# bezirganyan/m2-mixer

Hardware: AMD Instinct MI355X
Metric: training samples/sec AV-MNIST M2-Mixer-B bf16 (higher is better)
Workload: dtype bf16

## Files before the change

### include/m2mixer.h

```cpp
#ifndef M2MIXER_H
#define M2MIXER_H

#include <stdint.h>

#ifdef __cplusplus
extern "C" {
#endif

#define M2M_ABI_VERSION 18
#define M2M_MAX_BLOCKS 8
#define M2M_ROWS_PER_WG 16

#define M2M_SPLIT_GPART 1472

#define M2M_PREC_BF16 0
#define M2M_PREC_F32 1

typedef struct m2m_block {
    const float* ln1_w;
    const float* ln1_b;
    const float* tok_w1;
    const float* tok_b1;
    const float* tok_w2;
    const float* tok_b2;
    const float* ln2_w;
    const float* ln2_b;
    const float* ch_w1;
    const float* ch_b1;
    const float* ch_w2;
    const float* ch_b2;
    void* w1n;
    void* w2c;
    void* w2tn;
    void* w1tc;
    float* ch_b1p;
    float* g_ln1_w; float* g_ln1_b; float* g_tok_w1; float* g_tok_b1; float* g_tok_w2; float* g_tok_b2;
    float* g_ln2_w; float* g_ln2_b; float* g_ch_w1; float* g_ch_b1; float* g_ch_w2; float* g_ch_b2;
    float* x_in;
    float* x_mid;
    void* at_chn;
    void* dyt_chn;
    void* h_chn;
    void* dh_chn;
} m2m_block;

typedef struct m2m_tower {
    int32_t prec;
    int32_t D, N, T, C;
    int32_t Cp;
    int32_t nblocks;
    int32_t has_final_ln;
    float p_drop;
    uint32_t site_base;
    const float* lnf_w;
    const float* lnf_b;
    float* g_lnf_w;
    float* g_lnf_b;
    float* x_final;
    float* ws_a;
    float* ws_b;
    m2m_block blk[M2M_MAX_BLOCKS];
    float* slabs;
    int32_t nsplit;
    int32_t wgrad_flags;
    float* xres;
    float* gpart;
    void* a_nat[M2M_MAX_BLOCKS];
    void* dy_nat[M2M_MAX_BLOCKS];
    float* wslot[M2M_MAX_BLOCKS];
    void* dx0_chn;
} m2m_tower;
#define M2M_WGRAD_OVERWRITE 1
#define M2M_WGRAD_GROUP_SLOTS 4
#define M2M_WGRAD_REDUCES_SMALL 2

typedef struct m2m_embed {
    int32_t prec;
    int32_t Cin, H, W, ph, pw;
    int32_t D;
    int32_t K;
    int32_t Kp;
    const float* w;
    const float* b;
    void* wn;
    float* g_w;
    float* g_b;
    int32_t wgrad_flags;
    int32_t reserved;
} m2m_embed;

int m2m_abi_version(void);
const char* m2m_last_error(void);
int64_t m2m_packed_bytes(int prec, int64_t I, int64_t K);

int m2m_pack(int prec, int mode, int order_k_major, const float* src, int64_t stride_i, int64_t stride_k,
             int64_t I, int64_t K, void* dst, void* stream);
int m2m_pack_tower(const m2m_tower* t, void* stream);
int m2m_pack_embed(const m2m_embed* e, void* stream);
int m2m_pack_all(const m2m_tower* const* towers, int ntowers, const m2m_embed* const* embeds, int nembeds, void* stream);
int m2m_pack_skips_w1tc(const m2m_tower* t);

int m2m_embed_forward(const m2m_embed* e, const float* input, int B, float* x0, void* stream);
typedef struct m2m_step_head {
    float* adam_state; uint32_t* drop_counter; float* losses; int32_t nlosses;
} m2m_step_head;
int m2m_embeds_forward(const m2m_embed* const* embeds, const float* const* inputs, float* const* x0s, const int* nsplits,
                       const int64_t* part_strides, int nembeds, int B, const m2m_step_head* head, void* stream);
int m2m_embed_fwd_splits(const m2m_embed* e);
int m2m_embed_forward_head(const m2m_embed* e, const float* input, int B, float* x0, const m2m_step_head* head, void* stream);

int m2m_tower_forward(const m2m_tower* t, const float* x0, int64_t x0_sample_stride, int B,
                      float* out, int64_t out_sample_stride, float* pooled,
                      int training, uint32_t seed, uint32_t step, const uint32_t* step_dev, void* stream);

int m2m_towers_can_group(const m2m_tower* a, const m2m_tower* b, int B);
typedef struct m2m_tower_io {
    const float* x0; int64_t x0_sample_stride;
    float* out; int64_t out_sample_stride;
    float* pooled;
    int32_t x0_parts;
    int64_t x0_part_stride;
} m2m_tower_io;
int m2m_towers_forward(const m2m_tower* const* towers, const m2m_tower_io* io, int ntowers, int B, int training,
                       uint32_t seed, uint32_t step, const uint32_t* step_dev, void* stream);
int m2m_towers_forward_embeds_ok(const m2m_tower* const* towers, int ntowers, const m2m_embed* const* embeds, int B);
int m2m_towers_forward_embeds(const m2m_tower* const* towers, const m2m_tower_io* io, int ntowers,
                              const m2m_embed* const* embeds, const float* const* inputs, const m2m_step_head* head,
                              int B, int training, uint32_t seed, uint32_t step, const uint32_t* step_dev, void* stream);

int m2m_tower_backward(const m2m_tower* t, int B, const float* d_out, int64_t d_out_sample_stride,
                       const float* d_pooled, float* d_x0, int64_t d_x0_sample_stride,
                       uint32_t seed, uint32_t step, const uint32_t* step_dev, void* stream);
typedef struct m2m_tower_gio {
    const float* d_out; int64_t d_out_sample_stride;
    const float* d_pooled;
    float* d_x0; int64_t d_x0_sample_stride;
} m2m_tower_gio;
int m2m_towers_backward(const m2m_tower* const* towers, const m2m_tower_gio* io, int ntowers, int B,
                        uint32_t seed, uint32_t step, const uint32_t* step_dev, void* stream);
int m2m_tower_wgrad(const m2m_tower* t, int B, uint32_t seed, uint32_t step, const uint32_t* step_dev, void* stream);
int m2m_wgrad_form(const m2m_tower* t, int B);
int m2m_towers_wgrad(const m2m_tower* const* towers, const m2m_tower* const* dev_towers, int ntowers,
                     const m2m_embed* const* embeds, const float* const* inputs, const float* const* d_x0s,
                     const m2m_tower* const* embed_towers, int nembeds,
                     int B, uint32_t seed, uint32_t step, const uint32_t* step_dev, void* stream);
int m2m_wgrad_groups(const m2m_tower* t, int B);
int m2m_embeds_wgrad_form(const m2m_embed* const* embeds, const m2m_tower* const* embed_towers, int nembeds, int B);
int m2m_wgrad_slot_groups(const m2m_tower* const* towers, int ntowers, int B);
int m2m_wgrad_fold(const m2m_tower* t, void* stream);
int m2m_embed_wgrad(const m2m_embed* e, const float* input, const float* d_x0, int B, void* stream);
int m2m_embeds_wgrad(const m2m_embed* const* embeds, const float* const* inputs, const float* const* d_x0s, int nembeds, int B,
                     void* stream);

typedef struct m2m_head {
    const float* pooled;
    const float* w;
    const float* b;
    float* g_w;
    float* g_b;
    float* d_pooled;
    float weight;
    float* g_part;
    const float* tokens;
    int64_t tok_sample_stride;
    int32_t ntok;
} m2m_head;
int m2m_heads_part_tiles(int B);
int m2m_heads_ce(const m2m_head* heads, int nheads, const int64_t* labels, int B, int D, int K,
                 float* logits, float* losses, int32_t* preds, int zero_losses, void* stream);

int m2m_heads_bce(const m2m_head* heads, int nheads, const float* targets, const float* pos_weight, int B, int D, int K,
                  float* logits, float* losses, int32_t* preds, int zero_losses, void* stream);

int m2m_heads_ce_w(const m2m_head* heads, int nheads, const int64_t* labels, int B, int D, int K,
                   float* logits, float* losses, int32_t* preds, int zero_losses, const float* weights, void* stream);
int m2m_heads_bce_w(const m2m_head* heads, int nheads, const float* targets, const float* pos_weight, int B, int D, int K,
                    float* logits, float* losses, int32_t* preds, int zero_losses, const float* weights, void* stream);

int m2m_towers_wgrad_heads(const m2m_tower* const* towers, const m2m_tower* const* dev_towers, int ntowers,
                           const m2m_embed* const* embeds, const float* const* inputs, const float* const* d_x0s,
                           const m2m_tower* const* embed_towers, int nembeds,
                           int B, uint32_t seed, uint32_t step, const uint32_t* step_dev,
                           const m2m_head* heads, int nheads, int K, void* stream);

int m2m_towers_wgrad_tail(const m2m_tower* const* towers, const m2m_tower* const* dev_towers, int ntowers,
                          const m2m_embed* const* embeds, const float* const* inputs, const float* const* d_x0s,
                          const m2m_tower* const* embed_towers, int nembeds,
                          int B, uint32_t seed, uint32_t step, const uint32_t* step_dev,
                          const m2m_head* heads, int nheads, int K, uint32_t* bump_counter, void* stream);

int m2m_tower_backward_heads_ok(const m2m_tower* t, int B, int nheads, int K);
int m2m_tower_backward_heads(const m2m_tower* t, int B, const m2m_head* heads, int nheads, int own, const int64_t* labels,
                             int K, float* logits, float* losses, int32_t* preds, float* d_x0, int64_t d_x0_sample_stride,
                             uint32_t seed, uint32_t step, const uint32_t* step_dev, void* stream);

#define M2M_MLP_MAX_LAYERS 4
typedef struct m2m_mlp {
    int32_t nlayers;
    int32_t has_out;
    int32_t dims[M2M_MLP_MAX_LAYERS + 1];
    float p_drop;
    uint32_t site_base;
    const float* w[M2M_MLP_MAX_LAYERS];
    const float* b[M2M_MLP_MAX_LAYERS];
    float* g_w[M2M_MLP_MAX_LAYERS];
    float* g_b[M2M_MLP_MAX_LAYERS];
    float* act[M2M_MLP_MAX_LAYERS];
} m2m_mlp;
int m2m_mlp_forward(const m2m_mlp* m, const float* x, int B, float* out, int64_t out_sample_stride, float* out_dense,
                    int training, uint32_t seed, uint32_t step, const uint32_t* step_dev, void* stream);
int m2m_mlp_backward(const m2m_mlp* m, const float* x, int B, const float* d_out, int64_t d_out_sample_stride,
                     const float* d_out_dense, void* stream);
int m2m_mlp_forward_ride(const m2m_mlp* m, const float* x, int B, float* out, int64_t out_sample_stride, float* out_dense,
                         int training, uint32_t seed, uint32_t step, const uint32_t* step_dev);
int m2m_mlp_backward_ride(const m2m_mlp* m, const float* x, int B, const float* d_out, int64_t d_out_sample_stride,
                          const float* d_out_dense);
int m2m_mlp_ride_flush(void* stream);

int m2m_adam_step(float* param, float* grad, float* exp_avg, float* exp_avg_sq, int64_t n,
                  float* state, float beta1, float beta2, float eps, float weight_decay,
                  float grad_scale, int bump_step, void* stream);
int m2m_adam_step_bf16(float* param, float* grad, const void* grad_bf16, float* exp_avg, float* exp_avg_sq, int64_t n,
                       float* state, float beta1, float beta2, float eps, float weight_decay,
                       float grad_scale, int bump_step, void* stream);

#define M2M_MAX_GRAD_RANGES 16
typedef struct m2m_grad_range { int64_t lo, n; const float* add; int32_t keep; int32_t reserved; } m2m_grad_range;
int m2m_adam_step_ranges(float* param, float* grad, const void* grad_bf16, float* exp_avg, float* exp_avg_sq, int64_t n,
                         float* state, float beta1, float beta2, float eps, float weight_decay, float grad_scale, int bump_step,
                         const m2m_grad_range* ranges, int nranges, void* stream);

int64_t m2m_adam_pack_plan_bytes(void);
int m2m_adam_pack_plan(const m2m_tower* const* towers, int ntowers, const m2m_embed* const* embeds, int nembeds,
                       float* param, float* grad, const void* grad_bf16, float* exp_avg, float* exp_avg_sq, int64_t n,
                       const float* state, float beta1, float beta2, float eps, float weight_decay, float grad_scale,
                       void* plan_host);
int m2m_adam_pack_plan_ranges(const m2m_tower* const* towers, int ntowers, const m2m_embed* const* embeds, int nembeds,
                              float* param, float* grad, const void* grad_bf16, float* exp_avg, float* exp_avg_sq, int64_t n,
                              const float* state, float beta1, float beta2, float eps, float weight_decay, float grad_scale,
                              const m2m_grad_range* ranges, int nranges, void* plan_host);
int m2m_adam_pack_all(const m2m_tower* const* towers, int ntowers, const m2m_embed* const* embeds, int nembeds,
                      const void* plan_dev, const void* plan_host, void* stream);

int m2m_step_prologue(float* adam_state, uint32_t* drop_counter, float* losses, int nlosses, void* stream);

int m2m_counter_add(uint32_t* counter, uint32_t delta, void* stream);

#define M2M_FUSION_SUM 1
#define M2M_FUSION_MEAN 2
#define M2M_FUSION_MAX 3
int m2m_fusion_forward(int mode, const float* a, const float* b, float* y, int64_t n, void* stream);
int m2m_fusion_backward(int mode, const float* a, const float* b, const float* dy, float* da, float* db, int64_t n, void* stream);

typedef struct m2m_gate {
    int32_t D;
    int32_t reserved;
    const float *w1, *b1, *w2, *b2, *wz, *bz;
    float *g_w1, *g_b1, *g_w2, *g_b2, *g_wz, *g_bz;
    float *t1, *t2, *z, *dh, *part;
} m2m_gate;
int64_t m2m_gate_part_floats(int64_t rows, int D);
int m2m_gate_forward(const m2m_gate* g, const float* a, const float* b, float* y, int64_t rows, int save, void* stream);
int m2m_gate_backward(const m2m_gate* g, const float* dy, float* da, float* db, int64_t rows, void* stream);
int m2m_gate_wgrad(const m2m_gate* g, const float* a, const float* b, int64_t rows, void* stream);

#define M2M_SCORES_MAX_CLASSES 64
#define M2M_SCORES_MAX_LABELS 128
int m2m_scores_multiclass(const int32_t* preds, const int64_t* labels, int nheads, int B, int K, uint64_t* table, void* stream);
int m2m_scores_multilabel(const int32_t* preds, const float* targets, int nheads, int B, int K, uint64_t* table, void* stream);

int m2m_dropout_mask(const m2m_tower* t, int blk, int site, int B, uint32_t seed, uint32_t step,
                     uint8_t* mask, void* stream);
int m2m_gelu_probe(const float* x, float* y, float* dy, int64_t n, void* stream);
int m2m_gelu_table_probe(int form, const float* x, float* y, float* dy, int64_t n, float scale, void* stream);
int m2m_gemm_probe(int prec, const float* A, const float* Bm, int I, int J, int K,
                   const float* Bc, int J2, float* C, float* C2, void* workspace, void* stream);

int m2m_clock_probe(uint64_t* out, int nwg, int spin_ticks, void* stream);

#ifdef __cplusplus
}
#endif
#endif
```

### m2_mixer_amd/_lib.py

```python
from __future__ import annotations

import ctypes as C
import os
import subprocess

_HERE = os.path.dirname(os.path.abspath(__file__))
LIB_PATH = os.environ.get("M2M_LIB_PATH", os.path.join(_HERE, "libm2mixer.so"))
CSRC = os.path.join(_HERE, "csrc")

ABI_VERSION = 18
MAX_BLOCKS = 8
ROWS_PER_WG = 16
HCHN_PAD = 4096
SPLIT_ROWS = 128
SPLIT_MAX = 8
SPLIT_GPART = 1472
PREC_BF16, PREC_F32 = 0, 1
PREC_BY_NAME = {"bf16": PREC_BF16, "fp32": PREC_F32, "f32": PREC_F32}

_fp = C.c_void_p


class Block(C.Structure):
    PARAMS = ["ln1_w", "ln1_b", "tok_w1", "tok_b1", "tok_w2", "tok_b2", "ln2_w", "ln2_b",
              "ch_w1", "ch_b1", "ch_w2", "ch_b2"]
    PACKED = ["w1n", "w2c", "w2tn", "w1tc", "ch_b1p"]
    GRADS = ["g_" + p for p in PARAMS]
    SAVED = ["x_in", "x_mid", "at_chn", "dyt_chn", "h_chn", "dh_chn"]
    _fields_ = [(n, _fp) for n in PARAMS + PACKED + GRADS + SAVED]


class Tower(C.Structure):
    _fields_ = [("prec", C.c_int32), ("D", C.c_int32), ("N", C.c_int32), ("T", C.c_int32), ("C", C.c_int32),
                ("Cp", C.c_int32), ("nblocks", C.c_int32), ("has_final_ln", C.c_int32),
                ("p_drop", C.c_float), ("site_base", C.c_uint32),
                ("lnf_w", _fp), ("lnf_b", _fp), ("g_lnf_w", _fp), ("g_lnf_b", _fp), ("x_final", _fp),
                ("ws_a", _fp), ("ws_b", _fp), ("blk", Block * MAX_BLOCKS),
                ("slabs", _fp), ("nsplit", C.c_int32), ("wgrad_flags", C.c_int32), ("xres", _fp), ("gpart", _fp),
                ("a_nat", _fp * MAX_BLOCKS), ("dy_nat", _fp * MAX_BLOCKS),
                ("wslot", _fp * MAX_BLOCKS),
                ("dx0_chn", _fp)]


WGRAD_OVERWRITE = 1
WGRAD_REDUCES_SMALL = 2
WGRAD_GROUP_SLOTS = 4
MAX_GRAD_RANGES = 16


class GradRange(C.Structure):
    _fields_ = [("lo", C.c_int64), ("n", C.c_int64), ("add", _fp), ("keep", C.c_int32), ("reserved", C.c_int32)]


class TowerIO(C.Structure):
    _fields_ = [("x0", _fp), ("x0_ss", C.c_int64), ("out", _fp), ("out_ss", C.c_int64), ("pooled", _fp),
                ("x0_parts", C.c_int32), ("x0_part_stride", C.c_int64)]


class StepHead(C.Structure):
    _fields_ = [("adam_state", _fp), ("drop_counter", _fp), ("losses", _fp), ("nlosses", C.c_int32)]


class TowerGIO(C.Structure):
    _fields_ = [("d_out", _fp), ("d_out_ss", C.c_int64), ("d_pooled", _fp), ("d_x0", _fp), ("d_x0_ss", C.c_int64)]


class Embed(C.Structure):
    _fields_ = [("prec", C.c_int32), ("Cin", C.c_int32), ("H", C.c_int32), ("W", C.c_int32), ("ph", C.c_int32),
                ("pw", C.c_int32), ("D", C.c_int32), ("K", C.c_int32), ("Kp", C.c_int32),
                ("w", _fp), ("b", _fp), ("wn", _fp), ("g_w", _fp), ("g_b", _fp), ("wgrad_flags", C.c_int32), ("reserved", C.c_int32)]


class Head(C.Structure):
    _fields_ = [("pooled", _fp), ("w", _fp), ("b", _fp), ("g_w", _fp), ("g_b", _fp), ("d_pooled", _fp),
                ("weight", C.c_float), ("g_part", _fp), ("tokens", _fp), ("tok_sample_stride", C.c_int64), ("ntok", C.c_int32)]


SCORES_MAX_CLASSES, SCORES_MAX_LABELS = 64, 128
FUSION_SUM, FUSION_MEAN, FUSION_MAX = 1, 2, 3


class Gate(C.Structure):
    _fields_ = [("D", C.c_int32), ("reserved", C.c_int32)] + [(n, _fp) for n in (
        "w1", "b1", "w2", "b2", "wz", "bz", "g_w1", "g_b1", "g_w2", "g_b2", "g_wz", "g_bz", "t1", "t2", "z", "dh", "part")]


MLP_MAX_LAYERS = 4


class Mlp(C.Structure):
    _fields_ = [("nlayers", C.c_int32), ("has_out", C.c_int32), ("dims", C.c_int32 * (MLP_MAX_LAYERS + 1)),
                ("p_drop", C.c_float), ("site_base", C.c_uint32),
                ("w", _fp * MLP_MAX_LAYERS), ("b", _fp * MLP_MAX_LAYERS), ("g_w", _fp * MLP_MAX_LAYERS),
                ("g_b", _fp * MLP_MAX_LAYERS), ("act", _fp * MLP_MAX_LAYERS)]


SIGNATURES = {
    "m2m_abi_version": (C.c_int, []),
    "m2m_last_error": (C.c_char_p, []),
    "m2m_packed_bytes": (C.c_int64, [C.c_int, C.c_int64, C.c_int64]),
    "m2m_pack": (C.c_int, [C.c_int, C.c_int, C.c_int, _fp, C.c_int64, C.c_int64, C.c_int64, C.c_int64, _fp, _fp]),
    "m2m_pack_tower": (C.c_int, [C.POINTER(Tower), _fp]),
    "m2m_pack_embed": (C.c_int, [C.POINTER(Embed), _fp]),
    "m2m_pack_skips_w1tc": (C.c_int, [C.POINTER(Tower)]),
    "m2m_pack_all": (C.c_int, [C.POINTER(C.POINTER(Tower)), C.c_int, C.POINTER(C.POINTER(Embed)), C.c_int, _fp]),
    "m2m_embed_forward": (C.c_int, [C.POINTER(Embed), _fp, C.c_int, _fp, _fp]),
    "m2m_embed_forward_head": (C.c_int, [C.POINTER(Embed), _fp, C.c_int, _fp, C.POINTER(StepHead), _fp]),
    "m2m_tower_forward": (C.c_int, [C.POINTER(Tower), _fp, C.c_int64, C.c_int, _fp, C.c_int64, _fp, C.c_int,
                                    C.c_uint32, C.c_uint32, _fp, _fp]),
    "m2m_tower_backward": (C.c_int, [C.POINTER(Tower), C.c_int, _fp, C.c_int64, _fp, _fp, C.c_int64,
                                     C.c_uint32, C.c_uint32, _fp, _fp]),
    "m2m_tower_backward_heads_ok": (C.c_int, [C.POINTER(Tower), C.c_int, C.c_int, C.c_int]),
    "m2m_tower_backward_heads": (C.c_int, [C.POINTER(Tower), C.c_int, C.POINTER(Head), C.c_int, C.c_int, _fp, C.c_int, _fp, _fp, _fp, _fp,
                                           C.c_int64, C.c_uint32, C.c_uint32, _fp, _fp]),
    "m2m_tower_wgrad": (C.c_int, [C.POINTER(Tower), C.c_int, C.c_uint32, C.c_uint32, _fp, _fp]),
    "m2m_towers_can_group": (C.c_int, [C.POINTER(Tower), C.POINTER(Tower), C.c_int]),
    "m2m_towers_forward": (C.c_int, [C.POINTER(C.POINTER(Tower)), C.POINTER(TowerIO), C.c_int, C.c_int, C.c_int, C.c_uint32,
                                     C.c_uint32, _fp, _fp]),
    "m2m_towers_forward_embeds_ok": (C.c_int, [C.POINTER(C.POINTER(Tower)), C.c_int, C.POINTER(C.POINTER(Embed)), C.c_int]),
    "m2m_towers_forward_embeds": (C.c_int, [C.POINTER(C.POINTER(Tower)), C.POINTER(TowerIO), C.c_int, C.POINTER(C.POINTER(Embed)),
                                            C.POINTER(_fp), C.POINTER(StepHead), C.c_int, C.c_int, C.c_uint32, C.c_uint32, _fp, _fp]),
    "m2m_towers_backward": (C.c_int, [C.POINTER(C.POINTER(Tower)), C.POINTER(TowerGIO), C.c_int, C.c_int, C.c_uint32, C.c_uint32,
                                      _fp, _fp]),
    "m2m_towers_wgrad": (C.c_int, [C.POINTER(C.POINTER(Tower)), C.POINTER(_fp), C.c_int, C.POINTER(C.POINTER(Embed)), C.POINTER(_fp),
                                   C.POINTER(_fp), C.POINTER(C.POINTER(Tower)), C.c_int, C.c_int, C.c_uint32, C.c_uint32, _fp, _fp]),
    "m2m_towers_wgrad_heads": (C.c_int, [C.POINTER(C.POINTER(Tower)), C.POINTER(_fp), C.c_int, C.POINTER(C.POINTER(Embed)), C.POINTER(_fp),
                                         C.POINTER(_fp), C.POINTER(C.POINTER(Tower)), C.c_int, C.c_int, C.c_uint32, C.c_uint32, _fp,
                                         C.POINTER(Head), C.c_int, C.c_int, _fp]),
    "m2m_towers_wgrad_tail": (C.c_int, [C.POINTER(C.POINTER(Tower)), C.POINTER(_fp), C.c_int, C.POINTER(C.POINTER(Embed)), C.POINTER(_fp),
                                        C.POINTER(_fp), C.POINTER(C.POINTER(Tower)), C.c_int, C.c_int, C.c_uint32, C.c_uint32, _fp,
                                        C.POINTER(Head), C.c_int, C.c_int, _fp, _fp]),
    "m2m_heads_part_tiles": (C.c_int, [C.c_int]),
    "m2m_wgrad_form": (C.c_int, [C.POINTER(Tower), C.c_int]),
    "m2m_embeds_wgrad_form": (C.c_int, [C.POINTER(C.POINTER(Embed)), C.POINTER(C.POINTER(Tower)), C.c_int, C.c_int]),
    "m2m_wgrad_groups": (C.c_int, [C.POINTER(Tower), C.c_int]),
    "m2m_wgrad_slot_groups": (C.c_int, [C.POINTER(C.POINTER(Tower)), C.c_int, C.c_int]),
    "m2m_wgrad_fold": (C.c_int, [C.POINTER(Tower), _fp]),
    "m2m_adam_step_ranges": (C.c_int, [_fp, _fp, _fp, _fp, _fp, C.c_int64, _fp, C.c_float, C.c_float, C.c_float, C.c_float,
                                       C.c_float, C.c_int, C.POINTER(GradRange), C.c_int, _fp]),
    "m2m_counter_add": (C.c_int, [_fp, C.c_uint32, _fp]),
    "m2m_embed_wgrad": (C.c_int, [C.POINTER(Embed), _fp, _fp, C.c_int, _fp]),
    "m2m_embeds_wgrad": (C.c_int, [C.POINTER(C.POINTER(Embed)), C.POINTER(_fp), C.POINTER(_fp), C.c_int, C.c_int, _fp]),
    "m2m_embeds_forward": (C.c_int, [C.POINTER(C.POINTER(Embed)), C.POINTER(_fp), C.POINTER(_fp), C.POINTER(C.c_int), C.POINTER(C.c_int64),
                                     C.c_int, C.c_int, C.POINTER(StepHead), _fp]),
    "m2m_embed_fwd_splits": (C.c_int, [C.POINTER(Embed)]),
    "m2m_heads_ce": (C.c_int, [C.POINTER(Head), C.c_int, _fp, C.c_int, C.c_int, C.c_int, _fp, _fp, _fp, C.c_int, _fp]),
    "m2m_step_prologue": (C.c_int, [_fp, _fp, _fp, C.c_int, _fp]),
    "m2m_heads_bce": (C.c_int, [C.POINTER(Head), C.c_int, _fp, _fp, C.c_int, C.c_int, C.c_int, _fp, _fp, _fp, C.c_int, _fp]),
    "m2m_heads_ce_w": (C.c_int, [C.POINTER(Head), C.c_int, _fp, C.c_int, C.c_int, C.c_int, _fp, _fp, _fp, C.c_int, _fp, _fp]),
    "m2m_heads_bce_w": (C.c_int, [C.POINTER(Head), C.c_int, _fp, _fp, C.c_int, C.c_int, C.c_int, _fp, _fp, _fp, C.c_int, _fp, _fp]),
    "m2m_fusion_forward": (C.c_int, [C.c_int, _fp, _fp, _fp, C.c_int64, _fp]),
    "m2m_fusion_backward": (C.c_int, [C.c_int, _fp, _fp, _fp, _fp, _fp, C.c_int64, _fp]),
    "m2m_gate_part_floats": (C.c_int64, [C.c_int64, C.c_int]),
    "m2m_gate_forward": (C.c_int, [C.POINTER(Gate), _fp, _fp, _fp, C.c_int64, C.c_int, _fp]),
    "m2m_gate_backward": (C.c_int, [C.POINTER(Gate), _fp, _fp, _fp, C.c_int64, _fp]),
    "m2m_gate_wgrad": (C.c_int, [C.POINTER(Gate), _fp, _fp, C.c_int64, _fp]),
    "m2m_scores_multiclass": (C.c_int, [_fp, _fp, C.c_int, C.c_int, C.c_int, _fp, _fp]),
    "m2m_scores_multilabel": (C.c_int, [_fp, _fp, C.c_int, C.c_int, C.c_int, _fp, _fp]),
    "m2m_mlp_forward": (C.c_int, [C.POINTER(Mlp), _fp, C.c_int, _fp, C.c_int64, _fp, C.c_int, C.c_uint32, C.c_uint32,
                                  _fp, _fp]),
    "m2m_mlp_backward": (C.c_int, [C.POINTER(Mlp), _fp, C.c_int, _fp, C.c_int64, _fp, _fp]),
    "m2m_mlp_forward_ride": (C.c_int, [C.POINTER(Mlp), _fp, C.c_int, _fp, C.c_int64, _fp, C.c_int, C.c_uint32, C.c_uint32, _fp]),
    "m2m_mlp_backward_ride": (C.c_int, [C.POINTER(Mlp), _fp, C.c_int, _fp, C.c_int64, _fp]),
    "m2m_mlp_ride_flush": (C.c_int, [_fp]),
    "m2m_adam_step": (C.c_int, [_fp, _fp, _fp, _fp, C.c_int64, _fp, C.c_float, C.c_float, C.c_float, C.c_float,
                                C.c_float, C.c_int, _fp]),
    "m2m_adam_step_bf16": (C.c_int, [_fp, _fp, _fp, _fp, _fp, C.c_int64, _fp, C.c_float, C.c_float, C.c_float, C.c_float,
                                     C.c_float, C.c_int, _fp]),
    "m2m_adam_pack_plan_bytes": (C.c_int64, []),
    "m2m_adam_pack_plan": (C.c_int, [C.POINTER(C.POINTER(Tower)), C.c_int, C.POINTER(C.POINTER(Embed)), C.c_int, _fp, _fp, _fp, _fp, _fp,
                                    C.c_int64, _fp, C.c_float, C.c_float, C.c_float, C.c_float, C.c_float, _fp]),
    "m2m_adam_pack_plan_ranges": (C.c_int, [C.POINTER(C.POINTER(Tower)), C.c_int, C.POINTER(C.POINTER(Embed)), C.c_int, _fp, _fp, _fp, _fp, _fp,
                                           C.c_int64, _fp, C.c_float, C.c_float, C.c_float, C.c_float, C.c_float,
                                           C.POINTER(GradRange), C.c_int, _fp]),
    "m2m_adam_pack_all": (C.c_int, [C.POINTER(C.POINTER(Tower)), C.c_int, C.POINTER(C.POINTER(Embed)), C.c_int, _fp, _fp, _fp]),
    "m2m_dropout_mask": (C.c_int, [C.POINTER(Tower), C.c_int, C.c_int, C.c_int, C.c_uint32, C.c_uint32, _fp, _fp]),
    "m2m_gelu_probe": (C.c_int, [_fp, _fp, _fp, C.c_int64, _fp]),
    "m2m_gelu_table_probe": (C.c_int, [C.c_int, _fp, _fp, _fp, C.c_int64, C.c_float, _fp]),
    "m2m_gemm_probe": (C.c_int, [C.c_int, _fp, _fp, C.c_int, C.c_int, C.c_int, _fp, C.c_int, _fp, _fp, _fp, _fp]),
    "m2m_clock_probe": (C.c_int, [_fp, C.c_int, C.c_int, _fp]),
}

_lib = None


def csrc_hash() -> str:
    import glob
    import hashlib
    h = hashlib.sha256()
    for f in sorted(glob.glob(os.path.join(CSRC, "*.hip")) + glob.glob(os.path.join(CSRC, "*.h")) +
                    [os.path.join(os.path.dirname(_HERE), "include", "m2mixer.h")]):
        h.update(os.path.basename(f).encode())
        h.update(open(f, "rb").read())
    return h.hexdigest()


def build(force: bool = False, verbose: bool = False) -> str:
    if force:
        subprocess.run(["make", "-C", CSRC, "clean"], check=True, capture_output=not verbose)
    r = subprocess.run(["make", "-C", CSRC, "-j", str(min(6, os.cpu_count() or 2))], capture_output=True, text=True)
    if r.returncode != 0:
        raise RuntimeError("building libm2mixer.so failed:\n" + r.stdout[-4000:] + r.stderr[-4000:])
    if verbose:
        print(r.stdout)
    return LIB_PATH


def lib() -> C.CDLL:
    global _lib
    if _lib is None:
        if not os.path.exists(LIB_PATH):
            raise RuntimeError(
                f"{LIB_PATH} is missing: the M2-Mixer hot path exists only as the HIP library "
                "(python -c 'import __graft_entry__ as g; g.build()' builds it); there is no CPU fallback")
        L = C.CDLL(LIB_PATH)
        for name, (res, args) in SIGNATURES.items():
            fn = getattr(L, name)
            fn.restype = res
            fn.argtypes = args
        got = L.m2m_abi_version()
        if got != ABI_VERSION:
            raise RuntimeError(f"libm2mixer ABI {got} != binding ABI {ABI_VERSION}; rebuild")
        _lib = L
    return _lib


def check(rc: int, what: str = "") -> None:
    if rc != 0:
        msg = lib().m2m_last_error().decode("utf-8", "replace")
        kind = "unsupported shape/argument" if rc == -1 else "HIP runtime error"
        raise RuntimeError(f"libm2mixer {what}: {kind}: {msg}")


def ptr(t) -> int:
    return 0 if t is None else t.data_ptr()


def stream_ptr() -> int:
    import torch
    return torch.cuda.current_stream().cuda_stream


def packed_bytes(prec: int, I: int, K: int) -> int:
    kb = 32 if prec == PREC_BF16 else 16
    return ((I + 15) // 16) * ((K + kb - 1) // kb) * 1024
```

### m2_mixer_amd/config.py

```python
from __future__ import annotations

import os

from . import _lib as L

_state = {
    "precision": os.environ.get("M2M_PRECISION", "bf16"),
    "seed": None,
    "device_step": False,
}


SWITCHES = {
    "M2M_PRECISION": ("bf16", "import of config", "bf16 / fp32: the precision of engines and modules built without an explicit one"),
    "M2M_LIB_PATH": (None, "import of _lib", "load another build of libm2mixer.so (default: the one beside the package)"),
    "M2M_DIST_BACKEND": (None, "parallel.init_from_env", "torch.distributed backend (default nccl on GPUs; gloo: several ranks on one GPU)"),
    "M2M_FUSED_UPDATE": (None, "engine construction", "1 / 0 force Adam + operand re-pack as one launch / as two; unset: one launch"),
    "M2M_CONCURRENT": ("1", "engine construction", "0: every launch on the main stream, no grouped two-tower launches"),
    "M2M_WGRAD_OVERWRITE": ("1", "engine construction", "weight gradients with a single owner are written, Adam leaves them uncleared"),
    "M2M_WGRAD_SLOT": ("1", "engine construction", "second row group of a grouped weight-gradient launch into a slot that Adam adds"),
    "M2M_EARLY_FUSION_WGRAD": ("0", "engine construction", "wide towers: the fusion tower's weight gradients on a side stream"),
    "M2M_HEADS_POOL": ("1", "engine construction", "wide towers: the heads launch pools the tower outputs itself"),
    "M2M_DEFER_SMALL": ("1", "engine construction", "the fusion backward's small-gradient slots are reduced by the weight-gradient launch"),
    "M2M_HEAD_SLOTS": ("1", "engine construction", "the heads' weight gradients through slots (bit-reproducible) instead of float atomics"),
    "M2M_GROUP_SLOTS": ("1", "engine construction", "the two-tower backward's small gradients through per-workgroup slots"),
    "M2M_EMBED_FAST": ("1", "engine construction", "patch-embedding weight gradients in the single-owner form (d_x0^T image)"),
    "M2M_EMBED_FOLD": ("0", "engine construction", "patch embeddings inside the two-tower forward launch"),
    "M2M_MIMIC_STREAMS": (None, "engine construction", "none / fwd / bwd / both: side streams of the MIMIC step; unset: none up to batch 1024, else both"),
    "M2M_MIMIC_MERGED_TAIL": ("1", "engine construction", "MIMIC on one stream: one weight-gradient launch, one Adam, one re-pack"),
    "M2M_MIMIC_EMBED_WGRAD_MERGED": ("1", "engine construction", "MIMIC merged tail: the input projection's weight gradient inside the towers' launch"),
    "M2M_MLP_RIDE": ("1", "engine construction", "MIMIC: the static MLP's workgroups ride in the time tower's token-mixing launches"),
    "M2M_CAPTURE_SHARE_SLOTS": ("0", "engine.capture()", "multi-step capture: every step reads the same input slot (diagnostic)"),
}


def switch(name: str, default=None):
    return os.environ.get(name, SWITCHES[name][0] if default is None else default)


def switch_on(name: str) -> bool:
    return switch(name) != "0" if SWITCHES[name][0] == "1" else switch(name) == "1"


def set_precision(name: str) -> None:
    if name not in L.PREC_BY_NAME:
        raise ValueError(f"precision must be one of {sorted(L.PREC_BY_NAME)}")
    _state["precision"] = name


def get_precision() -> str:
    return _state["precision"]


def prec_id(name: str | None = None) -> int:
    return L.PREC_BY_NAME[name or _state["precision"]]


def set_dropout_seed(seed: int) -> None:
    _state["seed"] = int(seed) & 0xFFFFFFFF


def dropout_seed() -> int:
    if _state["seed"] is None:
        import torch
        _state["seed"] = int(torch.initial_seed()) & 0xFFFFFFFF
    return _state["seed"]


def set_device_dropout_step(on: bool) -> None:
    _state["device_step"] = bool(on)


def device_dropout_step() -> bool:
    return _state["device_step"]
```

### m2_mixer_amd/csrc/embed.hip

```cpp
#include "tile.h"
#include "embed_wgrad.h"

#include "embed_fwd.h"
#include "dispatch.h"

template <int P, int D, int RB>
__global__ __launch_bounds__(NTHREADS) void embed_fwd_kernel(const m2m_embed em, const float* __restrict__ in, long M, int N,
                                                             float* __restrict__ x0, int fast, const m2m_step_head head) {
    extern __shared__ __attribute__((aligned(16))) char smem[];
    if (blockIdx.x == 0) {
        const int t = threadIdx.x;
        if (t == 0 && head.adam_state) head.adam_state[0] += 1.0f;
        if (t == 1 && head.drop_counter) *head.drop_counter += 1u;
        if (head.losses && t < head.nlosses) head.losses[t] = 0.f;
    }
    if (P == PREC_BF16 && fast) embed_fwd_fast_body<D>(em, in, M, N, x0, blockIdx.x, 0, 1, smem);
    else embed_fwd_body<P, D, RB>(em, in, M, N, x0, blockIdx.x, smem);
}

struct EmbedFwdGroupArgs {
    m2m_embed em[2];
    const float* in[2];
    float* x0[2];
    long M[2];
    int N[2], nwg0, fast[2], nsplit[2];
    long part_stride[2];
    float* adam_state;
    unsigned int* drop_counter;
    float* losses;
    int nlosses, prologue;
};
template <int P, int D, int RB>
__global__ __launch_bounds__(NTHREADS, (P == PREC_BF16 && D <= 128) ? 4 : 1) void embed_fwd_group_kernel(const EmbedFwdGroupArgs a) {
    extern __shared__ __attribute__((aligned(16))) char smem[];
    if (a.prologue && blockIdx.x == 0) {
        const int t = threadIdx.x;
        if (t == 0 && a.adam_state) a.adam_state[0] += 1.0f;
        if (t == 1 && a.drop_counter) *a.drop_counter += 1u;
        if (a.losses && t < a.nlosses) a.losses[t] = 0.f;
    }
    const int e = (int)blockIdx.x < a.nwg0 ? 0 : 1;
    const int wg = e ? blockIdx.x - a.nwg0 : blockIdx.x;
    if (P == PREC_BF16 && a.fast[e]) {
        const int ns = a.nsplit[e], split = wg % ns;
        embed_fwd_fast_body<D>(a.em[e], a.in[e], a.M[e], a.N[e], a.x0[e] + split * a.part_stride[e], wg / ns, split, ns, smem);
    }
    else {
        const int ns = a.nsplit[e], split = wg % ns, tile = wg / ns;
        if (split == 0) embed_fwd_body<P, D, RB>(a.em[e], a.in[e], a.M[e], a.N[e], a.x0[e], tile, smem);
        else {
            float* part = a.x0[e] + split * a.part_stride[e];
            const long m0 = (long)tile * RB;
            for (int idx = threadIdx.x; idx < RB * D; idx += NTHREADS) {
                const long m = m0 + idx / D;
                if (m < a.M[e]) part[m * D + idx % D] = 0.f;
            }
        }
    }
}

template <int P, int D>
__global__ __launch_bounds__(NTHREADS) void embed_wgrad_kernel(const m2m_embed em, const float* __restrict__ in,
                                                               const float* __restrict__ dx0, long M, int N, int tiles_per_group) {
    extern __shared__ __attribute__((aligned(16))) char smem[];
    embed_wgrad_body<P, D, NTHREADS>(em, in, dx0, M, N, tiles_per_group, blockIdx.x, blockIdx.y, gridDim.y == 1, smem);
}

template <int P, int D>
__global__ __launch_bounds__(NTHREADS) void embed_wgrad_group_kernel(const EmbedWgradGroupArgs a) {
    extern __shared__ __attribute__((aligned(16))) char smem[];
    embed_wgrad_group_body<P, D, NTHREADS>(a, blockIdx.x, smem);
}

int m2m_check_embed(const m2m_embed* e, int B) {
    if (!e || B < 1) { m2m_set_error("embed: bad argument", __FILE__, __LINE__); return -1; }
    if (e->H % e->ph || e->W % e->pw) { m2m_set_error("embed: image not divisible by patch", __FILE__, __LINE__); return -1; }
    if (e->K != e->Cin * e->ph * e->pw) { m2m_set_error("embed: K != Cin*ph*pw", __FILE__, __LINE__); return -1; }
    const int KB = e->prec == PREC_BF16 ? 32 : 16;
    if (e->Kp % KB || e->Kp < e->K) { m2m_set_error("embed: Kp must be K rounded up to the k-block", __FILE__, __LINE__); return -1; }
    if (e->Kp > EMB_KMAX - EMB_KS) { m2m_set_error("embed: patch too large (Cin*ph*pw must be <= 3968)", __FILE__, __LINE__); return -1; }
    return 0;
}

template <int P, int D>
static int launch_embed_fwd(const m2m_embed* e, const float* in, int B, float* x0, hipStream_t st, const m2m_step_head* head = nullptr) {
    m2m_step_head hd;
    memset(&hd, 0, sizeof(hd));
    if (head) {
        if (head->nlosses < 0 || head->nlosses > 64) { m2m_set_error("embed_forward: step head nlosses must be in [0, 64]", __FILE__, __LINE__); return -1; }
        hd = *head;
    }
    const int N = (e->H / e->ph) * (e->W / e->pw);
    const long M = (long)B * N;
    constexpr int RB = 16;
    const size_t lds = (size_t)RB * EMB_LD * 4 + (size_t)RB * EMB_KS * Prec<P>::ESZ + EMB_KMAX * 4 + RB * 8;
    return m2m_launch<embed_fwd_kernel<P, D, RB>>(dim3((unsigned)((M + RB - 1) / RB)), dim3(NTHREADS), lds, lds, st, *e, in, M, N, x0,
                                                  (int)embed_fwd_fast_ok(e, in), hd);
}
template <int P, int D>
static int launch_embed_fwd_group(const m2m_embed* const* es, const float* const* ins, float* const* x0s, const int* nsplits,
                                  const int64_t* part_strides, const m2m_step_head* head, int B, hipStream_t st) {
    constexpr int RB = 16;
    EmbedFwdGroupArgs a;
    memset(&a, 0, sizeof(a));
    if (head) {
        if (head->nlosses < 0 || head->nlosses > 64) { m2m_set_error("embeds_forward: step head nlosses must be in [0, 64]", __FILE__, __LINE__); return -1; }
        a.prologue = 1; a.adam_state = head->adam_state; a.drop_counter = head->drop_counter; a.losses = head->losses; a.nlosses = head->nlosses;
    }
    const int first = es[1]->Kp > es[0]->Kp ? 1 : 0;
    int total = 0;
    for (int k = 0; k < 2; ++k) {
        const int i = k == 0 ? first : 1 - first;
        const int N = (es[i]->H / es[i]->ph) * (es[i]->W / es[i]->pw);
        a.em[k] = *es[i]; a.in[k] = ins[i]; a.x0[k] = x0s[i]; a.N[k] = N; a.M[k] = (long)B * N;
        a.fast[k] = embed_fwd_fast_ok(es[i], ins[i]);
        a.nsplit[k] = nsplits ? nsplits[i] : 1;
        a.part_stride[k] = part_strides ? (long)part_strides[i] : 0;
        if (a.nsplit[k] < 1 || a.nsplit[k] > 4 || (a.nsplit[k] > 1 && a.part_stride[k] < a.M[k] * (long)D)) {
            m2m_set_error("embeds_forward: 1..4 k-splits, part stride >= B*N*D", __FILE__, __LINE__);
            return -1;
        }
        const int nwg = (int)((a.M[k] + RB - 1) / RB) * a.nsplit[k];
        if (k == 0) a.nwg0 = nwg;
        total += nwg;
    }
    const size_t lds = (size_t)RB * EMB_LD * 4 + (size_t)RB * EMB_KS * Prec<P>::ESZ + EMB_KMAX * 4 + RB * 8;
    return m2m_launch<embed_fwd_group_kernel<P, D, RB>>(dim3((unsigned)total), dim3(NTHREADS), lds, lds, st, a);
}

template <int P, int D>
static int launch_embed_wgrad(const m2m_embed* e, const float* in, const float* dx0, int B, hipStream_t st) {
    const EmbedWgradPlan pl = embed_wgrad_plan(e, B, 256);
    const size_t lds = embed_wgrad_lds<D, P>();
    return m2m_launch<embed_wgrad_kernel<P, D>>(dim3((unsigned)pl.nchunks, (unsigned)pl.groups), dim3(NTHREADS), lds, lds, st, *e, in, dx0, pl.M, pl.N, pl.tpg);
}
template <int P, int D>
static int launch_embed_wgrad_group(const m2m_embed* const* es, const float* const* ins, const float* const* dx0s, int B, hipStream_t st) {
    EmbedWgradGroupArgs a;
    const int total = embed_wgrad_group_args(a, es, ins, dx0s, B, 256);
    const size_t lds = embed_wgrad_lds<D, P>();
    return m2m_launch<embed_wgrad_group_kernel<P, D>>(dim3((unsigned)total), dim3(NTHREADS), lds, lds, st, a);
}

extern "C" int m2m_embed_forward(const m2m_embed* e, const float* input, int B, float* x0, void* stream) {
    return m2m_embed_forward_head(e, input, B, x0, nullptr, stream);
}
extern "C" int m2m_embed_forward_head(const m2m_embed* e, const float* input, int B, float* x0, const m2m_step_head* head, void* stream) {
    if (int rc = m2m_check_embed(e, B)) return rc;
    hipStream_t st = reinterpret_cast<hipStream_t>(stream);
    const int rc = m2m_dispatch_pd(m2m_wide_dims{}, e->prec, e->D, [&](auto P, auto D) { return launch_embed_fwd<P(), D()>(e, input, B, x0, st, head); });
    if (rc != M2M_NO_BUILD) return rc;
    m2m_set_error("embed_forward: unsupported (prec, D)", __FILE__, __LINE__);
    return -1;
}

extern "C" int m2m_embed_wgrad(const m2m_embed* e, const float* input, const float* d_x0, int B, void* stream) {
    if (int rc = m2m_check_embed(e, B)) return rc;
    hipStream_t st = reinterpret_cast<hipStream_t>(stream);
    const int rc = m2m_dispatch_pd(m2m_wide_dims{}, e->prec, e->D, [&](auto P, auto D) { return launch_embed_wgrad<P(), D()>(e, input, d_x0, B, st); });
    if (rc != M2M_NO_BUILD) return rc;
    m2m_set_error("embed_wgrad: unsupported (prec, D)", __FILE__, __LINE__);
    return -1;
}

extern "C" int m2m_embeds_wgrad(const m2m_embed* const* embeds, const float* const* inputs, const float* const* d_x0s, int nembeds,
                                int B, void* stream) {
    if (!embeds || !inputs || !d_x0s || nembeds != EMB_GROUP) { m2m_set_error("embeds_wgrad: exactly two embeddings", __FILE__, __LINE__); return -1; }
    for (int i = 0; i < nembeds; ++i) {
        if (int rc = m2m_check_embed(embeds[i], B)) return rc;
        if (embeds[i]->prec != embeds[0]->prec || embeds[i]->D != embeds[0]->D) {
            m2m_set_error("embeds_wgrad: the embeddings of one launch must share precision and hidden_dim", __FILE__, __LINE__);
            return -1;
        }
    }
    hipStream_t st = reinterpret_cast<hipStream_t>(stream);
    const m2m_embed* e = embeds[0];
    const int rc = m2m_dispatch_pd(m2m_wide_dims{}, e->prec, e->D, [&](auto P, auto D) { return launch_embed_wgrad_group<P(), D()>(embeds, inputs, d_x0s, B, st); });
    if (rc != M2M_NO_BUILD) return rc;
    m2m_set_error("embeds_wgrad: unsupported (prec, D)", __FILE__, __LINE__);
    return -1;
}

extern "C" int m2m_embed_fwd_splits(const m2m_embed* e) {
    if (!e) return 1;
    static const int forced = m2m_env_int("M2M_EMBED_SPLITS", 0);
    const bool pays = embed_fwd_fast_ok(e, nullptr) && e->Kp >= 4 * EMB_FKS;
    if (pays && forced >= 1 && forced <= 4) return forced;
    return pays ? 2 : 1;
}

extern "C" int m2m_embeds_forward(const m2m_embed* const* embeds, const float* const* inputs, float* const* x0s, const int* nsplits,
                                  const int64_t* part_strides, int nembeds, int B, const m2m_step_head* head, void* stream) {
    if (!embeds || !inputs || !x0s || nembeds != 2) { m2m_set_error("embeds_forward: exactly two embeddings", __FILE__, __LINE__); return -1; }
    for (int i = 0; i < nembeds; ++i) {
        if (int rc = m2m_check_embed(embeds[i], B)) return rc;
        if (embeds[i]->prec != embeds[0]->prec || embeds[i]->D != embeds[0]->D) {
            m2m_set_error("embeds_forward: the embeddings of one launch must share precision and hidden_dim", __FILE__, __LINE__);
            return -1;
        }
    }
    hipStream_t st = reinterpret_cast<hipStream_t>(stream);
    const m2m_embed* e = embeds[0];
    const int rc = m2m_dispatch_pd(m2m_wide_dims{}, e->prec, e->D, [&](auto P, auto D) { return launch_embed_fwd_group<P(), D()>(embeds, inputs, x0s, nsplits, part_strides, head, B, st); });
    if (rc != M2M_NO_BUILD) return rc;
    m2m_set_error("embeds_forward: unsupported (prec, D)", __FILE__, __LINE__);
    return -1;
}
```

### m2_mixer_amd/csrc/embed_fwd.h

```cpp
#pragma once
#include "tile.h"
#include "embed_wgrad.h"

#define EMB_KS 128
#define EMB_LD (EMB_KS + 4)
#define EMB_KMAX 4096

template <int P, int D, int RB>
static __device__ __forceinline__ void embed_fwd_body(const m2m_embed& em, const float* __restrict__ in, long M, int N,
                                                      float* __restrict__ x0, int wg, char* smem) {
    typedef Prec<P> Pr;
    constexpr int DT = D / 16, KSB = EMB_KS / Pr::KB;
    constexpr int DPW = (DT + NWAVES - 1) / NWAVES;
    float* tile = reinterpret_cast<float*>(smem);
    char* img = smem + RB * EMB_LD * 4;
    int* koff = reinterpret_cast<int*>(img + RB * EMB_KS * Pr::ESZ);
    long* rbase = reinterpret_cast<long*>(koff + EMB_KMAX);

    const int tid = threadIdx.x, lane = tid & 63, wave = tid >> 6, g = lane >> 4, il = lane & 15;
    PatchGeom pg{em.Cin, em.H, em.W, em.ph, em.pw, em.W / em.pw, N, em.K};
    const long m0 = (long)wg * RB;
    const int nKB = em.Kp / Pr::KB;
    const int kext = (em.Kp + EMB_KS - 1) / EMB_KS * EMB_KS;
    for (int k = tid; k < kext; k += NTHREADS) koff[k] = patch_koff(pg, k);
    if (tid < RB) rbase[tid] = patch_rowbase(pg, m0 + tid, M);

    f32x4_t acc[(RB / 16)][DPW];
#pragma unroll
    for (int mt = 0; mt < (RB / 16); ++mt)
#pragma unroll
        for (int j = 0; j < DPW; ++j) acc[mt][j] = f32x4_t{0.f, 0.f, 0.f, 0.f};

    constexpr int EPT = RB * EMB_KS / NTHREADS;
    float pre[EPT];
    Frag wpre[DPW][KSB];
    auto load_stage = [&](int k0) {
#pragma unroll
        for (int i = 0; i < EPT; ++i) {
            const int idx = i * NTHREADS + tid;
            const int r = idx / EMB_KS, kk = idx % EMB_KS;
            const long rb = rbase[r];
            const int ko = koff[k0 + kk];
            pre[i] = (rb >= 0 && ko >= 0) ? in[rb + ko] : 0.f;
        }
        const int kb0 = k0 / Pr::KB;
#pragma unroll
        for (int j = 0; j < DPW; ++j) {
            const int dt = wave + NWAVES * j;
#pragma unroll
            for (int kb = 0; kb < KSB; ++kb) {
                wpre[j][kb].u = u32x4_t{0u, 0u, 0u, 0u};
                if (dt < DT && kb0 + kb < nKB) wpre[j][kb] = ld_frag_global(em.wn, (long)dt * nKB + kb0 + kb, lane);
            }
        }
    };
    __syncthreads();
    load_stage(0);
    for (int k0 = 0; k0 < em.Kp; k0 += EMB_KS) {
#pragma unroll
        for (int i = 0; i < EPT; ++i) {
            const int idx = i * NTHREADS + tid;
            tile[(idx / EMB_KS) * EMB_LD + idx % EMB_KS] = pre[i];
        }
        Frag wcur[DPW][KSB];
#pragma unroll
        for (int j = 0; j < DPW; ++j)
#pragma unroll
            for (int kb = 0; kb < KSB; ++kb) wcur[j][kb] = wpre[j][kb];
        __syncthreads();
        if (k0 + EMB_KS < em.Kp) load_stage(k0 + EMB_KS);
        for (int slot = tid; slot < (RB / 16) * KSB * 64; slot += NTHREADS) {
            const int blk = slot >> 6;
            *reinterpret_cast<u32x4_t*>(img + slot * 16) =
                gather_slot<P>(tile, EMB_LD, PACK_NAT, false, blk / KSB, blk % KSB, slot & 63);
        }
        __syncthreads();
#pragma unroll
        for (int j = 0; j < DPW; ++j) {
            const int dt = wave + NWAVES * j;
            if (dt < DT) {
#pragma unroll
                for (int kb = 0; kb < KSB; ++kb) {
#pragma unroll
                    for (int mt = 0; mt < (RB / 16); ++mt) {
                        const Frag a = ld_frag_lds(img, mt * KSB + kb, lane);
                        Pr::mma(acc[mt][j], a, wcur[j][kb]);
                    }
                }
            }
        }
    }
#pragma unroll
    for (int j = 0; j < DPW; ++j) {
        const int dt = wave + NWAVES * j;
        if (dt < DT) {
            const int d = 16 * dt + il;
            const float bv = em.b[d];
#pragma unroll
            for (int mt = 0; mt < (RB / 16); ++mt)
#pragma unroll
                for (int r = 0; r < 4; ++r) {
                    const long m = m0 + 16 * mt + 4 * g + r;
                    if (m < M) x0[m * D + d] = acc[mt][j][r] + bv;
                }
        }
    }
}

#define EMB_FKS 256
#define EMB_FDEPTH 2
template <int D>
static __device__ __forceinline__ void embed_fwd_fast_body(const m2m_embed& em, const float* __restrict__ in, long M, int N,
                                                           float* __restrict__ x0, int wg, int split, int nsplit, char* smem) {
    typedef Prec<PREC_BF16> Pr;
    constexpr int KSB = EMB_FKS / 32, DT = D / 16, DPW = (DT + NWAVES - 1) / NWAVES, IMG_B = 16 * EMB_FKS * 2;
    static_assert(KSB == NWAVES, "one k-block of the stage per wave");
    char* img = smem;
    const int tid = threadIdx.x, lane = tid & 63, wave = tid >> 6, g = lane >> 4, il = lane & 15;
    PatchGeom pg{em.Cin, em.H, em.W, em.ph, em.pw, em.W / em.pw, N, em.K};
    const long m0 = (long)wg * 16;
    const long rb = patch_rowbase(pg, m0 + il, M);
    const int nKB = em.Kp / 32;
    const int nst_all = (em.Kp + EMB_FKS - 1) / EMB_FKS;
    const int per = (nst_all + nsplit - 1) / nsplit;
    const int st_begin = split * per, nst = min(nst_all, st_begin + per);

    f32x4_t acc[DPW];
#pragma unroll
    for (int j = 0; j < DPW; ++j) acc[j] = f32x4_t{0.f, 0.f, 0.f, 0.f};
    struct Pre {
        f32x4_t p0, p1;
        Frag w[DPW][KSB];
    };
    auto load = [&](Pre& p, int st) {
        const int k = min(st * EMB_FKS + wave * 32 + 8 * g, em.K - 8);
        const float* src = in + (rb >= 0 ? rb : 0) + patch_koff(pg, k);
        p.p0 = *reinterpret_cast<const f32x4_t*>(src);
        p.p1 = *reinterpret_cast<const f32x4_t*>(src + 4);
#pragma unroll
        for (int j = 0; j < DPW; ++j) {
            const int dt = min(wave + NWAVES * j, DT - 1);
#pragma unroll
            for (int kb = 0; kb < KSB; ++kb) p.w[j][kb] = ld_frag_global(em.wn, (long)dt * nKB + min(st * KSB + kb, nKB - 1), lane);
        }
    };
    auto step = [&](Pre& p, int st) {
        const bool valid = rb >= 0 && st < nst && st * EMB_FKS + wave * 32 + 8 * g < em.K;
        Frag f;
        f.u[0] = pack_bf2(p.p0[0], p.p0[1]); f.u[1] = pack_bf2(p.p0[2], p.p0[3]);
        f.u[2] = pack_bf2(p.p1[0], p.p1[1]); f.u[3] = pack_bf2(p.p1[2], p.p1[3]);
        if (!valid) f.u = u32x4_t{0u, 0u, 0u, 0u};
        char* cur = img + ((st - st_begin) & 1) * IMG_B;
        *reinterpret_cast<u32x4_t*>(cur + tid * 16) = f.u;
        __syncthreads();
#pragma unroll
        for (int kb = 0; kb < KSB; ++kb) {
            const Frag a = ld_frag_lds(cur, kb, lane);
#pragma unroll
            for (int j = 0; j < DPW; ++j)
                if (wave + NWAVES * j < DT) Pr::mma(acc[j], a, p.w[j][kb]);
        }
        load(p, st + EMB_FDEPTH);
    };
    Pre ring[EMB_FDEPTH];
#pragma unroll
    for (int d = 0; d < EMB_FDEPTH; ++d) load(ring[d], st_begin + d);
    for (int st = st_begin; st < nst; st += EMB_FDEPTH) {
#pragma unroll
        for (int d = 0; d < EMB_FDEPTH; ++d) step(ring[d], st + d);
    }
#pragma unroll
    for (int j = 0; j < DPW; ++j) {
        const int dt = wave + NWAVES * j;
        if (dt < DT) {
            const int d = 16 * dt + il;
            const float bv = split == 0 ? em.b[d] : 0.f;
#pragma unroll
            for (int r = 0; r < 4; ++r) {
                const long m = m0 + 4 * g + r;
                if (m < M) x0[m * D + d] = acc[j][r] + bv;
            }
        }
    }
}
static inline bool embed_fwd_fast_ok(const m2m_embed* e, const float* in) {
    return e->prec == PREC_BF16 && e->pw % 8 == 0 && e->W % 4 == 0 && e->K >= 8 && (reinterpret_cast<uintptr_t>(in) & 15) == 0;
}
```

### m2_mixer_amd/csrc/embed_wgrad.h

```cpp
#pragma once
#include "host.h"

#define EBM 32

struct PatchGeom {
    int Cin, H, W, ph, pw, GW, N, K;
};
static __device__ __forceinline__ int patch_koff(const PatchGeom& pg, int k) {
    if (k >= pg.K) return -1;
    const int c = k / (pg.ph * pg.pw), rem = k % (pg.ph * pg.pw);
    const int py = rem / pg.pw, px = rem % pg.pw;
    return (c * pg.H + py) * pg.W + px;
}
static __device__ __forceinline__ long patch_rowbase(const PatchGeom& pg, long m, long M) {
    if (m >= M) return -1;
    const long b = m / pg.N;
    const int n = (int)(m % pg.N);
    const int gy = n / pg.GW, gx = n % pg.GW;
    return (b * pg.Cin * pg.H + gy * pg.ph) * (long)pg.W + gx * pg.pw;
}

template <int P, int D, int NT>
static __device__ __forceinline__ void embed_wgrad_body(const m2m_embed& em, const float* __restrict__ in,
                                                        const float* __restrict__ dx0, long M, int N, int tiles_per_group,
                                                        int chunk, int group, bool single, char* smem) {
    typedef Prec<P> Pr;
    constexpr int DT = D / 16, NKM = EBM / Pr::KB, XLD = TileGeom<D>::XLD;
    constexpr int KC = 64, KCT = KC / 16, PLD = KC + 4;
    constexpr int DPW = (DT + (NT / 64) - 1) / (NT / 64);
    constexpr int NDX = (EBM * (D / 4) + NT - 1) / NT;
    constexpr int NPT = EBM * KC / NT;
    static_assert(NT % KC == 0 && EBM % (NT / KC) == 0, "patch tile mapping");
    float* dxt = reinterpret_cast<float*>(smem);
    float* pt = dxt + EBM * XLD;
    char* aimg = reinterpret_cast<char*>(pt + EBM * PLD);
    char* bimg = aimg + EBM * D * Pr::ESZ;

    const int tid = threadIdx.x, lane = tid & 63, wave = tid >> 6, g = lane >> 4, il = lane & 15;
    PatchGeom pg{em.Cin, em.H, em.W, em.ph, em.pw, em.W / em.pw, N, em.K};
    const int k0 = chunk * KC;
    const int ko = patch_koff(pg, k0 + (tid % KC));

    f32x4_t acc[DPW][KCT];
#pragma unroll
    for (int j = 0; j < DPW; ++j)
#pragma unroll
        for (int kt = 0; kt < KCT; ++kt) acc[j][kt] = f32x4_t{0.f, 0.f, 0.f, 0.f};
    float bsum = 0.f;

    const long ntiles = (M + EBM - 1) / EBM;
    const long t_begin = (long)group * tiles_per_group;
    const long t_end = min(ntiles, t_begin + tiles_per_group);
    float4 dxr[NDX];
    float ptr_[NPT];
    auto load_tile = [&](long tl) {
        const long m0 = tl * EBM;
#pragma unroll
        for (int i = 0; i < NDX; ++i) {
            const int idx = i * NT + tid;
            const int r = idx / (D / 4), c = (idx % (D / 4)) * 4;
            dxr[i] = make_float4(0.f, 0.f, 0.f, 0.f);
            if (idx < EBM * (D / 4) && m0 + r < M) dxr[i] = *reinterpret_cast<const float4*>(dx0 + (m0 + r) * D + c);
        }
#pragma unroll
        for (int i = 0; i < NPT; ++i) {
            const long rb = patch_rowbase(pg, m0 + tid / KC + (NT / KC) * i, M);
            ptr_[i] = (rb >= 0 && ko >= 0) ? in[rb + ko] : 0.f;
        }
    };
    if (t_begin < t_end) load_tile(t_begin);
    for (long tl = t_begin; tl < t_end; ++tl) {
        __syncthreads();
#pragma unroll
        for (int i = 0; i < NDX; ++i) {
            const int idx = i * NT + tid;
            if (idx < EBM * (D / 4)) *reinterpret_cast<float4*>(dxt + (idx / (D / 4)) * XLD + (idx % (D / 4)) * 4) = dxr[i];
        }
#pragma unroll
        for (int i = 0; i < NPT; ++i) pt[(tid / KC + (NT / KC) * i) * PLD + tid % KC] = ptr_[i];
        if (tl + 1 < t_end) load_tile(tl + 1);
        __syncthreads();
        if (chunk == 0 && tid < D) {
            float s = 0.f;
            for (int r = 0; r < EBM; ++r) s += dxt[r * XLD + tid];
            bsum += s;
        }
        for (int slot = tid; slot < DT * NKM * 64; slot += NT) {
            const int blk = slot >> 6;
            *reinterpret_cast<u32x4_t*>(aimg + slot * 16) =
                gather_slot<P>(dxt, XLD, PACK_NAT, true, blk / NKM, blk % NKM, slot & 63);
        }
        for (int slot = tid; slot < KCT * NKM * 64; slot += NT) {
            const int blk = slot >> 6;
            *reinterpret_cast<u32x4_t*>(bimg + slot * 16) =
                gather_slot<P>(pt, PLD, PACK_NAT, true, blk / NKM, blk % NKM, slot & 63);
        }
        __syncthreads();
#pragma unroll
        for (int j = 0; j < DPW; ++j) {
            const int dt = wave + (NT / 64) * j;
            if (dt < DT) {
#pragma unroll
                for (int kbm = 0; kbm < NKM; ++kbm) {
                    const Frag a = ld_frag_lds(aimg, dt * NKM + kbm, lane);
#pragma unroll
                    for (int kt = 0; kt < KCT; ++kt) {
                        const Frag b = ld_frag_lds(bimg, kt * NKM + kbm, lane);
                        Pr::mma(acc[j][kt], a, b);
                    }
                }
            }
        }
    }
#pragma unroll
    for (int j = 0; j < DPW; ++j) {
        const int dt = wave + (NT / 64) * j;
        if (dt < DT) {
#pragma unroll
            for (int kt = 0; kt < KCT; ++kt)
#pragma unroll
                for (int r = 0; r < 4; ++r) {
                    const int d = 16 * dt + 4 * g + r, k = k0 + 16 * kt + il;
                    if (k < em.K) {
                        float* p = em.g_w + (long)d * em.K + k;
                        if (single) *p += acc[j][kt][r]; else atomicAdd(p, acc[j][kt][r]);
                    }
                }
        }
    }
    if (chunk == 0 && tid < D) { if (single) em.g_b[tid] += bsum; else atomicAdd(em.g_b + tid, bsum); }
}

#define EFK 32
template <int D, int NT> static constexpr size_t embed_wgrad_fast_red_bytes() { return (size_t)(NT / 64) * (EFK / 16) * (D / 16) * 64 * 16; }
template <int D, int NT>
static __device__ __forceinline__ void embed_wgrad_fast_body(const m2m_embed& em, const float* __restrict__ in,
                                                             const char* __restrict__ dx0_chn, long M, int N, int npairs, int rpt,
                                                             int chunk, bool vec2, char* smem) {
    typedef Prec<PREC_BF16> Pr;
    constexpr int DT = D / 16, NW = NT / 64, NB = EFK / 16;
    static_assert(NB == 2, "two 16-column fragments per workgroup (the 8-byte gather pairs them)");
    const int tid = threadIdx.x, lane = tid & 63, g = lane >> 4, il = lane & 15;
    const int wave = __builtin_amdgcn_readfirstlane(tid >> 6);
    PatchGeom pg{em.Cin, em.H, em.W, em.ph, em.pw, em.W / em.pw, N, em.K};
    const int k0 = chunk * EFK;
    int ko[NB];
#pragma unroll
    for (int jb = 0; jb < NB; ++jb) ko[jb] = patch_koff(pg, vec2 ? k0 + 2 * il + jb : k0 + 16 * jb + il);
    int* tokoff = reinterpret_cast<int*>(smem + embed_wgrad_fast_red_bytes<D, NT>());
    for (int n = tid; n < N; n += NT) tokoff[n] = (n / pg.GW) * pg.ph * pg.W + (n % pg.GW) * pg.pw;
    __syncthreads();
    const unsigned int sstride = (unsigned int)(em.Cin * em.H * em.W), uN = (unsigned int)N, uM = (unsigned int)M;
    const unsigned int magic = 0xFFFFFFFFu / uN;

    f32x4_t acc[NB][DT];
#pragma unroll
    for (int jb = 0; jb < NB; ++jb)
#pragma unroll
        for (int dt = 0; dt < DT; ++dt) acc[jb][dt] = f32x4_t{0.f, 0.f, 0.f, 0.f};

    struct Tile { Frag a[DT]; float v[NB][8]; unsigned int okbits; };
    auto load = [&](Tile& t, int p) {
#pragma unroll
        for (int dt = 0; dt < DT; ++dt) t.a[dt] = ld_frag_global(dx0_chn, (long)p * DT + dt, lane);
        unsigned int rb[8];
        bool okr[8];
#pragma unroll
        for (int e = 0; e < 8; ++e) {
            const int r = 4 * g + (e & 3);
            const unsigned int row = (unsigned int)((2 * p + (e >> 2)) * rpt + r);
            okr[e] = r < rpt && row < uM;
            const unsigned int rowc = okr[e] ? row : 0u;
            unsigned int q = __umulhi(rowc, magic);
            unsigned int n = rowc - q * uN;
            if (n >= uN) { n -= uN; q += 1u; }
            rb[e] = q * sstride + (unsigned int)tokoff[n];
        }
        if (vec2) {
            const unsigned int k2 = (unsigned int)max(ko[0], 0);
#pragma unroll
            for (int e = 0; e < 8; ++e) {
                const float2 x = *reinterpret_cast<const float2*>(in + rb[e] + k2);
                t.v[0][e] = x.x; t.v[1][e] = x.y;
            }
        } else {
#pragma unroll
            for (int e = 0; e < 8; ++e)
#pragma unroll
                for (int jb = 0; jb < NB; ++jb) t.v[jb][e] = in[rb[e] + (unsigned int)max(ko[jb], 0)];
        }
        t.okbits = 0u;
#pragma unroll
        for (int e = 0; e < 8; ++e) t.okbits |= (okr[e] ? 1u : 0u) << e;
    };
    auto mac = [&](const Tile& t) {
#pragma unroll
        for (int jb = 0; jb < NB; ++jb) {
            Frag b;
            float z[8];
#pragma unroll
            for (int e = 0; e < 8; ++e) z[e] = ((t.okbits >> e) & 1u) && ko[jb] >= 0 ? t.v[jb][e] : 0.f;
#pragma unroll
            for (int e = 0; e < 4; ++e) b.u[e] = pack_bf2(z[2 * e], z[2 * e + 1]);
#pragma unroll
            for (int dt = 0; dt < DT; ++dt) Pr::mma(acc[jb][dt], t.a[dt], b);
        }
    };
    Tile t0, t1;
    const int p0 = wave;
    if (p0 < npairs) load(t0, p0);
    for (int p = p0; p < npairs; p += 2 * NW) {
        if (p + NW < npairs) load(t1, p + NW);
        mac(t0);
        if (p + NW < npairs) {
            if (p + 2 * NW < npairs) load(t0, p + 2 * NW);
            mac(t1);
        }
    }
    f32x4_t* red = reinterpret_cast<f32x4_t*>(smem);
#pragma unroll
    for (int jb = 0; jb < NB; ++jb)
#pragma unroll
        for (int dt = 0; dt < DT; ++dt) red[((wave * NB + jb) * DT + dt) * 64 + lane] = acc[jb][dt];
    __syncthreads();
    for (int q = wave; q < NB * DT; q += NW) {
        const int jb = q / DT, dt = q % DT;
        f32x4_t s = red[q * 64 + lane];
#pragma unroll
        for (int w = 1; w < NW; ++w) s = s + red[(w * NB * DT + q) * 64 + lane];
        const int k = vec2 ? k0 + 2 * il + jb : k0 + 16 * jb + il;
        if (k < em.K) {
            const bool store = (em.wgrad_flags & M2M_WGRAD_OVERWRITE) != 0;
#pragma unroll
            for (int r = 0; r < 4; ++r) {
                float* qd = em.g_w + (long)(16 * dt + 4 * g + r) * em.K + k;
                *qd = store ? s[r] : *qd + s[r];
            }
        }
    }
    if (chunk == 0) {
        Frag ones;
        ones.u = u32x4_t{0x3F803F80u, 0x3F803F80u, 0x3F803F80u, 0x3F803F80u};
        f32x4_t accb[DT];
#pragma unroll
        for (int dt = 0; dt < DT; ++dt) accb[dt] = f32x4_t{0.f, 0.f, 0.f, 0.f};
        for (int p = wave; p < npairs; p += NW) {
            Frag a[DT];
#pragma unroll
            for (int dt = 0; dt < DT; ++dt) a[dt] = ld_frag_global(dx0_chn, (long)p * DT + dt, lane);
#pragma unroll
            for (int dt = 0; dt < DT; ++dt) Pr::mma(accb[dt], a[dt], ones);
        }
        __syncthreads();
#pragma unroll
        for (int dt = 0; dt < DT; ++dt) red[(wave * DT + dt) * 64 + lane] = accb[dt];
        __syncthreads();
        for (int dt = wave; dt < DT; dt += NW) {
            f32x4_t sb = red[dt * 64 + lane];
#pragma unroll
            for (int w = 1; w < NW; ++w) sb = sb + red[(w * DT + dt) * 64 + lane];
            if (il == 0) {
#pragma unroll
                for (int r = 0; r < 4; ++r) em.g_b[16 * dt + 4 * g + r] += sb[r];
            }
        }
    }
}
template <int D, int NT> static constexpr size_t embed_wgrad_fast_lds() { return embed_wgrad_fast_red_bytes<D, NT>() + 128 * sizeof(int); }

#define EMB_GROUP 2
struct EmbedWgradGroupArgs {
    m2m_embed em[EMB_GROUP];
    const float* in[EMB_GROUP];
    const float* dx0[EMB_GROUP];
    long M[EMB_GROUP];
    int N[EMB_GROUP], tpg[EMB_GROUP], nchunks[EMB_GROUP], groups[EMB_GROUP];
    const char* dx0_chn[EMB_GROUP];
    int npairs[EMB_GROUP], rpt[EMB_GROUP], vec2[EMB_GROUP], fast;
};
template <int P, int D, int NT>
static __device__ __forceinline__ void embed_wgrad_group_body(const EmbedWgradGroupArgs& a, int id, char* smem) {
    const int n0 = a.nchunks[0] * a.groups[0];
    const int e = id < n0 ? 0 : 1;
    if (e) id -= n0;
    if constexpr (P == PREC_BF16) {
        if (a.fast) {
            embed_wgrad_fast_body<D, NT>(a.em[e], a.in[e], a.dx0_chn[e], a.M[e], a.N[e], a.npairs[e], a.rpt[e], id, a.vec2[e] != 0, smem);
            return;
        }
    }
    if constexpr (NT % 64 == 0 && EBM % (NT / 64) == 0)
        embed_wgrad_body<P, D, NT>(a.em[e], a.in[e], a.dx0[e], a.M[e], a.N[e], a.tpg[e], id % a.nchunks[e], id / a.nchunks[e],
                                   a.groups[e] == 1, smem);
}

struct EmbedWgradPlan { long M; int N, nchunks, groups, tpg; };
static EmbedWgradPlan embed_wgrad_plan(const m2m_embed* e, int B, int target_wgs) {
    EmbedWgradPlan pl;
    pl.N = (e->H / e->ph) * (e->W / e->pw);
    pl.M = (long)B * pl.N;
    pl.nchunks = (e->K + 63) / 64;
    const long ntiles = (pl.M + EBM - 1) / EBM;
    long groups = (target_wgs + pl.nchunks - 1) / pl.nchunks;
    if (groups > ntiles / 4) groups = ntiles / 4;
    if (groups < 1) groups = 1;
    pl.tpg = (int)((ntiles + groups - 1) / groups);
    pl.groups = (int)((ntiles + pl.tpg - 1) / pl.tpg);
    return pl;
}
template <int D, int P> static constexpr size_t embed_wgrad_lds() {
    return (size_t)EBM * TileGeom<D>::XLD * 4 + (size_t)EBM * 68 * 4 + (size_t)EBM * D * Prec<P>::ESZ + (size_t)EBM * 64 * Prec<P>::ESZ;
}


static inline int embed_wgrad_group_args_fast(EmbedWgradGroupArgs& a, const m2m_embed* const* es, const float* const* ins,
                                              const m2m_tower* const* tw, int B) {
    memset(&a, 0, sizeof(a));
    int total = 0;
    for (int i = 0; i < EMB_GROUP; ++i) {
        const m2m_embed* e = es[i];
        const m2m_tower* t = tw ? tw[i] : nullptr;
        const int N = (e->H / e->ph) * (e->W / e->pw);
        if (!t || !t->dx0_chn || e->prec != PREC_BF16 || t->prec != PREC_BF16 || m2m_is_wide(t) || t->N != N || t->D != e->D) return 0;
        if (m2m_split_eligible(t, B, 1)) return 0;
        if (N > 128 || e->D > 128 || (long)B * e->Cin * e->H * e->W >= (1L << 31)) return 0;
        const int SPW = BM / t->N, nchain = (B + SPW - 1) / SPW;
        a.em[i] = *e; a.in[i] = ins[i]; a.dx0_chn[i] = (const char*)t->dx0_chn;
        a.M[i] = (long)B * N; a.N[i] = N; a.npairs[i] = (nchain * BM + WPAIR - 1) / WPAIR; a.rpt[i] = SPW * t->N;
        a.nchunks[i] = (e->K + EFK - 1) / EFK; a.groups[i] = 1; a.tpg[i] = 0;
        static const int vec2_on = m2m_env_int("M2M_EMBED_VEC2", 1);
        a.vec2[i] = (vec2_on && e->pw % 2 == 0 && e->W % 2 == 0 && ((long)e->H * e->W) % 2 == 0 && e->K % 2 == 0 && ((uintptr_t)ins[i] & 7) == 0) ? 1 : 0;
        total += a.nchunks[i];
    }
    a.fast = 1;
    return total;
}

static inline int embed_wgrad_group_args(EmbedWgradGroupArgs& a, const m2m_embed* const* es, const float* const* ins,
                                         const float* const* dx0s, int B, int target_wgs, int n = EMB_GROUP) {
    memset(&a, 0, sizeof(a));
    if (n == 1) {
        const EmbedWgradPlan p0 = embed_wgrad_plan(es[0], B, target_wgs);
        a.em[0] = *es[0]; a.in[0] = ins[0]; a.dx0[0] = dx0s[0];
        a.M[0] = p0.M; a.N[0] = p0.N; a.tpg[0] = p0.tpg; a.nchunks[0] = p0.nchunks; a.groups[0] = p0.groups;
        a.em[1] = *es[0];
        return p0.nchunks * p0.groups;
    }
    EmbedWgradPlan pl[EMB_GROUP];
    for (int i = 0; i < EMB_GROUP; ++i) pl[i] = embed_wgrad_plan(es[i], B, target_wgs);
    const int first = pl[1].tpg > pl[0].tpg ? 1 : 0;
    int total = 0;
    for (int k = 0; k < EMB_GROUP; ++k) {
        const int i = k == 0 ? first : 1 - first;
        a.em[k] = *es[i]; a.in[k] = ins[i]; a.dx0[k] = dx0s[i];
        a.M[k] = pl[i].M; a.N[k] = pl[i].N; a.tpg[k] = pl[i].tpg; a.nchunks[k] = pl[i].nchunks; a.groups[k] = pl[i].groups;
        total += pl[i].nchunks * pl[i].groups;
    }
    return total;
}
```

### m2_mixer_amd/csrc/tower_wgrad.hip

```cpp
#include "tile.h"
#include "embed_wgrad.h"
#include "dispatch.h"
#include <string.h>

#if defined(__HIP_DEVICE_COMPILE__)
#define M2M_GLOBAL_AS __attribute__((address_space(1)))
#else
#define M2M_GLOBAL_AS
#endif

#define WBM 32
#define WG_RING_MAX 24
#define WG_WAVES 4
#define WG_WAVES_WIDE 5
#define WG_LA 4
#define WG_MINWAVES 2
#define WG_OUT_ATOMIC 0
#define WG_OUT_ADD 1
#define WG_OUT_STORE 2

TIMER_DECL(g_tm_wg);
TIMER_READER(m2m_debug_timers_wgrad, g_tm_wg)

#include "tower_wgrad_rc.h"
// ... 174 lines not shown
#pragma unroll
            for (int j = 0; j < CPW; ++j) {
                hf[j].u = u32x4_t{x.h0[2 * j], x.h0[2 * j + 1], x.h1[2 * j], x.h1[2 * j + 1]};
                df[j].u = u32x4_t{x.d0[2 * j], x.d0[2 * j + 1], x.d1[2 * j], x.d1[2 * j + 1]};
            }
            load_st(min(tile + 1, t_end - 1));
            load_hd(x, min(tile + 2, t_end - 1));
            __syncthreads();
            constexpr int NQ = DT;
            constexpr int LA = WG_LA < NQ ? WG_LA : NQ;
            Frag aq[LA], dq[LA];
#pragma unroll
            for (int q = 0; q < LA; ++q) { aq[q] = ld_frag_lds(cur, q, lane); dq[q] = ld_frag_lds(cur + IMG_B, q, lane); }
#pragma unroll
            for (int q = 0; q < NQ; ++q) {
                const Frag at = aq[q % LA], dyt = dq[q % LA];
                if (q + LA < NQ) { aq[q % LA] = ld_frag_lds(cur, q + LA, lane); dq[q % LA] = ld_frag_lds(cur + IMG_B, q + LA, lane); }
#pragma unroll
                for (int j = 0; j < CPW; ++j) {
                    Pr::mma(dw1[j][q], df[j], at);
                    Pr::mma(dw2[j][q], hf[j], dyt);
                }
                if (q == NQ - 1) {
#pragma unroll
                    for (int j = 0; j < CPW; ++j) Pr::mma(db1[j], df[j], ones);
                }
            }
        };
        HD ring[2];
        load_hd(ring[0], t_begin);
        load_st(t_begin);
        load_hd(ring[1], min(t_begin + 1, t_end - 1));
        int tile = t_begin, it = 0;
        for (; tile + 2 <= t_end; tile += 2) {
            step2(ring[0], tile, it++);
            step2(ring[1], tile + 1, it++);
        }
        if (tile < t_end) step2(ring[0], tile, it++);
    } else {
    Pre p[DEPTH];
#pragma unroll
    for (int k = 0; k < DEPTH; ++k) tile_load(p[k], min(t_begin + k, t_end - 1), t_end);
    int tile = t_begin, it = 0;
    if (DEPTH == 1) {
        for (; tile < t_end; ++tile) step(p[0], tile, t_end, it++);
    } else {
        for (; tile + DEPTH <= t_end; tile += DEPTH) {
#pragma unroll
            for (int k = 0; k < DEPTH; ++k) step(p[k], tile + k, t_end, it++);
        }
#pragma unroll
        for (int k = 0; k + 1 < DEPTH; ++k)
            if (tile + k < t_end) step(p[k], tile + k, t_end, it++);
    }
    }

    __syncthreads();
    wgrad_write_w<D, CPW>(dw1, dw2, out, ct0, nct, C, smem, wave, lane);
#pragma unroll
    for (int j = 0; j < CPW; ++j) {
        if (ct0 + j >= nct || il != 0) continue;
#pragma unroll
        for (int r = 0; r < 4; ++r) {
            const int c = 16 * (ct0 + j) + 4 * g + r;
            if (c >= C) continue;
            if (out.mode == WG_OUT_ATOMIC) atomicAdd(out.b1 + c, db1[j][r]);
            else if (out.mode == WG_OUT_ADD) out.b1[c] += db1[j][r];
            else out.b1[c] = db1[j][r];
        }
    }
    TIMER_MARK(g_tm_wg, 4);
}

template <class TW>
static __device__ __forceinline__ WgOut wgrad_out(const TW& tw, int b, int group, int ngroups, int slot_mode) {
    const m2m_block& bk = tw.blk[b];
    WgOut o;
    o.w1 = bk.g_ch_w1; o.w2 = bk.g_ch_w2; o.b1 = bk.g_ch_b1;
    const bool overwrite = (tw.wgrad_flags & M2M_WGRAD_OVERWRITE) != 0;
    if (ngroups == 1) o.mode = overwrite ? WG_OUT_STORE : WG_OUT_ADD;
    else if (slot_mode) {
        if (group == 0) o.mode = overwrite ? WG_OUT_STORE : WG_OUT_ADD;
        else {
            const long cd = (long)tw.C * tw.D;
            float* s = tw.wslot[b];
            o.w1 = s; o.b1 = s + cd; o.w2 = s + cd + tw.C;
            o.mode = WG_OUT_STORE;
        }
    } else o.mode = WG_OUT_ATOMIC;
    return o;
}

template <int P, int D, int RCDM> struct WgradKernelGeom {
    static constexpr bool RC = RCDM >= 0;
    static constexpr int LDS_B = RC ? RcGeom<D>::LDS_B : WgradGeom<P, D>::LDS_B;
    static constexpr int COLS = RC ? RcGeom<D>::COLS : WgradGeom<P, D>::COLS;
    static constexpr int MINWAVES = RC ? 2 : WgradGeom<P, D>::MINWAVES;
    static constexpr int THREADS = RC ? RC_THREADS : WgradGeom<P, D>::THREADS;
};

template <int P, int D, int RCDM, class TW>
static __device__ __forceinline__ void wgrad_dispatch(const TW& tw, int b, int slice, int group, int ngroups, int slot_mode, int ntiles,
                                                      int tpg, int rows_per_t16, unsigned int seed, unsigned int step, char* smem) {
    const WgOut out = wgrad_out(tw, b, group, ngroups, slot_mode);
    if constexpr (RCDM >= 0) {
        const Drop dr = make_drop(true, tw.p_drop, seed, step, tw.site_base + 4u * (unsigned int)b + 2u);
        wgrad_rc_body<D, RCDM>(tw.blk[b], out, tw.Cp, tw.C, slice, group, ntiles, tpg, rows_per_t16, dr.key, dr.scale, smem);
    } else {
        wgrad_body<P, D>(tw.blk[b], out, tw.Cp, tw.C, slice, group, ntiles, tpg, smem);
    }
}

template <int P, int D, int RCDM>
__global__ __launch_bounds__((WgradKernelGeom<P, D, RCDM>::THREADS), (WgradKernelGeom<P, D, RCDM>::MINWAVES)) void tower_wgrad_kernel(
    const m2m_tower tw, int ntiles, int tiles_per_group, int slot_mode, int rows_per_t16, unsigned int seed, unsigned int step_host,
    const unsigned int* __restrict__ step_dev, int dma) {
    extern __shared__ __attribute__((aligned(16))) char smem[];
    const unsigned int step = step_host + (step_dev ? *step_dev : 0u);
    wgrad_dispatch<P, D, RCDM>(tw, (int)blockIdx.y, (int)blockIdx.x, (int)blockIdx.z, (int)gridDim.z, slot_mode, ntiles, tiles_per_group,
                               rows_per_t16, seed, step, smem);
}

#define WG_MAX_TOWERS 4
#define WG_MAX_JOBS 32
struct WgradGroupArgs {
    const m2m_tower* tw[WG_MAX_TOWERS];
    int ntiles[WG_MAX_TOWERS], tpg[WG_MAX_TOWERS], groups[WG_MAX_TOWERS], nsl[WG_MAX_TOWERS], slot[WG_MAX_TOWERS], rpt[WG_MAX_TOWERS];
    unsigned char job_tower[WG_MAX_JOBS], job_block[WG_MAX_JOBS];
    short job_start[WG_MAX_JOBS + 1];
    short xcd_start[8], xcd_len[8];
    int njobs, n_tower_wgs;
    int dma;
    int n_embed_first, n_embed_pad;
    int n_reduce, reduce_sets;
    unsigned int seed, step_host;
    const unsigned int* step_dev;
    unsigned int* bump_counter;
};
template <int P, int D, int RCDM>
__global__ __launch_bounds__((WgradKernelGeom<P, D, RCDM>::THREADS), (WgradKernelGeom<P, D, RCDM>::MINWAVES)) void tower_wgrad_group_kernel(const WgradGroupArgs a,
                                                                                                          const EmbedWgradGroupArgs ea,
                                                                                                          const SplitReduceArgs ra) {
    extern __shared__ __attribute__((aligned(16))) char smem[];
    int id = blockIdx.x;
    if (a.bump_counter && blockIdx.x == 0 && threadIdx.x == 0) *a.bump_counter += 1u;
#ifndef M2M_WG_PROBE_TOWERS_ONLY
    if (a.n_reduce && id >= (int)gridDim.x - a.n_reduce) {
        const int rid = id - ((int)gridDim.x - a.n_reduce);
        const int bx = rid % SPR_NBX, L = (rid / SPR_NBX) % a.reduce_sets, z = rid / (SPR_NBX * a.reduce_sets);
        split_small_grads_body<WgradKernelGeom<P, D, RCDM>::THREADS>(ra.t[z], bx, L, reinterpret_cast<float*>(smem));
        return;
    }
    if (id < a.n_embed_pad) {
        if (id < a.n_embed_first) embed_wgrad_group_body<P, D, WgradKernelGeom<P, D, RCDM>::THREADS>(ea, id, smem);
        return;
    }
    id -= a.n_embed_pad;
    if (id >= a.n_tower_wgs) {
        embed_wgrad_group_body<P, D, WgradKernelGeom<P, D, RCDM>::THREADS>(ea, id - a.n_tower_wgs, smem);
        return;
    }
#endif
    const int xcd = id & 7, idx = id >> 3;
    if (idx >= a.xcd_len[xcd]) return;
    const int lin = a.xcd_start[xcd] + idx;
    int job = 0;
    while (job + 1 < a.njobs && lin >= a.job_start[job + 1]) ++job;
    const int t = a.job_tower[job], rel = lin - a.job_start[job];
    const int slice = rel % a.nsl[t], group = rel / a.nsl[t];
    const m2m_tower& tw = *a.tw[t];
    const unsigned int step = a.step_host + (a.step_dev ? *a.step_dev : 0u);
    wgrad_dispatch<P, D, RCDM>(tw, (int)a.job_block[job], slice, group, a.groups[t], a.slot[t], a.ntiles[t], a.tpg[t], a.rpt[t], a.seed,
                               step, smem);
}

static_assert(sizeof(WgradGroupArgs) + sizeof(EmbedWgradGroupArgs) + sizeof(SplitReduceArgs) <= 3840, "kernel arguments are limited to 4 KiB");

#ifdef M2M_ISA_PROBE
template __global__ void tower_wgrad_group_kernel<PREC_BF16, 128, -1>(const WgradGroupArgs, const EmbedWgradGroupArgs, const SplitReduceArgs);
template __global__ void tower_wgrad_group_kernel<PREC_BF16, 128, DM_HALF>(const WgradGroupArgs, const EmbedWgradGroupArgs, const SplitReduceArgs);
#else
template <int D>
__global__ __launch_bounds__(256, 2) void embed_wgrad_fast_group_kernel(const EmbedWgradGroupArgs ea) {
    extern __shared__ __attribute__((aligned(16))) char smem[];
    embed_wgrad_group_body<PREC_BF16, D, 256>(ea, blockIdx.x, smem);
}

bool m2m_wgrad_recompute(const m2m_tower* t, int B) {
    static const int on = m2m_env_int("M2M_WGRAD_RECOMP", 0);
    if (!on || t->prec != PREC_BF16 || t->D != 128 || t->nblocks < 1 || t->Cp < 64) return false;
    if (m2m_drop_mode(1, t->p_drop) == DM_GEN) return false;
    if (m2m_split_eligible(t, B, 1)) return false;
    return true;
}
extern "C" int m2m_wgrad_form(const m2m_tower* t, int B) { return t && m2m_wgrad_recompute(t, B) ? 1 : 0; }

static bool wgrad_slot_usable(const m2m_tower* t) {
    static const int on = m2m_env_int("M2M_WGRAD_SLOT", 1);
    if (!on || t->nblocks < 1) return false;
    for (int b = 0; b < t->nblocks; ++b) {
        const m2m_block& k = t->blk[b];
        if (!t->wslot[b]) return false;
        if (k.g_ch_b1 != k.g_ch_w1 + (long)t->C * t->D || k.g_ch_w2 != k.g_ch_b1 + t->C) return false;
    }
    return true;
}

struct WgradPlan { int ntiles, nsl, groups, tpg, rpt, slot; };
static WgradPlan wgrad_plan(const m2m_tower* t, int B, int cols, bool honour_overwrite = true) {
    const bool wide = m2m_is_wide(t);
    const int SPW = wide ? 1 : BM / t->N;
    const int nchain = wide ? (int)(((long)B * t->N + BM - 1) / BM) : (B + SPW - 1) / SPW;
    const int ntiles = (nchain * BM + WBM - 1) / WBM;
    const int nsl = (t->Cp + cols - 1) / cols;
    int groups = 1;
    const int wgs = nsl * t->nblocks;
    while (wgs * groups < 128 && (ntiles + groups - 1) / groups > 64) ++groups;
    if (groups < (32 + wgs - 1) / wgs) groups = (32 + wgs - 1) / wgs;
    groups = m2m_env_int("M2M_WGRAD_GROUPS", groups);
    if (ntiles > 64) groups = m2m_env_int("M2M_WGRAD_LONG_GROUPS", groups);
    if (honour_overwrite && (t->wgrad_flags & M2M_WGRAD_OVERWRITE)) groups = 1;
    if (groups < 1) groups = 1;
    int tpg = (ntiles + groups - 1) / groups;
    if (tpg < 4) tpg = 4;
    if (tpg > ntiles) tpg = ntiles;
    groups = (ntiles + tpg - 1) / tpg;
    WgradPlan pl;
    pl.ntiles = ntiles; pl.nsl = nsl; pl.groups = groups; pl.tpg = tpg; pl.slot = 0;
    pl.rpt = wide ? BM : SPW * t->N;
    return pl;
}
static int wgrad_cols(const m2m_tower* t, int B) {
    if (m2m_wgrad_recompute(t, B)) return RcGeom<128>::COLS;
    if (t->prec == PREC_BF16 && t->D == 128) return WgradGeom<PREC_BF16, 128>::COLS;
    return t->prec == PREC_BF16 && t->D < 128 ? WG_WAVES * 32 : WG_WAVES * 16;
}
extern "C" int m2m_wgrad_groups(const m2m_tower* t, int B) {
    if (!t || t->nblocks < 1) return 1;
    return wgrad_plan(t, B, wgrad_cols(t, B), false).groups;
}

template <int P, int D, int RCDM>
static int launch_wgrad(const m2m_tower* t, int B, unsigned int seed, unsigned int step, const unsigned int* step_dev, hipStream_t st) {
    typedef WgradKernelGeom<P, D, RCDM> KG;
    const WgradPlan pl = wgrad_plan(t, B, KG::COLS);
    const size_t lds = (size_t)KG::LDS_B;
    return m2m_launch<tower_wgrad_kernel<P, D, RCDM>>(dim3(pl.nsl, t->nblocks, pl.groups), dim3(KG::THREADS), lds, lds, st, *t, pl.ntiles, pl.tpg, 0,
                                                      pl.rpt, seed, step, step_dev, 0);
}

static void wgrad_group_plans(const m2m_tower* const* host, int n, int B, int cols, WgradPlan* pl) {
    int min_tpg = 1 << 30;
    WgradPlan nat[WG_MAX_TOWERS];
    for (int i = 0; i < n; ++i) {
        pl[i] = wgrad_plan(host[i], B, cols);
        nat[i] = wgrad_plan(host[i], B, cols, false);
        if (nat[i].tpg < min_tpg) min_tpg = nat[i].tpg;
    }
    for (int i = 0; i < n; ++i) {
        if (n < 2 || !wgrad_slot_usable(host[i])) continue;
        if (nat[i].groups == 2) { pl[i] = nat[i]; pl[i].slot = 1; }
        else if (nat[i].groups == 1 && nat[i].tpg >= 2 * min_tpg && nat[i].tpg >= 32) { pl[i] = nat[i]; pl[i].groups = 2; pl[i].tpg = (pl[i].ntiles + 1) / 2; pl[i].slot = 1; }
    }
}

template <int P, int D, int RCDM>
static int launch_wgrad_group(const m2m_tower* const* host, const m2m_tower* const* dev, int n, const m2m_embed* const* embeds,
                              const float* const* inputs, const float* const* d_x0s, const m2m_tower* const* embed_towers,
                              int nembeds, int B, unsigned int seed, unsigned int step, const unsigned int* step_dev, hipStream_t st,
                              const SplitReduceTower* heads_reduce = nullptr, unsigned int* bump_counter = nullptr) {
    typedef WgradKernelGeom<P, D, RCDM> KG;
    WgradGroupArgs a;
    memset(&a, 0, sizeof(a));
    int njobs = 0, total = 0;
    int order[WG_MAX_TOWERS];
    WgradPlan pl[WG_MAX_TOWERS];
    wgrad_group_plans(host, n, B, KG::COLS, pl);
    for (int i = 0; i < n; ++i) order[i] = i;
    for (int i = 0; i < n; ++i)
        for (int j = i + 1; j < n; ++j)
            if (pl[order[j]].tpg > pl[order[i]].tpg) { const int t = order[i]; order[i] = order[j]; order[j] = t; }
    for (int k = 0; k < n; ++k) {
        const int i = order[k];
        a.tw[i] = dev[i];
        a.ntiles[i] = pl[i].ntiles; a.tpg[i] = pl[i].tpg; a.groups[i] = pl[i].groups; a.nsl[i] = pl[i].nsl; a.slot[i] = pl[i].slot;
        a.rpt[i] = pl[i].rpt;
        for (int b = 0; b < host[i]->nblocks; ++b) {
            if (njobs >= WG_MAX_JOBS) { m2m_set_error("towers_wgrad: more than 32 (tower, block) jobs", __FILE__, __LINE__); return -1; }
            a.job_tower[njobs] = (unsigned char)i;
            a.job_block[njobs] = (unsigned char)b;
            a.job_start[njobs] = (short)total;
            total += pl[i].nsl * pl[i].groups;
            ++njobs;
        }
    }
    if (njobs == 0 && nembeds == 0) return 0;
    if (total > 32000) { m2m_set_error("towers_wgrad: too many workgroups for one launch", __FILE__, __LINE__); return -1; }
    a.job_start[njobs] = (short)total;
    int max_len = 0;
    for (int x = 0, at = 0; x < 8; ++x) {
        const int len = total / 8 + (x < total % 8 ? 1 : 0);
        a.xcd_start[x] = (short)at; a.xcd_len[x] = (short)len;
        at += len;
        if (len > max_len) max_len = len;
    }
    a.njobs = njobs; a.n_tower_wgs = 8 * max_len;
    a.seed = seed; a.step_host = step; a.step_dev = step_dev;
    a.bump_counter = bump_counter;
    a.dma = 0;
    EmbedWgradGroupArgs ea;
    memset(&ea, 0, sizeof(ea));
    int n_embed_wgs = 0;
    size_t lds_e = 0;
    bool embeds_separately = false;
    if (nembeds) {
        n_embed_wgs = (P == PREC_BF16 && nembeds == EMB_GROUP) ? embed_wgrad_group_args_fast(ea, embeds, inputs, embed_towers, B) : 0;
        if (n_embed_wgs) lds_e = embed_wgrad_fast_lds<D, KG::THREADS>();
        else if (KG::THREADS == 256) { static const int ewgs = m2m_env_int("M2M_EMBED_WGS", D >= 256 ? 128 : 512);    n_embed_wgs = embed_wgrad_group_args(ea, embeds, inputs, d_x0s, B, ewgs, nembeds); lds_e = embed_wgrad_lds<D, P>(); }
        else embeds_separately = true;
    }
    if (embeds_separately) {
        if (nembeds == 1) { if (int rc = m2m_embed_wgrad(embeds[0], inputs[0], d_x0s[0], B, (void*)st)) return rc; }
        else if (int rc = m2m_embeds_wgrad(embeds, inputs, d_x0s, nembeds, B, (void*)st)) return rc;
    }
    if constexpr (P == PREC_BF16) {
        static const int merged = m2m_env_int("M2M_EMBED_MERGED", 1);
        if (n_embed_wgs && ea.fast && !merged && KG::THREADS != 256) {
            const size_t le = embed_wgrad_fast_lds<D, 256>();
            if (int rc = m2m_launch<embed_wgrad_fast_group_kernel<D>>(dim3((unsigned)n_embed_wgs), dim3(256), le, le, st, ea)) return rc;
            n_embed_wgs = 0; lds_e = 0;
        }
    }
    const size_t lds_t = (size_t)KG::LDS_B;
    const size_t lds = lds_t > lds_e ? lds_t : lds_e;
    static const int embed_first = m2m_env_int("M2M_EMBED_FIRST", 1);
    if (ea.fast && n_embed_wgs && embed_first) { a.n_embed_first = n_embed_wgs; a.n_embed_pad = (n_embed_wgs + 7) & ~7; n_embed_wgs = 0; }
    SplitReduceArgs ra;
    memset(&ra, 0, sizeof(ra));
    for (int i = 0; i < n; ++i) {
        if (!(host[i]->wgrad_flags & M2M_WGRAD_REDUCES_SMALL)) continue;
        SplitReduceTower x;
        if (!m2m_small_part_deferred(x, host[i], B)) continue;
        if (ra.ntow < SPR_MAX_TOWERS && KG::THREADS % SPR_COLS == 0) { ra.t[ra.ntow++] = x; continue; }
        SplitReduceArgs one;
        memset(&one, 0, sizeof(one));
        one.t[0] = x; one.ntow = 1;
        if (int rc = m2m_split_small_grads(one, st)) return rc;
    }
    if (heads_reduce) {
        if (ra.ntow < SPR_MAX_TOWERS && KG::THREADS % SPR_COLS == 0) ra.t[ra.ntow++] = *heads_reduce;
        else {
            SplitReduceArgs one;
            memset(&one, 0, sizeof(one));
            one.t[0] = *heads_reduce; one.ntow = 1;
            if (int rc = m2m_split_small_grads(one, st)) return rc;
        }
    }
    for (int i = 0; i < ra.ntow; ++i) a.reduce_sets = ra.t[i].nlaunch > a.reduce_sets ? ra.t[i].nlaunch : a.reduce_sets;
    a.n_reduce = SPR_NBX * a.reduce_sets * ra.ntow;
    return m2m_launch<tower_wgrad_group_kernel<P, D, RCDM>>(dim3((unsigned)(a.n_embed_pad + a.n_tower_wgs + n_embed_wgs + a.n_reduce)), dim3(KG::THREADS),
                                                            lds, lds, st, a, ea, ra);
}

extern "C" int m2m_wgrad_slot_groups(const m2m_tower* const* towers, int ntowers, int B) {
    if (!towers || ntowers < 1 || ntowers > WG_MAX_TOWERS) return 0;
    WgradPlan pl[WG_MAX_TOWERS];
    wgrad_group_plans(towers, ntowers, B, wgrad_cols(towers[0], B), pl);
    int bits = 0;
    for (int i = 0; i < ntowers; ++i) bits |= pl[i].slot << i;
    return bits;
}

extern "C" int m2m_tower_wgrad(const m2m_tower* t, int B, uint32_t seed, uint32_t step, const uint32_t* step_dev, void* stream) {
    if (int rc = m2m_check_tower(t, B)) return rc;
    if (t->nblocks == 0) return 0;
    hipStream_t st = reinterpret_cast<hipStream_t>(stream);
    if (t->wgrad_flags & M2M_WGRAD_REDUCES_SMALL) {
        SplitReduceArgs one;
        memset(&one, 0, sizeof(one));
        if (m2m_small_part_deferred(one.t[0], t, B)) {
            one.ntow = 1;
            if (int rc = m2m_split_small_grads(one, st)) return rc;
        }
    }
    if (m2m_wgrad_recompute(t, B))
        return m2m_dispatch<DM_NONE, DM_HALF>(m2m_drop_mode(1, t->p_drop), -1, [&](auto DM) { return launch_wgrad<PREC_BF16, 128, DM()>(t, B, seed, step, step_dev, st); });
    const int rc = m2m_dispatch_pd(m2m_wide_dims{}, t->prec, t->D, [&](auto P, auto D) { return launch_wgrad<P(), D(), -1>(t, B, seed, step, step_dev, st); });
    if (rc != M2M_NO_BUILD) return rc;
    m2m_set_error("tower_wgrad: unsupported (prec, D)", __FILE__, __LINE__);
    return -1;
}

static int towers_wgrad_impl(const m2m_tower* const* towers, const m2m_tower* const* dev_towers, int ntowers,
                             const m2m_embed* const* embeds, const float* const* inputs, const float* const* d_x0s,
                             const m2m_tower* const* embed_towers, int nembeds,
                             int B, uint32_t seed, uint32_t step, const uint32_t* step_dev,
                             const m2m_head* heads, int nheads, int K, void* stream, uint32_t* bump_counter = nullptr) {
    SplitReduceTower hr;
    const SplitReduceTower* heads_reduce = nullptr;
    if (heads && nheads > 0) {
        if (nheads > 3 || K < 2 || !towers || ntowers < 1 || !towers[0]) { m2m_set_error("towers_wgrad_heads: 1..3 heads, K >= 2", __FILE__, __LINE__); return -1; }
        const int D = towers[0]->D, tiles = m2m_heads_part_tiles(B);
        if ((long)K * D + K + 2 > SPP_STRIDE) { m2m_set_error("towers_wgrad_heads: K*D + K + 2 exceeds the slot", __FILE__, __LINE__); return -1; }
        memset(&hr, 0, sizeof(hr));
        for (int h = 0; h < nheads; ++h) {
            if (!heads[h].g_part || !heads[h].g_w || !heads[h].g_b || heads[h].g_part != heads[0].g_part + (long)h * tiles * SPP_STRIDE) {
                m2m_set_error("towers_wgrad_heads: every head needs g_w, g_b and consecutive g_part buffers", __FILE__, __LINE__);
                return -1;
            }
            hr.g_hw[h] = heads[h].g_w; hr.g_hb[h] = heads[h].g_b;
        }
        hr.part = heads[0].g_part; hr.ntiles = tiles; hr.nlaunch = nheads; hr.D = D; hr.head_set0 = 0; hr.nheads = nheads; hr.K = K;
        hr.losses = nullptr;
        heads_reduce = &hr;
    }
    if (!towers || !dev_towers || ntowers < 1 || ntowers > WG_MAX_TOWERS) { m2m_set_error("towers_wgrad: 1..4 towers", __FILE__, __LINE__); return -1; }
    if (nembeds != 0 && (nembeds < 1 || nembeds > EMB_GROUP || !embeds || !inputs || !d_x0s)) {
        m2m_set_error("towers_wgrad: at most two patch embeddings", __FILE__, __LINE__);
        return -1;
    }
    for (int i = 0; i < ntowers; ++i) {
        if (int rc = m2m_check_tower(towers[i], B)) return rc;
        if (!dev_towers[i]) { m2m_set_error("towers_wgrad: missing device-resident descriptor", __FILE__, __LINE__); return -1; }
        if (towers[i]->prec != towers[0]->prec || towers[i]->D != towers[0]->D) {
            m2m_set_error("towers_wgrad: the towers of one launch must share precision and hidden_dim", __FILE__, __LINE__);
            return -1;
        }
        if (m2m_wgrad_recompute(towers[i], B) != m2m_wgrad_recompute(towers[0], B) ||
            (m2m_wgrad_recompute(towers[0], B) && m2m_drop_mode(1, towers[i]->p_drop) != m2m_drop_mode(1, towers[0]->p_drop))) {
            m2m_set_error("towers_wgrad: the towers of one launch must share the weight-gradient form and the dropout mode", __FILE__, __LINE__);
            return -1;
        }
    }
    for (int i = 0; i < nembeds; ++i) {
        if (int rc = m2m_check_embed(embeds[i], B)) return rc;
        if (!inputs[i] || !d_x0s[i]) { m2m_set_error("towers_wgrad: null embedding input", __FILE__, __LINE__); return -1; }
        if (embeds[i]->prec != towers[0]->prec || embeds[i]->D != towers[0]->D) {
            m2m_set_error("towers_wgrad: embeddings must share the towers' precision and hidden_dim", __FILE__, __LINE__);
            return -1;
        }
    }
    hipStream_t st = reinterpret_cast<hipStream_t>(stream);
    const m2m_tower* t = towers[0];
    if (bump_counter && m2m_wgrad_recompute(t, B)) {
        m2m_set_error("towers_wgrad_tail: the recompute form READS the dropout counter in this launch; advance it with m2m_counter_add", __FILE__, __LINE__);
        return -1;
    }
    if (m2m_wgrad_recompute(t, B))
        return m2m_dispatch<DM_NONE, DM_HALF>(m2m_drop_mode(1, t->p_drop), -1, [&](auto DM) {
            return launch_wgrad_group<PREC_BF16, 128, DM()>(towers, dev_towers, ntowers, embeds, inputs, d_x0s, embed_towers, nembeds, B, seed, step, step_dev, st, heads_reduce);
        });
    const int rc = m2m_dispatch_pd(m2m_wide_dims{}, t->prec, t->D, [&](auto P, auto D) {
        return launch_wgrad_group<P(), D(), -1>(towers, dev_towers, ntowers, embeds, inputs, d_x0s, embed_towers, nembeds, B, seed, step, step_dev, st, heads_reduce, bump_counter);
    });
    if (rc != M2M_NO_BUILD) return rc;
    m2m_set_error("towers_wgrad: unsupported (prec, D)", __FILE__, __LINE__);
    return -1;
}

extern "C" int m2m_towers_wgrad(const m2m_tower* const* towers, const m2m_tower* const* dev_towers, int ntowers,
                                const m2m_embed* const* embeds, const float* const* inputs, const float* const* d_x0s,
                                const m2m_tower* const* embed_towers, int nembeds,
                                int B, uint32_t seed, uint32_t step, const uint32_t* step_dev, void* stream) {
    return towers_wgrad_impl(towers, dev_towers, ntowers, embeds, inputs, d_x0s, embed_towers, nembeds, B, seed, step, step_dev, nullptr, 0, 0, stream);
}
extern "C" int m2m_towers_wgrad_heads(const m2m_tower* const* towers, const m2m_tower* const* dev_towers, int ntowers,
                                      const m2m_embed* const* embeds, const float* const* inputs, const float* const* d_x0s,
                                      const m2m_tower* const* embed_towers, int nembeds,
                                      int B, uint32_t seed, uint32_t step, const uint32_t* step_dev,
                                      const m2m_head* heads, int nheads, int K, void* stream) {
    return towers_wgrad_impl(towers, dev_towers, ntowers, embeds, inputs, d_x0s, embed_towers, nembeds, B, seed, step, step_dev, heads, nheads, K, stream);
}

extern "C" int m2m_towers_wgrad_tail(const m2m_tower* const* towers, const m2m_tower* const* dev_towers, int ntowers,
                                     const m2m_embed* const* embeds, const float* const* inputs, const float* const* d_x0s,
                                     const m2m_tower* const* embed_towers, int nembeds,
                                     int B, uint32_t seed, uint32_t step, const uint32_t* step_dev,
                                     const m2m_head* heads, int nheads, int K, uint32_t* bump_counter, void* stream) {
    return towers_wgrad_impl(towers, dev_towers, ntowers, embeds, inputs, d_x0s, embed_towers, nembeds, B, seed, step, step_dev, heads, nheads, K, stream, bump_counter);
}

extern "C" int m2m_embeds_wgrad_form(const m2m_embed* const* embeds, const m2m_tower* const* embed_towers, int nembeds, int B) {
    if (!embeds || !embed_towers || nembeds != EMB_GROUP) return 0;
    EmbedWgradGroupArgs ea;
    const float* ins[EMB_GROUP] = {nullptr, nullptr};
    return embed_wgrad_group_args_fast(ea, embeds, ins, embed_towers, B) > 0 ? 1 : 0;
}

__global__ void wgrad_fold_kernel(float* __restrict__ g, const float* __restrict__ s, long n) {
    const long stride = (long)gridDim.x * blockDim.x;
    for (long i = (long)blockIdx.x * blockDim.x + threadIdx.x; i < n; i += stride) g[i] += s[i];
}
extern "C" int m2m_wgrad_fold(const m2m_tower* t, void* stream) {
    if (!t) { m2m_set_error("wgrad_fold: null tower", __FILE__, __LINE__); return -1; }
    if (!wgrad_slot_usable(t)) { m2m_set_error("wgrad_fold: channel gradients are not contiguous", __FILE__, __LINE__); return -1; }
    hipStream_t st = reinterpret_cast<hipStream_t>(stream);
    const long n = 2L * t->C * t->D + t->C;
    for (int b = 0; b < t->nblocks; ++b) {
        if (int rc = m2m_launch<wgrad_fold_kernel>(dim3(512), dim3(256), 0, 0, st, t->blk[b].g_ch_w1, t->wslot[b], n)) return rc;
    }
    return 0;
}
#endif
```

### m2_mixer_amd/data.py

```python
from __future__ import annotations

import os
from typing import Dict, Iterator, Optional, Tuple

import numpy as np
import torch


class ResidentAVMnist:

    TRAIN_SPLIT = 55000

    def __init__(self, root_dir: str, device="cuda:0", rank: int = 0, world: int = 1):
        self.device = torch.device(device)
        self.rank, self.world = rank, world
        self.splits: Dict[str, Tuple[torch.Tensor, torch.Tensor, torch.Tensor]] = {}
        tr = self._load(root_dir, "train")
        n = tr[2].shape[0]
        cut = self.TRAIN_SPLIT if n > self.TRAIN_SPLIT else (n * 11) // 12
        self.splits["train"] = tuple(t[:cut] for t in tr)
        self.splits["val"] = tuple(t[cut:] for t in tr)
        if os.path.exists(os.path.join(root_dir, "test_labels.npy")):
            self.splits["test"] = self._load(root_dir, "test")

    def _load(self, root: str, stage: str):
        image = np.load(os.path.join(root, "image", f"{stage}_data.npy"))
        audio = np.load(os.path.join(root, "audio", f"{stage}_data.npy"))
        labels = np.load(os.path.join(root, f"{stage}_labels.npy"))
        if image.shape[0] != audio.shape[0] or image.shape[0] != labels.shape[0]:
            raise ValueError(f"{stage}: image / audio / label counts differ")
        image = torch.from_numpy(image.astype(np.float32)).reshape(image.shape[0], 1, 28, 28)
        audio = torch.from_numpy(audio.astype(np.float32))[:, None, :, :]
        labels = torch.from_numpy(labels.astype(np.int64))
        return image.to(self.device), audio.to(self.device), labels.to(self.device)

    def num_samples(self, split: str) -> int:
        n = self.splits[split][2].shape[0]
        return (n + self.world - 1) // self.world

    def num_batches(self, split: str, batch_size: int, drop_last: bool = False) -> int:
        n = self.num_samples(split)
        return n // batch_size if drop_last else (n + batch_size - 1) // batch_size

    def batches(self, split: str, batch_size: int, shuffle: bool = False, generator: Optional[torch.Generator] = None,
                drop_last: bool = False) -> Iterator[Tuple[torch.Tensor, torch.Tensor, torch.Tensor]]:
        image, audio, labels = self.splits[split]
        n = labels.shape[0]
        if shuffle:
            order = torch.randperm(n, device=self.device, generator=generator)
        elif self.world > 1:
            order = torch.arange(n, device=self.device)
        else:
            order = None
        if order is not None and self.world > 1:
            pad = self.num_samples(split) * self.world - n
            if pad:
                order = torch.cat([order, order[:pad]])
            order = order[self.rank::self.world]
        mine = self.num_samples(split)
        for b in range(self.num_batches(split, batch_size, drop_last)):
            lo, hi = b * batch_size, min((b + 1) * batch_size, mine)
            if order is None:
                yield image[lo:hi], audio[lo:hi], labels[lo:hi]
            else:
                idx = order[lo:hi]
                yield image.index_select(0, idx), audio.index_select(0, idx), labels.index_select(0, idx)


class PlateauLR:

    def __init__(self, engine, lr: float, patience: int = 5, factor: float = 0.1, threshold: float = 1e-4, min_lr: float = 0.0):
        self.engine, self.lr, self.patience, self.factor, self.threshold, self.min_lr = engine, lr, patience, factor, threshold, min_lr
        self.best, self.bad = float("inf"), 0

    def step(self, metric: float) -> float:
        if metric < self.best * (1 - self.threshold):
            self.best, self.bad = metric, 0
        else:
            self.bad += 1
        if self.bad > self.patience:
            self.lr = max(self.lr * self.factor, self.min_lr)
            self.engine.set_lr(self.lr)
            self.bad = 0
        return self.lr


def prepare_tail_engine(engine, data: "ResidentAVMnist", split: str, batch_size: int):
    rem = data.num_samples(split) % batch_size
    if rem == 0:
        return None
    if rem not in engine._tail_engines:
        engine._tail_engines[rem] = engine.sibling(rem)
    return engine._tail_engines[rem]


def run_epoch(engine, data: ResidentAVMnist, split: str, batch_size: int, train: bool, log_interval_steps: int = 50,
              replay=None, log=None, tail_engine=None, grad_sync=None, epoch: int = 0, shuffle_seed: int = 0) -> Dict[str, float]:
    dev = engine.device
    table = None
    if getattr(engine, "scores", None) is not None:
        table = engine.score_table("train" if train else (split if split != "train" else "train_eval"))
    if table is not None:
        table.reset()
    acc = torch.zeros(11, device=dev, dtype=torch.float64)
    seen, host = 0, np.zeros(11)
    if train and grad_sync is None and getattr(data, "world", 1) > 1:
        raise RuntimeError("run_epoch: world > 1 needs the gradient exchange (grad_sync=parallel.GradSync(...))")
    nb = data.num_batches(split, batch_size)
    shuffle, gen = split == "test", None
    if shuffle and getattr(data, "world", 1) > 1:
        gen = torch.Generator(device=data.device)
        gen.manual_seed(int(shuffle_seed) + int(epoch))
    for i, (image, audio, labels) in enumerate(data.batches(split, batch_size, shuffle=shuffle, generator=gen)):
        bs = labels.shape[0]
        eng = engine
        if bs != batch_size:
            if tail_engine is None:
                tail_engine = engine._tail_engines.get(bs)
            if tail_engine is None:
                tail_engine = engine.sibling(bs, trains=train)
                if train:
                    engine._tail_engines[bs] = tail_engine
            eng = tail_engine
            eng.pack()
            image, audio, labels = image.contiguous(), audio.contiguous(), labels.contiguous()
        if train:
            if replay is not None and eng is engine:
                replay(image, audio, labels)
            else:
                eng.train_step(image, audio, labels, grad_sync=grad_sync)
        else:
            eng.evaluate(image, audio, labels, **({} if table is None else {"scores": table}))
        if eng is not engine and train:
            engine.pack()
        acc[:4] += eng.losses
        acc[4:8] += eng.losses * bs
        acc[8:11] += (eng.preds == labels.to(eng.preds.dtype)[None, :]).sum(dim=1)
        seen += bs
        if (i + 1) % log_interval_steps == 0 or i + 1 == nb:
            host = acc.cpu().numpy()
            if log is not None:
                log({"split": split, "step": i + 1, "loss": host[3] / (i + 1), "acc": host[10] / seen})
    steps, n = max(nb, 1), max(seen, 1)
    a, b = getattr(engine, "MODS", ("image", "audio"))
    out = {} if table is None else table.compute()
    out.update({"loss": float(host[7]) / n, "loss_step_mean": float(host[3]) / steps,
            f"loss_{a}": float(host[0]) / steps, f"loss_{b}": float(host[1]) / steps, "loss_fusion": float(host[2]) / steps,
            "acc": float(host[10]) / n, f"acc_{a}": float(host[8]) / n, f"acc_{b}": float(host[9]) / n,
            "hits": int(round(host[10])), f"hits_{a}": int(round(host[8])), f"hits_{b}": int(round(host[9])),
            "steps": nb, "samples": seen})
    return out
```

### m2_mixer_amd/engine.py

```python
from __future__ import annotations

from collections import OrderedDict
from typing import Dict, List, Optional, Sequence, Tuple

import ctypes as C

import torch

from . import _lib as L
from . import config
from .runtime import (AdamPackPlan, BLOCK_FIELDS, BLOCK_KEYS, EmbedRuntime, MlpRuntime, TowerRuntime, block_param_shapes, heads_bce,
                      heads_ce, can_group, can_group_embeds, can_pack_all, embeds_forward, pack_all,
                      towers_backward, towers_forward, towers_forward_embeds_ok, towers_wgrad, wgrad_slot_groups,
                      _embed_ptrs, _grad_ranges, _tower_ptrs)


def config_fused_update(n_params: int = 0) -> bool:
    env = config.switch("M2M_FUSED_UPDATE")
    if env is not None:
        return env == "1"
    return n_params > 0


def _num_patch(c: dict) -> int:
# ... 386 lines not shown
                               "that the sibling's backward would not overwrite; build training siblings before capture() "
                               "(or capture again afterwards)")
        for eng, other in ((self, theirs), (sib, mine)):
            eng._ranges_add = [(lo, n, v, int(k and lo in other)) for lo, n, v, k in eng._ranges_add]
        return sib

    def _check_grad_bf16(self, grad_bf16: Optional[torch.Tensor]):
        if grad_bf16 is not None and (grad_bf16.dtype != torch.bfloat16 or grad_bf16.numel() != self.n_params or not grad_bf16.is_cuda):
            raise RuntimeError("grad_bf16 must be a bf16 device copy of the whole flat gradient")

    def _adam(self, lo: int, hi: int, scale: float, grad_bf16: Optional[torch.Tensor] = None, ranges=None):
        self._check_grad_bf16(grad_bf16)
        n = hi - lo
        p, g, m, v = (t.data_ptr() + lo * 4 for t in (self.flat_p, self.flat_g, self.flat_m, self.flat_v))
        g16 = 0 if grad_bf16 is None else grad_bf16.data_ptr() + lo * 2
        tail = (self.adam_state.data_ptr(), self.betas[0], self.betas[1], self.eps, self.weight_decay, -abs(scale), 0)
        if ranges:
            L.check(L.lib().m2m_adam_step_ranges(p, g, g16, m, v, n, *tail, _grad_ranges(ranges), len(ranges), L.stream_ptr()),
                    "adam_step_ranges")
        elif grad_bf16 is None:
            L.check(L.lib().m2m_adam_step(p, g, m, v, n, *tail, L.stream_ptr()), "adam_step")
        else:
            L.check(L.lib().m2m_adam_step_bf16(p, g, g16, m, v, n, *tail, L.stream_ptr()), "adam_step_bf16")

    def _prologue(self):
        L.check(L.lib().m2m_step_prologue(self.adam_state.data_ptr(), self.drop_step.data_ptr(), self.losses.data_ptr(), 4,
                                          L.stream_ptr()), "step_prologue")

    def forward_backward(self, *batch):
        self._step(batch, fused_update=False)
        for t in self._slot_towers:
            t.wgrad_fold()
        self._slots_folded = True

    def fused_step(self, *batch):
        self._step(batch, fused_update=True)
        return self.losses

    def _step(self, batch, fused_update: bool):
        self._check_trains()
        self._slots_folded = False
        self._forward(*batch, training=True, with_grad=True, prologue=True)
        self._score_forward(batch[-1])
        self._backward(*batch[:-1], fused_update=fused_update)
        self._score_backward(batch[-1])

    def new_score_table(self) -> ScoreTable:
        return ScoreTable(self.SCORES_TASK, self.HEAD_NAMES, self.K, self.device)

    def score_table(self, split: str) -> ScoreTable:
        if split == "train":
            if self.scores is None:
                raise RuntimeError("score_table('train'): this engine was built with scores=False")
            return self.scores
        tables = self.__dict__.setdefault("_split_scores", {})
        if split not in tables:
            tables[split] = self.new_score_table()
        return tables[split]

    def _preds_in_forward(self) -> bool:
        return not self._fused_heads

    def _score_forward(self, truth):
        if self.scores is not None and self._preds_in_forward():
            self.scores.add(self.preds, truth)

    def _score_backward(self, truth):
        if self.scores is not None and not self._preds_in_forward():
            self.scores.add(self.preds, truth)

    def _check_trains(self):
        if self._eval_only:
            raise RuntimeError("this engine was built with sibling(..., trains=False): it only evaluates")

    def pack(self):
        if can_pack_all(self._towers, self._embeds):
            pack_all(self._towers, self._embeds)
            return
        for m in self._towers + self._embeds:
            m.pack(force=True)

    def _adam_pack_modules(self):
        return (self._towers, self._embeds) if can_pack_all(self._towers, self._embeds) else None

    def _update(self, grad_scale: float = 1.0, grad_bf16: Optional[torch.Tensor] = None):
        mods = self._adam_pack_modules() if self._fused_update else None
        ranges = self._ranges_keep if (self._slots_folded or grad_bf16 is not None) else self._ranges_add
        self._slots_folded = False
        if mods is None:
            self._adam(0, self.n_params, grad_scale, grad_bf16, ranges)
            self.pack()
            return
        key = (abs(float(grad_scale)), 0 if grad_bf16 is None else grad_bf16.data_ptr(), tuple((lo, n, 0 if v is None else v.data_ptr(), k) for lo, n, v, k in ranges))
        plan = self._adam_plans.get(key)
        if plan is None:
            self._check_grad_bf16(grad_bf16)
            plan = AdamPackPlan(mods[0], mods[1], self.flat_p, self.flat_g, grad_bf16, self.flat_m, self.flat_v, self.adam_state,
                                self.betas, self.eps, self.weight_decay, grad_scale, ranges)
            self._adam_plans[key] = plan
        plan.run()

    def optimizer_step(self, grad_scale: float = 1.0, grad_bf16: Optional[torch.Tensor] = None):
        self._update(grad_scale, grad_bf16)

    def train_step(self, *batch, grad_sync=None):
        self._run_step(grad_sync, *self._phases(batch, grad_sync))
        return self.losses

    def _run_step(self, grad_sync, first, update) -> float:
        mode = _exchange_mode(grad_sync)
        first()
        if mode == "none":
            return 1.0
        if mode == "single":
            scale = grad_sync(self.flat_g)
            update(0, scale)
            return scale
        chunks = self._update_chunks()
        scale = grad_sync.start(self.flat_g, [(lo, hi) for lo, hi, _ in chunks])
        for k in range(len(chunks)):
            grad_sync.wait(k)
            update(k, scale)
        self._slots_folded = False
        return scale

    def _phases(self, batch, grad_sync):
        mode = _exchange_mode(grad_sync)
        if mode == "none":
            return (lambda: self.fused_step(*batch)), None
        if mode == "single":
            return (lambda: self.forward_backward(*batch)), (lambda k, scale: self.optimizer_step(scale, getattr(grad_sync, "reduced_bf16", None)))
        return (lambda: self.forward_backward(*batch)), self._update_one_chunk

    def _update_chunks(self):
        return [(0, self.n_params, None)]

    def _adam_chunk(self, lo: int, hi: int, scale: float):
        ranges = []
        for rlo, rn, _, keep in self._ranges_keep:
            a, b = max(rlo, lo), min(rlo + rn, hi)
            if a < b:
                ranges.append((a - lo, b - a, None, keep))
        self._adam(lo, hi, scale, None, ranges)

    def _update_one_chunk(self, k: int, scale: float):
        lo, hi, mods = self._update_chunks()[k]
        self._adam_chunk(lo, hi, scale)
        if mods is None:
            self.pack()
        else:
            for m in mods:
                m.pack(force=True)

    def release_capture(self):
        self._graph = None
        self._static = None

    def capture(self, *batch, grad_sync=None, steps: int = 1):
        if steps < 1 or (steps > 1 and grad_sync is not None):
            raise ValueError("steps > 1 is only supported without a gradient exchange")
        nb = len(batch)
        slots = [tuple(t.clone() for t in batch) for _ in range(steps)]
        if steps > 1 and config.switch_on("M2M_CAPTURE_SHARE_SLOTS"):
            slots = [slots[0]] * steps
        self._static = slots[0] if steps == 1 else slots
        st = slots[0]
        state = [self.flat_p, self.flat_m, self.flat_v, self.flat_g, self.adam_state, self.drop_step]
        if self.scores is not None:
            state.append(self.scores.table)
        snap = [t.clone() for t in state]
        s = torch.cuda.Stream(device=self.device)
        s.wait_stream(torch.cuda.current_stream())
        with torch.cuda.stream(s):
            first, update = self._phases(st, grad_sync)
            for _ in range(2):
                scale = self._run_step(grad_sync, first, update)
        torch.cuda.current_stream().wait_stream(s)
        torch.cuda.synchronize()
        for dst, src in zip(state, snap):
            dst.copy_(src)
        self.pack()
        torch.cuda.synchronize()

        def graph_of(fn):
            g = torch.cuda.CUDAGraph()
            with torch.cuda.graph(g, capture_error_mode="thread_local"):
                fn()
            return g

        out_losses = self.losses
        if steps > 1:
            home = (self.losses, self.logits, self.preds)
            self.losses_steps = torch.zeros(steps, *self.losses.shape, device=self.device)
            self.logits_steps = torch.zeros(steps, *self.logits.shape, device=self.device)
            self.preds_steps = torch.zeros(steps, *self.preds.shape, dtype=self.preds.dtype, device=self.device)
            out_losses = self.losses_steps

            def all_steps():
                for i in range(steps):
                    self.losses, self.logits, self.preds = self.losses_steps[i], self.logits_steps[i], self.preds_steps[i]
                    self.fused_step(*slots[i])

            first = all_steps
        nupd = {"none": 0, "single": 1, "pipelined": len(self._update_chunks())}[_exchange_mode(grad_sync)]
        graphs = (graph_of(first), *[graph_of(lambda k=k: update(k, scale)) for k in range(nupd)])
        if steps > 1:
            self.losses, self.logits, self.preds = home
        self._slots_folded = False
        self._graph = graphs

        def replay(*new_batch):
            if new_batch and new_batch[0] is not None:
                if len(new_batch) != nb * steps:
                    raise ValueError(f"replay expects {nb * steps} tensors ({steps} step(s) x {nb}), got {len(new_batch)}")
                for i in range(steps):
                    for dst, src in zip(slots[i], new_batch[i * nb:(i + 1) * nb]):
                        dst.copy_(src, non_blocking=True)
            self._run_step(grad_sync, graphs[0].replay, lambda k, scale: graphs[1 + k].replay())
            return out_losses

        replay.losses = out_losses
        return replay


class _TwoTowerEngine(_FlatEngine):

    MODS: Tuple[str, str] = ("image", "audio")

    def _param_shapes(self, cfg):
        return two_tower_param_shapes(cfg, self.MODS)

    def _segment_of(self, k: str) -> str:
        a, b = self.MODS
        return a if k.startswith(f"{a}_mixer.") else (b if k.startswith(f"{b}_mixer.") else "fusion")

    def _build(self):
        a, b = self.MODS
        cfg = self.cfg
        ca, cb, cm = cfg[a], cfg[b], cfg["multimodal"]
        self.D = ca["hidden_dim"]
        self.fusion_name = fusion_function_name(cm)
        self.concat = self.fusion_name == "ConcatFusion"
        if not (cb["hidden_dim"] == self.D == cm["hidden_dim"]):
            raise RuntimeError(f"both towers and the fusion mixer must share hidden_dim ({self.fusion_name} on dim 1)")
        if self.fusion_name == "BiModalGatedUnit" and not (cm["mod1_in"] == cm["mod2_in"] == cm["out_size"] == self.D):
            raise RuntimeError(f"multimodal.mod1_in / mod2_in / out_size = {cm['mod1_in']} / {cm['mod2_in']} / {cm['out_size']}: "
                               f"the engine's BiModalGatedUnit takes and gives the towers' hidden_dim {self.D} (one D for the heads)")
        self.Na, self.Nb = _num_patch(ca), _num_patch(cb)
        self.Nf = fusion_tokens(cm, self.Na, self.Nb)
        self.t_a = self._make_tower(f"{a}_mixer.", ca, self.Na, 0)
        self.t_b = self._make_tower(f"{b}_mixer.", cb, self.Nb, 1024)
        self.t_fus = self._make_tower("fusion_mixer.", cm, self.Nf, 2048)

        def make_embed(prefix, c):
            e = EmbedRuntime(c["in_channels"], c["image_size"][0], c["image_size"][1], c["patch_size"], c["patch_size"],
                             self.D, self.prec)
            e.bind_params(self.params[prefix + "to_patch_embedding.0.weight"], self.params[prefix + "to_patch_embedding.0.bias"])
            e.bind_grads(self.grads[prefix + "to_patch_embedding.0.weight"], self.grads[prefix + "to_patch_embedding.0.bias"])
            return e

        self.e_a = make_embed(f"{a}_mixer.", ca)
        self.e_b = make_embed(f"{b}_mixer.", cb)
        self._towers, self._embeds = [self.t_a, self.t_b, self.t_fus], [self.e_a, self.e_b]
        B, D, dev = self.B, self.D, self.device
        f = lambda *s: torch.zeros(*s, device=dev)
        grouped = can_group_embeds(self.e_a, self.e_b) and can_group(self.t_a, self.t_b, self.B)
        self.x0_splits = (self.e_a.fwd_splits(), self.e_b.fwd_splits()) if grouped and not self.t_a.wide else (1, 1)
        self._x0_a, self._x0_b = f(self.x0_splits[0], B * self.Na, D), f(self.x0_splits[1], B * self.Nb, D)
        self.x0_a, self.x0_b = self._x0_a[0], self._x0_b[0]
        self.fused, self.fus_out = f(B, self.Nf, D), f(B, self.Nf, D)
        self.pool_a, self.pool_b, self.pool_fus = f(B, D), f(B, D), f(B, D)
        self.dpool_a, self.dpool_b, self.dpool_fus = f(B, D), f(B, D), f(B, D)
        self.d_fused = f(B, self.Nf, D)
        self.dx0_a, self.dx0_b = f(B * self.Na, D), f(B * self.Nb, D)
        self._build_fusion()
        self.preds = torch.zeros(self._preds_shape(), dtype=torch.int32, device=dev)
        self._early_fus_wgrad = (self.concurrent and self.t_fus.wide and B * self.Nf <= 8192 and
                                 config.switch_on("M2M_EARLY_FUSION_WGRAD"))
        self._setup_wgrad([[self.t_fus], [self.t_a, self.t_b]] if self._early_fus_wgrad else [[self.t_fus, self.t_a, self.t_b]])
        self._fused_heads = self._heads_are_ce() and self.t_fus.backward_heads_ok(B, 3, self.K)
        self._heads_pool = (self.t_a.wide and self.t_b.wide and self.t_fus.wide and config.switch_on("M2M_HEADS_POOL"))
        self.t_fus.set_wgrad_reduces_small(not self._fused_heads and config.switch_on("M2M_DEFER_SMALL"))
        self._head_part, self._wgrad_heads = None, None
        if (self._heads_are_ce() and not self._fused_heads and config.switch_on("M2M_HEAD_SLOTS")
                and self.K * D + self.K + 2 <= L.SPLIT_GPART):
            self._head_part = torch.zeros(3, int(L.lib().m2m_heads_part_tiles(B)), L.SPLIT_GPART, device=dev)
        if (config.switch_on("M2M_GROUP_SLOTS") and self.t_a.has_small_slots() and self.t_b.has_small_slots()
                and can_group(self.t_a, self.t_b, self.B)):
            for t in (self.t_a, self.t_b):
                t.set_wgrad_group_slots(True)
                t.set_wgrad_reduces_small(True)
        self._embed_towers = []
        if config.switch_on("M2M_EMBED_FAST") and self.t_a.enable_dx0_image(B) and self.t_b.enable_dx0_image(B):
            self._embed_towers = [self.t_a, self.t_b]
            fast = bool(L.lib().m2m_embeds_wgrad_form(_embed_ptrs(self._embeds), _tower_ptrs(self._embed_towers), 2, B))
            if fast and config.switch_on("M2M_WGRAD_OVERWRITE") and len(self._ranges_add) + 2 <= L.MAX_GRAD_RANGES:
                for e, pre in ((self.e_a, f"{a}_mixer."), (self.e_b, f"{b}_mixer.")):
                    gw = self.grads[pre + "to_patch_embedding.0.weight"]
                    e.set_wgrad_overwrite(True)
                    self._ranges_add.append(((gw.data_ptr() - self.flat_g.data_ptr()) // 4, gw.numel(), None, 1))
                self._ranges_add.sort(key=lambda r: r[0])

        self._embed_fold = (config.switch_on("M2M_EMBED_FOLD") and grouped and self.concurrent and not self._early_fus_wgrad
                            and self.x0_splits is not None and self.e_a.prec == self.t_a.prec and self.e_a.D == self.t_a.D
                            and towers_forward_embeds_ok([self.t_a, self.t_b], [self.e_a, self.e_b], B)
                            and self.t_a.wgrad_form(B) == 0 and self.t_fus.wgrad_form(B) == 0)
        self._pending_bump = False

    def _build_fusion(self):
        B, D, dev = self.B, self.D, self.device
        self.out_a = self.out_b = self.d_out_a = self.d_out_b = None
        self.gate = None
        if self.concat:
            return
        f = lambda *s: torch.zeros(*s, device=dev)
        self.out_a, self.out_b = f(B, self.Na, D), f(B, self.Nb, D)
        if self.fusion_name == "SumFusion":
            self.d_out_a = self.d_out_b = self.d_fused
        else:
            self.d_out_a, self.d_out_b = f(B, self.Na, D), f(B, self.Nb, D)
        if self.fusion_name != "BiModalGatedUnit":
            return
        rows = B * self.Nf
        self._gate_bufs = dict(t1=f(rows, D), t2=f(rows, D), z=f(rows, D), dh=f(rows, 3 * D),
                               part=f(int(L.lib().m2m_gate_part_floats(rows, D))))
        g = L.Gate()
        g.D = D
        P, G = self.params, self.grads
        for fld, key in (("w1", "mod1_hidden.weight"), ("b1", "mod1_hidden.bias"), ("w2", "mod2_hidden.weight"),
                         ("b2", "mod2_hidden.bias"), ("wz", "z_hidden.weight"), ("bz", "z_hidden.bias")):
            setattr(g, fld, P["fusion_function." + key].data_ptr())
            setattr(g, "g_" + fld, G["fusion_function." + key].data_ptr())
        for fld, t in self._gate_bufs.items():
            setattr(g, fld, t.data_ptr())
        self.gate = g

    def _tower_outputs(self):
        D = self.D
        if self.concat:
            return self.fused, self.fused.view(-1)[self.Na * D:], self.Nf * D
        return self.out_a, self.out_b, None

    def _fusion_forward(self, training: bool):
        rows = self.B * self.Nf
        if self.concat:
            return
        if self.gate is not None:
            L.check(L.lib().m2m_gate_forward(C.byref(self.gate), self.out_a.data_ptr(), self.out_b.data_ptr(), self.fused.data_ptr(),
                                             rows, int(training), L.stream_ptr()), "gate_forward")
        else:
            L.check(L.lib().m2m_fusion_forward(_ELEM_FUSION_MODE[self.fusion_name], self.out_a.data_ptr(), self.out_b.data_ptr(),
                                               self.fused.data_ptr(), rows * self.D, L.stream_ptr()), "fusion_forward")

    def _fusion_backward(self):
        rows = self.B * self.Nf
        if self.concat or self.fusion_name == "SumFusion":
            return
        if self.gate is not None:
            L.check(L.lib().m2m_gate_backward(C.byref(self.gate), self.d_fused.data_ptr(), self.d_out_a.data_ptr(),
                                              self.d_out_b.data_ptr(), rows, L.stream_ptr()), "gate_backward")
            L.check(L.lib().m2m_gate_wgrad(C.byref(self.gate), self.out_a.data_ptr(), self.out_b.data_ptr(), rows, L.stream_ptr()),
                    "gate_wgrad")
        else:
            L.check(L.lib().m2m_fusion_backward(_ELEM_FUSION_MODE[self.fusion_name], self.out_a.data_ptr(), self.out_b.data_ptr(),
                                                self.d_fused.data_ptr(), self.d_out_a.data_ptr(), self.d_out_b.data_ptr(),
                                                rows * self.D, L.stream_ptr()), "fusion_backward")

    def _preds_shape(self):
        return (3, self.B)

    def _loss_heads(self, heads, labels, zero_losses):
        raise NotImplementedError

    def _heads_are_ce(self) -> bool:
        return False

    def _forward(self, xa, xb, labels, training: bool, with_grad: bool, prologue: bool = False):
        B, D = self.B, self.D
        sd = self.drop_step if training else None
        fs = self.Nf * D
        out_a, b_part, ts = self._tower_outputs()
        sa_, sb_ = (ts, ts) if self.concat else (self.Na * D, self.Nb * D)
        main, side, _ = self._streams()
        so = 0
        pa, pb, pf = (None, None, None) if self._heads_pool else (self.pool_a, self.pool_b, self.pool_fus)
        self._pending_bump = False
        if self._embed_fold and training and prologue:
            so, self._pending_bump = 1, True
            towers_forward([self.t_a, self.t_b],
                           [(self.x0_a, self.Na * D, out_a, sa_, pa), (self.x0_b, self.Nb * D, b_part, sb_, pb)],
                           B, training, self.seed, so, sd, embeds=[self.e_a, self.e_b], inputs=[xa, xb],
                           head=(self.adam_state, self.losses))
        elif self.concurrent and can_group(self.t_a, self.t_b, self.B):
            sa, sb = self.x0_splits
            if can_group_embeds(self.e_a, self.e_b):
                head = (self.adam_state, self.drop_step, self.losses) if prologue else None
                embeds_forward([self.e_a, self.e_b], [xa, xb], [self._x0_a, self._x0_b], B, [sa, sb], head)
            else:
                if prologue:
                    self._prologue()
                sa = sb = 1
                self.e_a.forward(xa, B, self.x0_a)
                self.e_b.forward(xb, B, self.x0_b)
            towers_forward([self.t_a, self.t_b],
                           [(self.x0_a, self.Na * D, out_a, sa_, pa, sa, B * self.Na * D),
                            (self.x0_b, self.Nb * D, b_part, sb_, pb, sb, B * self.Nb * D)],
                           B, training, self.seed, 0, sd)
        else:
            if prologue:
                self._prologue()
            side.wait_stream(main)
            with torch.cuda.stream(side):
                self.e_b.forward(xb, B, self.x0_b)
                self.t_b.forward(self.x0_b, self.Nb * D, B, b_part, sb_, pb, training, self.seed, 0, sd)
            self.e_a.forward(xa, B, self.x0_a)
            self.t_a.forward(self.x0_a, self.Na * D, B, out_a, sa_, pa, training, self.seed, 0, sd)
            main.wait_stream(side)
        self._fusion_forward(training and with_grad)
        self.t_fus.forward(self.fused, fs, B, self.fus_out, fs, pf, training, self.seed, so, sd)
        a, b = self.MODS
        hw = self.head_weights
        heads = [self._head(a, self.pool_a, self.dpool_a, hw[a], with_grad),
                 self._head(b, self.pool_b, self.dpool_b, hw[b], with_grad),
                 self._head("fusion", self.pool_fus, self.dpool_fus, hw["fusion"], with_grad)]
        if self._heads_pool:
            heads[0]["tokens"] = (out_a, self.Na, sa_)
            heads[1]["tokens"] = (b_part.data_ptr(), self.Nb, sb_)
            heads[2]["tokens"] = (self.fus_out, self.Nf, fs)
        self._wgrad_heads = None
        if training and with_grad and self._head_part is not None:
            for i, h in enumerate(heads):
                h["g_part"] = self._head_part[i]
            self._wgrad_heads = heads
        self._heads = heads
        self._labels = labels
        if training and with_grad and self._fused_heads:
            return
        self._loss_heads(heads, labels, not training)

    def _backward(self, xa, xb, fused_update: bool = False):
        B, D = self.B, self.D
        fs = self.Nf * D
        sd = self.drop_step
        a, b = self.MODS
        so = 1 if self._pending_bump else 0
        if self._fused_heads:
            self.t_fus.backward_heads(B, self._heads, 2, self._labels, self.K, (self.logits, self.losses, self.preds),
                                      self.d_fused, fs, self.seed, so, sd)
        else:
            self.t_fus.backward(B, None, 0, self.dpool_fus, self.d_fused, fs, self.seed, so, sd)
        if self.concat:
            d_a_part, d_b_part, sa_, sb_ = self.d_fused, self.d_fused.view(-1)[self.Na * D:], fs, fs
        else:
            self._fusion_backward()
            d_a_part, d_b_part, sa_, sb_ = self.d_out_a, self.d_out_b, self.Na * D, self.Nb * D
        main, s_a, s_f = self._streams()
        wg_towers = [self.t_fus, self.t_a, self.t_b]
        if self._early_fus_wgrad:
            s_f.wait_stream(main)
            with torch.cuda.stream(s_f):
# ... 268 lines not shown
```

### m2_mixer_amd/runtime.py

```python
from __future__ import annotations

import ctypes as C
from typing import Dict, List, Optional, Sequence

import torch

from . import _lib as L

BLOCK_KEYS = {
    "ln1_w": "token_mix.0.weight", "ln1_b": "token_mix.0.bias",
    "tok_w1": "token_mix.2.net.0.weight", "tok_b1": "token_mix.2.net.0.bias",
    "tok_w2": "token_mix.2.net.3.weight", "tok_b2": "token_mix.2.net.3.bias",
    "ln2_w": "channel_mix.0.weight", "ln2_b": "channel_mix.0.bias",
    "ch_w1": "channel_mix.1.net.0.weight", "ch_b1": "channel_mix.1.net.0.bias",
    "ch_w2": "channel_mix.1.net.3.weight", "ch_b2": "channel_mix.1.net.3.bias",
}
BLOCK_FIELDS = list(BLOCK_KEYS.keys())


def block_param_shapes(D: int, N: int, T: int, Cc: int) -> Dict[str, tuple]:
    return {"ln1_w": (D,), "ln1_b": (D,), "tok_w1": (T, N), "tok_b1": (T,), "tok_w2": (N, T), "tok_b2": (N,),
            "ln2_w": (D,), "ln2_b": (D,), "ch_w1": (Cc, D), "ch_b1": (Cc,), "ch_w2": (D, Cc), "ch_b2": (D,)}


def _check_tensor(t: torch.Tensor, shape, name: str):
    if not t.is_cuda:
        raise RuntimeError(f"{name}: m2_mixer_amd runs on the GPU only (got a {t.device} tensor); "
                           "there is no CPU path -- the CPU restatement under oracle/ is test infrastructure")
    if t.dtype != torch.float32 or not t.is_contiguous() or tuple(t.shape) != tuple(shape):
        raise RuntimeError(f"{name}: expected contiguous float32 {tuple(shape)}, got {t.dtype} {tuple(t.shape)}")


def _tower_ptrs(towers):
    return (C.POINTER(L.Tower) * max(len(towers), 1))(*[C.pointer(t.desc) for t in towers])


def _embed_ptrs(embeds):
    return (C.POINTER(L.Embed) * max(len(embeds), 1))(*[C.pointer(e.desc) for e in embeds])


def _data_ptrs(tensors):
    return (C.c_void_p * max(len(tensors), 1))(*[t.data_ptr() for t in tensors])


def _device_descs(towers):
    return (C.c_void_p * max(len(towers), 1))(*[t.device_desc() for t in towers])


def _grad_ranges(ranges):
    arr = (L.GradRange * max(len(ranges), 1))()
    for i, (lo, n, add, keep) in enumerate(ranges):
        arr[i].lo, arr[i].n, arr[i].add, arr[i].keep = lo, n, L.ptr(add), int(keep)
    return arr


def _step_head(adam_state, losses, drop_counter=None):
    return C.byref(L.StepHead(L.ptr(adam_state), L.ptr(drop_counter), L.ptr(losses), int(losses.numel())))


def _drop_tail(seed: int, step: int, step_dev: Optional[torch.Tensor] = None):
    return seed & 0xFFFFFFFF, step & 0xFFFFFFFF, L.ptr(step_dev), L.stream_ptr()


class TowerRuntime:

    def __init__(self, D: int, N: int, T: int, Cc: int, nblocks: int, has_final_ln: bool, p_drop: float,
                 prec: int, site_base: int = 0):
        if nblocks > L.MAX_BLOCKS:
            raise RuntimeError(f"one m2m_tower holds at most {L.MAX_BLOCKS} blocks; deeper towers are a chain of them "
                               "(modules/mixer.py does that; the fused engines take towers of up to 8 blocks)")
        self.D, self.N, self.T, self.C, self.nblocks = D, N, T, Cc, nblocks
        self.Cp = (Cc + 31) // 32 * 32
        self.prec = prec
        self.has_final_ln = bool(has_final_ln)
        self.desc = L.Tower()
        d = self.desc
        d.prec, d.D, d.N, d.T, d.C, d.Cp = prec, D, N, T, Cc, self.Cp
        d.nblocks, d.has_final_ln = nblocks, int(self.has_final_ln)
        d.p_drop = float(p_drop)
        d.site_base = site_base
        self._keep: Dict[str, object] = {}
        self._param_ptrs: List[int] = []
        self._param_versions: List[int] = []
        self._packed_for: Optional[List[int]] = None
        self._bufB = 0
        self._wsB = 0
        self._splitB = 0
        self.device = None
        self.wide = N > 8 or D > 128

    def bind_params(self, blocks: Sequence[Dict[str, torch.Tensor]], lnf: Optional[Sequence[torch.Tensor]]):
        shapes = block_param_shapes(self.D, self.N, self.T, self.C)
        ptrs, vers = [], []
        for i, bp in enumerate(blocks):
            for f in BLOCK_FIELDS:
                t = bp[f]
                _check_tensor(t, shapes[f], f"block {i} {BLOCK_KEYS[f]}")
                setattr(self.desc.blk[i], f, t.data_ptr())
                ptrs.append(t.data_ptr())
                vers.append(t._version)
            self._keep[f"params{i}"] = dict(bp)
        if self.has_final_ln:
            for t, f in zip(lnf, ("lnf_w", "lnf_b")):
                _check_tensor(t, (self.D,), f"layer_norm {f}")
                setattr(self.desc, f, t.data_ptr())
                ptrs.append(t.data_ptr())
                vers.append(t._version)
            self._keep["lnf"] = tuple(lnf)
        self.device = blocks[0]["ln1_w"].device if blocks else lnf[0].device
        self._param_ptrs, self._param_versions = ptrs, vers
        self._packed_for = None
        self._ensure_packed_buffers()

    def params_changed(self, blocks, lnf) -> bool:
        ptrs = [bp[f].data_ptr() for bp in blocks for f in BLOCK_FIELDS]
        if self.has_final_ln:
            ptrs += [lnf[0].data_ptr(), lnf[1].data_ptr()]
        return ptrs != self._param_ptrs

    def _ensure_packed_buffers(self):
        if "packed0" in self._keep or self.nblocks == 0:
            return
        nb = L.packed_bytes(self.prec, self.Cp, self.D)
        for i in range(self.nblocks):
            bufs = {k: torch.zeros(nb, dtype=torch.uint8, device=self.device) for k in ("w1n", "w2c", "w2tn", "w1tc")}
            bufs["ch_b1p"] = torch.zeros(self.Cp, dtype=torch.float32, device=self.device)
            for k, v in bufs.items():
                setattr(self.desc.blk[i], k, v.data_ptr())
            self._keep[f"packed{i}"] = bufs

    def _pack_versions(self):
        cur = []
        for i in range(self.nblocks):
            bp = self._keep[f"params{i}"]
            cur += [bp["ch_w1"]._version, bp["ch_w2"]._version, bp["ch_b1"]._version]
        return cur

    def pack_all_skips_w1tc(self) -> bool:
        return bool(L.lib().m2m_pack_skips_w1tc(C.byref(self.desc)))

    def mark_packed(self):
        self._packed_for = self._pack_versions()

    def invalidate(self):
        self._packed_for = None

    def pack(self, force: bool = False):
        if force or self._pack_versions() != self._packed_for:
            L.check(L.lib().m2m_pack_tower(C.byref(self.desc), L.stream_ptr()), "pack_tower")
            self.mark_packed()

    def ensure_buffers(self, B: int):
        if B == self._bufB:
            return
        if self.wide:
            ntiles = (B * self.N + L.ROWS_PER_WG - 1) // L.ROWS_PER_WG
        else:
            spw = L.ROWS_PER_WG // self.N
            ntiles = (B + spw - 1) // spw
        esz = 2 if self.prec == L.PREC_BF16 else 4
        npairs = (ntiles * L.ROWS_PER_WG + 31) // 32
        img = npairs * 32 * self.D * esz
        M = B * self.N
        for i in range(self.nblocks):
            bufs = {"x_in": torch.empty(M, self.D, device=self.device), "x_mid": torch.empty(M, self.D, device=self.device)}
            for k in ("at_chn", "dyt_chn"):
                bufs[k] = torch.zeros(img, dtype=torch.uint8, device=self.device)
            for k in ("h_chn", "dh_chn"):
                bufs[k] = torch.zeros((self.Cp // 16) * (npairs * 2048 + L.HCHN_PAD), dtype=torch.uint8, device=self.device)
            for k, v in bufs.items():
                setattr(self.desc.blk[i], k, v.data_ptr())
            self._keep[f"saved{i}"] = bufs
        xf = torch.empty(M, self.D, device=self.device)
        self.desc.x_final = xf.data_ptr()
        self._keep["x_final"] = xf
        if self._keep.get("want_dx0_image"):
            img0 = torch.zeros(img, dtype=torch.uint8, device=self.device)
            self.desc.dx0_chn = img0.data_ptr()
            self._keep["dx0_chn"] = img0
        self._bufB = B

    def fresh_saved(self, B: int) -> dict:
        self.ensure_buffers(B)
        M = B * self.N
        f = lambda: torch.empty(M, self.D, device=self.device)
        saved = {"B": B, "x_in": [f() for _ in range(self.nblocks)], "x_mid": [f() for _ in range(self.nblocks)], "x_final": f()}
        if "split" in self._keep and self._splitB == B:
            sp = self._keep["split"]
            saved["a_nat"] = [torch.zeros_like(t) for t in sp["a_nat"]]
            saved["at_chn"] = [torch.zeros_like(self._keep[f"saved{i}"]["at_chn"]) for i in range(self.nblocks)]
        self.use_saved(saved)
        return saved

    def use_saved(self, saved: dict):
        for i in range(self.nblocks):
# ... 75 lines not shown
                 d_x0: torch.Tensor, d_x0_ss: int, seed: int, step: int, step_dev: Optional[torch.Tensor] = None):
        L.check(L.lib().m2m_tower_backward(C.byref(self.desc), B, L.ptr(d_out), d_out_ss, L.ptr(d_pooled),
                                           d_x0.data_ptr(), d_x0_ss, *_drop_tail(seed, step, step_dev)), "tower_backward")

    def enable_dx0_image(self, B: int) -> bool:
        if self.wide or self.prec != L.PREC_BF16 or self.nblocks == 0:
            return False
        self._keep["want_dx0_image"] = True
        self._bufB = 0
        self.ensure_buffers(B)
        return True

    def wgrad_form(self, B: int) -> int:
        return int(L.lib().m2m_wgrad_form(C.byref(self.desc), B))

    def wgrad_groups(self, B: int) -> int:
        return int(L.lib().m2m_wgrad_groups(C.byref(self.desc), B))

    def channel_grad_ranges(self, flat_g: torch.Tensor):
        out = []
        cd = self.C * self.D
        base, end = flat_g.data_ptr(), flat_g.data_ptr() + flat_g.numel() * 4
        for i in range(self.nblocks):
            b = self.desc.blk[i]
            w1, b1, w2 = b.g_ch_w1, b.g_ch_b1, b.g_ch_w2
            if not w1 or b1 != w1 + 4 * cd or w2 != b1 + 4 * self.C or w1 < base or w2 + 4 * cd > end:
                return None
            out.append(((w1 - base) // 4, 2 * cd + self.C))
        return out

    def alloc_wslot(self, flat_g: torch.Tensor) -> bool:
        rng = self.channel_grad_ranges(flat_g)
        if rng is None or self.nblocks == 0:
            return False
        n = rng[0][1]
        buf = torch.zeros(self.nblocks * (n + 8), device=self.device)
        views = []
        off = 0
        for i, (lo, _) in enumerate(rng):
            while (off - lo) % 4:
                off += 1
            v = buf[off:off + n]
            self.desc.wslot[i] = v.data_ptr()
            views.append(v)
            off += n
        self._keep["wslot"] = (buf, views)
        return True

    def clear_wslot(self):
        for i in range(L.MAX_BLOCKS):
            self.desc.wslot[i] = None
        self._keep.pop("wslot", None)

    def wslot_views(self):
        return self._keep["wslot"][1] if "wslot" in self._keep else None

    def set_wgrad_overwrite(self, on: bool):
        self.desc.wgrad_flags = (self.desc.wgrad_flags | L.WGRAD_OVERWRITE) if on else (self.desc.wgrad_flags & ~L.WGRAD_OVERWRITE)

    def set_wgrad_reduces_small(self, on: bool):
        self.desc.wgrad_flags = (self.desc.wgrad_flags | L.WGRAD_REDUCES_SMALL) if on else (self.desc.wgrad_flags & ~L.WGRAD_REDUCES_SMALL)

    def has_small_slots(self) -> bool:
        return (not self.wide and self.prec == L.PREC_BF16 and self.D == 128 and self.nblocks > 0
                and 2 * self.T * self.N + self.T + self.N <= 576)

    def set_wgrad_group_slots(self, on: bool):
        self.desc.wgrad_flags = (self.desc.wgrad_flags | L.WGRAD_GROUP_SLOTS) if on else (self.desc.wgrad_flags & ~L.WGRAD_GROUP_SLOTS)

    def wgrad_fold(self):
        L.check(L.lib().m2m_wgrad_fold(C.byref(self.desc), L.stream_ptr()), "wgrad_fold")

    def backward_heads_ok(self, B: int, nheads: int, K: int) -> bool:
        return bool(L.lib().m2m_tower_backward_heads_ok(C.byref(self.desc), B, nheads, K))

    def backward_heads(self, B: int, heads: Sequence[dict], own: int, labels: torch.Tensor, K: int, out, d_x0: torch.Tensor,
                       d_x0_ss: int, seed: int, step: int, step_dev: Optional[torch.Tensor] = None):
        arr = _head_array(heads)
        logits, losses, preds = out
        L.check(L.lib().m2m_tower_backward_heads(C.byref(self.desc), B, arr, len(heads), own, labels.data_ptr(), K, logits.data_ptr(),
                                                 losses.data_ptr(), preds.data_ptr(), d_x0.data_ptr(), d_x0_ss,
                                                 *_drop_tail(seed, step, step_dev)), "tower_backward_heads")

    def wgrad(self, B: int, seed: int, step: int, step_dev: Optional[torch.Tensor] = None):
        L.check(L.lib().m2m_tower_wgrad(C.byref(self.desc), B, *_drop_tail(seed, step, step_dev)), "tower_wgrad")

    def device_desc(self) -> int:
        raw = bytes(self.desc)
        if self._keep.get("desc_bytes") != raw:
            self._keep["desc_dev"] = torch.frombuffer(bytearray(raw), dtype=torch.uint8).to(self.device)
            self._keep["desc_bytes"] = raw
        return self._keep["desc_dev"].data_ptr()

    def dropout_mask(self, blk: int, site: int, B: int, seed: int, step: int) -> torch.Tensor:
        n = {0: B * self.D * self.T, 1: B * self.D * self.N, 2: B * self.N * self.Cp, 3: B * self.N * self.D}[site]
        m = torch.empty(n, dtype=torch.uint8, device=self.device)
        L.check(L.lib().m2m_dropout_mask(C.byref(self.desc), blk, site, B, *_drop_tail(seed, step)[:2], m.data_ptr(), L.stream_ptr()),
                "dropout_mask")
        return m


def can_group(a: TowerRuntime, b: TowerRuntime, B: Optional[int] = None) -> bool:
    if B is not None:
        return bool(L.lib().m2m_towers_can_group(C.byref(a.desc), C.byref(b.desc), B))
    return (not a.wide and not b.wide and a.prec == b.prec and a.D == b.D and a.desc.p_drop == b.desc.p_drop
            and (a.N <= 4) == (b.N <= 4) and (a.T % 16 == 0) == (b.T % 16 == 0) and a.nblocks <= 4 and b.nblocks <= 4)


def towers_forward_embeds_ok(towers: Sequence[TowerRuntime], embeds: Sequence["EmbedRuntime"], B: int) -> bool:
    return bool(L.lib().m2m_towers_forward_embeds_ok(_tower_ptrs(towers), len(towers), _embed_ptrs(embeds), B))


def towers_forward(towers: Sequence[TowerRuntime], ios: Sequence[tuple], B: int, training: bool, seed: int, step: int,
                   step_dev: Optional[torch.Tensor] = None, embeds: Sequence["EmbedRuntime"] = (), inputs: Sequence[torch.Tensor] = (),
                   head: Optional[tuple] = None):
    n = len(towers)
    for t in towers:
        if training:
            t.ensure_buffers(B)
        t.ensure_workspace(B)
    host = _tower_ptrs(towers)
    io = (L.TowerIO * n)()
    for i, (x0, x0_ss, out, out_ss, pooled, *parts) in enumerate(ios):
        io[i].x0, io[i].x0_ss, io[i].out, io[i].out_ss, io[i].pooled = x0.data_ptr(), x0_ss, out.data_ptr(), out_ss, L.ptr(pooled)
        io[i].x0_parts, io[i].x0_part_stride = parts if parts else (1, 0)
    if len(embeds):
        hd = _step_head(*head) if head is not None else None
        L.check(L.lib().m2m_towers_forward_embeds(host, io, n, _embed_ptrs(embeds), _data_ptrs(inputs), hd, B, int(training),
                                                  *_drop_tail(seed, step, step_dev)), "towers_forward_embeds")
        return
    L.check(L.lib().m2m_towers_forward(host, io, n, B, int(training), *_drop_tail(seed, step, step_dev)), "towers_forward")


def towers_backward(towers: Sequence[TowerRuntime], ios: Sequence[tuple], B: int, seed: int, step: int,
                    step_dev: Optional[torch.Tensor] = None):
    n = len(towers)
    io = (L.TowerGIO * n)()
    for i, (d_out, d_out_ss, d_pooled, d_x0, d_x0_ss) in enumerate(ios):
        io[i].d_out, io[i].d_out_ss, io[i].d_pooled = L.ptr(d_out), d_out_ss, L.ptr(d_pooled)
        io[i].d_x0, io[i].d_x0_ss = d_x0.data_ptr(), d_x0_ss
    L.check(L.lib().m2m_towers_backward(_tower_ptrs(towers), io, n, B, *_drop_tail(seed, step, step_dev)), "towers_backward")


def wgrad_slot_groups(towers: Sequence[TowerRuntime], B: int) -> int:
    return int(L.lib().m2m_wgrad_slot_groups(_tower_ptrs(towers), len(towers), B))


def towers_wgrad(towers: Sequence[TowerRuntime], B: int, embeds: Sequence["EmbedRuntime"] = (),
                 inputs: Sequence[torch.Tensor] = (), d_x0s: Sequence[torch.Tensor] = (), seed: int = 0, step: int = 0,
                 step_dev: Optional[torch.Tensor] = None, embed_towers: Sequence[TowerRuntime] = (),
                 heads: Optional[Sequence[dict]] = None, K: int = 0, bump: Optional[torch.Tensor] = None):
    n, ne = len(towers), len(embeds)
    et = _tower_ptrs(embed_towers) if len(embed_towers) == ne and ne else None
    args = (_tower_ptrs(towers), _device_descs(towers), n, _embed_ptrs(embeds), _data_ptrs(inputs), _data_ptrs(d_x0s), et, ne, B,
            *_drop_tail(seed, step, step_dev)[:3])
    if bump is not None:
        L.check(L.lib().m2m_towers_wgrad_tail(*args, _head_array(heads) if heads else None, len(heads) if heads else 0, K,
                                              bump.data_ptr(), L.stream_ptr()), "towers_wgrad_tail")
        return
    if heads:
        L.check(L.lib().m2m_towers_wgrad_heads(*args, _head_array(heads), len(heads), K, L.stream_ptr()), "towers_wgrad_heads")
        return
    L.check(L.lib().m2m_towers_wgrad(*args, L.stream_ptr()), "towers_wgrad")


def can_pack_all(towers: Sequence[TowerRuntime], embeds: Sequence["EmbedRuntime"]) -> bool:
    precs = {t.prec for t in towers} | {e.prec for e in embeds}
    return len(towers) <= 3 and len(embeds) <= 2 and len(precs) == 1 and all(t.nblocks <= 4 for t in towers)


def pack_all(towers: Sequence[TowerRuntime], embeds: Sequence["EmbedRuntime"]):
    L.check(L.lib().m2m_pack_all(_tower_ptrs(towers), len(towers), _embed_ptrs(embeds), len(embeds), L.stream_ptr()), "pack_all")
    for t in towers:
        t.mark_packed()
    for e in embeds:
        e.mark_packed()


class AdamPackPlan:

    def __init__(self, towers: Sequence[TowerRuntime], embeds: Sequence["EmbedRuntime"], flat_p, flat_g, grad_bf16, flat_m, flat_v,
                 state, betas, eps: float, weight_decay: float, grad_scale: float, ranges=None):
        self.towers, self.embeds = list(towers), list(embeds)
        nt, ne = len(towers), len(embeds)
        self._tp, self._ep = _tower_ptrs(towers), _embed_ptrs(embeds)
        nbytes = int(L.lib().m2m_adam_pack_plan_bytes())
        self.host = C.create_string_buffer(nbytes)
        ranges = list(ranges or [])
        L.check(L.lib().m2m_adam_pack_plan_ranges(self._tp, nt, self._ep, ne, flat_p.data_ptr(), flat_g.data_ptr(), L.ptr(grad_bf16),
                                                  flat_m.data_ptr(), flat_v.data_ptr(), flat_p.numel(), state.data_ptr(), betas[0], betas[1],
                                                  eps, weight_decay, abs(grad_scale), _grad_ranges(ranges), len(ranges), self.host),
                "adam_pack_plan_ranges")
        self.dev = torch.frombuffer(bytearray(self.host.raw), dtype=torch.uint8).to(flat_p.device)
        self._keep = (flat_p, flat_g, grad_bf16, flat_m, flat_v, state, [r[2] for r in ranges])

    def run(self):
        L.check(L.lib().m2m_adam_pack_all(self._tp, len(self.towers), self._ep, len(self.embeds), self.dev.data_ptr(), self.host,
                                          L.stream_ptr()), "adam_pack_all")
        for t in self.towers:
            t.mark_packed()
        for e in self.embeds:
            e.mark_packed()


class EmbedRuntime:

    def __init__(self, Cin: int, H: int, W: int, ph: int, pw: int, D: int, prec: int):
        self.desc = L.Embed()
        d = self.desc
        kb = 32 if prec == L.PREC_BF16 else 16
        K = Cin * ph * pw
        d.prec, d.Cin, d.H, d.W, d.ph, d.pw, d.D, d.K = prec, Cin, H, W, ph, pw, D, K
        d.Kp = (K + kb - 1) // kb * kb
        self.N = (H // ph) * (W // pw)
        self.D, self.K, self.prec = D, K, prec
        self._keep = {}
        self._packed_for = None

    def bind_params(self, w: torch.Tensor, b: torch.Tensor):
        if not w.is_cuda:
            raise RuntimeError("patch embedding: m2_mixer_amd runs on the GPU only; there is no CPU path")
        if w.dtype != torch.float32 or not w.is_contiguous() or w.numel() != self.D * self.K:
            raise RuntimeError(f"embedding weight: expected contiguous float32 with {self.D * self.K} elements")
        self.desc.w, self.desc.b = w.data_ptr(), b.data_ptr()
        self._keep["w"], self._keep["b"] = w, b
        self._packed_for = None
        if "wn" not in self._keep:
            wn = torch.zeros(L.packed_bytes(self.prec, self.D, self.desc.Kp), dtype=torch.uint8, device=w.device)
            self.desc.wn = wn.data_ptr()
            self._keep["wn"] = wn

    def params_changed(self, w, b) -> bool:
        return w.data_ptr() != self.desc.w or b.data_ptr() != self.desc.b

    def mark_packed(self):
        self._packed_for = self._keep["w"]._version

    def invalidate(self):
        self._packed_for = None

    def pack(self, force: bool = False):
        if force or self._keep["w"]._version != self._packed_for:
            L.check(L.lib().m2m_pack_embed(C.byref(self.desc), L.stream_ptr()), "pack_embed")
            self.mark_packed()

    def bind_grads(self, g_w: torch.Tensor, g_b: torch.Tensor):
        self.desc.g_w, self.desc.g_b = g_w.data_ptr(), g_b.data_ptr()
        self._keep["g"] = (g_w, g_b)

    def set_wgrad_overwrite(self, on: bool):
        self.desc.wgrad_flags = L.WGRAD_OVERWRITE if on else 0

    def fwd_splits(self) -> int:
        return int(L.lib().m2m_embed_fwd_splits(C.byref(self.desc)))

    def forward(self, inp: torch.Tensor, B: int, x0: torch.Tensor, step_head: Optional[tuple] = None):
        head = _step_head(step_head[0], step_head[2], step_head[1]) if step_head is not None else None
        L.check(L.lib().m2m_embed_forward_head(C.byref(self.desc), inp.data_ptr(), B, x0.data_ptr(), head, L.stream_ptr()),
                "embed_forward")

    def wgrad(self, inp: torch.Tensor, d_x0: torch.Tensor, B: int):
        L.check(L.lib().m2m_embed_wgrad(C.byref(self.desc), inp.data_ptr(), d_x0.data_ptr(), B, L.stream_ptr()),
                "embed_wgrad")


def can_group_embeds(a: EmbedRuntime, b: EmbedRuntime) -> bool:
    return a.prec == b.prec and a.D == b.D


def embeds_forward(embeds: Sequence[EmbedRuntime], inputs: Sequence[torch.Tensor], x0s: Sequence[torch.Tensor], B: int,
                   nsplits: Optional[Sequence[int]] = None, step_head: Optional[tuple] = None):
    n = len(embeds)
    ns = (C.c_int * n)(*(nsplits if nsplits is not None else [1] * n))
    ps = (C.c_int64 * n)(*[B * e.N * e.D for e in embeds])
    head = _step_head(step_head[0], step_head[2], step_head[1]) if step_head is not None else None
    L.check(L.lib().m2m_embeds_forward(_embed_ptrs(embeds), _data_ptrs(inputs), _data_ptrs(x0s), ns, ps, n, B, head, L.stream_ptr()),
            "embeds_forward")


def embeds_wgrad(embeds: Sequence[EmbedRuntime], inputs: Sequence[torch.Tensor], d_x0s: Sequence[torch.Tensor], B: int):
    L.check(L.lib().m2m_embeds_wgrad(_embed_ptrs(embeds), _data_ptrs(inputs), _data_ptrs(d_x0s), len(embeds), B, L.stream_ptr()),
            "embeds_wgrad")


class MlpRuntime:

    def __init__(self, dims: Sequence[int], has_out: bool, p_drop: float, site_base: int = 0):
        nl = len(dims) - 1
        if nl < 1 or nl > L.MLP_MAX_LAYERS:
            raise RuntimeError(f"MLP: 1..{L.MLP_MAX_LAYERS} Linear layers supported, got {nl}")
        self.dims, self.nlayers, self.has_out = list(dims), nl, bool(has_out)
        self.desc = L.Mlp()
        d = self.desc
        d.nlayers, d.has_out, d.p_drop, d.site_base = nl, int(self.has_out), float(p_drop), site_base
        for i, w in enumerate(dims):
            d.dims[i] = int(w)
        self._keep: Dict[str, object] = {}
        self._B = 0

    def bind(self, params: Sequence[tuple], grads: Optional[Sequence[tuple]], B: int):
        for i, (w, b) in enumerate(params):
            _check_tensor(w, (self.dims[i + 1], self.dims[i]), f"mlp layer {i} weight")
            _check_tensor(b, (self.dims[i + 1],), f"mlp layer {i} bias")
            self.desc.w[i], self.desc.b[i] = w.data_ptr(), b.data_ptr()
        if grads is not None:
            for i, (gw, gb) in enumerate(grads):
                self.desc.g_w[i], self.desc.g_b[i] = gw.data_ptr(), gb.data_ptr()
        self._keep["params"], self._keep["grads"] = list(params), grads
        self.ensure_buffers(B, params[0][0].device)

    def ensure_buffers(self, B: int, device):
        if B == self._B:
            return
        self.use_acts([torch.zeros(B, self.dims[i + 1], device=device) for i in range(self.nlayers)])
        self._B = B

    def fresh_acts(self, B: int, device) -> list:
        acts = [torch.zeros(B, self.dims[i + 1], device=device) for i in range(self.nlayers)]
        self.use_acts(acts)
        self._B = B
        return acts

    def use_acts(self, acts: list):
        for i, a in enumerate(acts):
            self.desc.act[i] = a.data_ptr()
        self._keep["act"] = acts

    def forward(self, x: torch.Tensor, B: int, out: torch.Tensor, out_ss: int, out_dense: Optional[torch.Tensor],
                training: bool, seed: int, step: int, step_dev: Optional[torch.Tensor] = None):
        _check_tensor(x, (B, self.dims[0]), "mlp input")
        self.ensure_buffers(B, x.device)
        L.check(L.lib().m2m_mlp_forward(C.byref(self.desc), x.data_ptr(), B, out.data_ptr(), out_ss, L.ptr(out_dense),
                                        int(training), *_drop_tail(seed, step, step_dev)), "mlp_forward")

    def backward(self, x: torch.Tensor, B: int, d_out: Optional[torch.Tensor], d_out_ss: int,
                 d_out_dense: Optional[torch.Tensor]):
        L.check(L.lib().m2m_mlp_backward(C.byref(self.desc), x.data_ptr(), B, L.ptr(d_out), d_out_ss, L.ptr(d_out_dense),
                                         L.stream_ptr()), "mlp_backward")

    def forward_ride(self, x: torch.Tensor, B: int, out: torch.Tensor, out_ss: int, out_dense: Optional[torch.Tensor],
                     training: bool, seed: int, step: int, step_dev: Optional[torch.Tensor] = None):
        _check_tensor(x, (B, self.dims[0]), "mlp input")
        self.ensure_buffers(B, x.device)
        L.check(L.lib().m2m_mlp_forward_ride(C.byref(self.desc), x.data_ptr(), B, out.data_ptr(), out_ss, L.ptr(out_dense),
                                             int(training), *_drop_tail(seed, step, step_dev)[:3]), "mlp_forward_ride")

    def backward_ride(self, x: torch.Tensor, B: int, d_out: Optional[torch.Tensor], d_out_ss: int,
                      d_out_dense: Optional[torch.Tensor]):
        L.check(L.lib().m2m_mlp_backward_ride(C.byref(self.desc), x.data_ptr(), B, L.ptr(d_out), d_out_ss, L.ptr(d_out_dense)),
                "mlp_backward_ride")

    @staticmethod
    def ride_flush():
        L.check(L.lib().m2m_mlp_ride_flush(L.stream_ptr()), "mlp_ride_flush")


def _head_array(heads: Sequence[dict]):
    nh = len(heads)
    arr = (L.Head * nh)()
    for i, h in enumerate(heads):
        arr[i].pooled, arr[i].w, arr[i].b = L.ptr(h.get("pooled")), h["w"].data_ptr(), h["b"].data_ptr()
        tok = h.get("tokens")
        if tok is not None:
            arr[i].tokens = tok[0] if isinstance(tok[0], int) else tok[0].data_ptr()
            arr[i].ntok, arr[i].tok_sample_stride = int(tok[1]), int(tok[2])
        elif h.get("pooled") is None:
            raise ValueError("a head needs `pooled` or `tokens`")
        arr[i].g_w, arr[i].g_b, arr[i].d_pooled = L.ptr(h.get("g_w")), L.ptr(h.get("g_b")), L.ptr(h.get("d_pooled"))
        arr[i].weight = float(h["weight"])
        arr[i].g_part = L.ptr(h.get("g_part"))
    return arr


def _check_weights(weights: Optional[torch.Tensor], nh: int):
    if weights is not None and (not weights.is_cuda or weights.dtype != torch.float32 or weights.numel() < nh
                                or not weights.is_contiguous()):
        raise ValueError(f"head weights: a contiguous float32 device tensor of at least {nh} entries")


def heads_bce(heads: Sequence[dict], targets: torch.Tensor, pos_weight: torch.Tensor, B: int, D: int, K: int, out=None,
              zero_losses: bool = True, weights: Optional[torch.Tensor] = None):
    nh = len(heads)
    _check_weights(weights, nh)
    arr = _head_array(heads)
    _check_tensor(targets, (B, K), "BCE targets")
    dev = targets.device
    if out is not None:
        logits, losses, preds = out
    else:
        logits = torch.empty(nh, B, K, device=dev)
        losses = torch.empty(nh + 1, device=dev)
        preds = torch.empty(nh, B, K, dtype=torch.int32, device=dev)
    if weights is not None:
        L.check(L.lib().m2m_heads_bce_w(arr, nh, targets.data_ptr(), pos_weight.data_ptr(), B, D, K, logits.data_ptr(),
                                        losses.data_ptr(), preds.data_ptr(), int(zero_losses), weights.data_ptr(), L.stream_ptr()),
                "heads_bce_w")
    else:
        L.check(L.lib().m2m_heads_bce(arr, nh, targets.data_ptr(), pos_weight.data_ptr(), B, D, K, logits.data_ptr(),
                                      losses.data_ptr(), preds.data_ptr(), int(zero_losses), L.stream_ptr()), "heads_bce")
    return logits, losses, preds


def heads_ce(heads: Sequence[dict], labels: torch.Tensor, B: int, D: int, K: int, out=None, zero_losses: bool = True,
             weights: Optional[torch.Tensor] = None):
    nh = len(heads)
    _check_weights(weights, nh)
    arr = _head_array(heads)
    dev = labels.device
    if out is not None:
        logits, losses, preds = out
    else:
        logits = torch.empty(nh, B, K, device=dev)
        losses = torch.empty(nh + 1, device=dev)
        preds = torch.empty(nh, B, dtype=torch.int32, device=dev)
    if weights is not None:
        L.check(L.lib().m2m_heads_ce_w(arr, nh, labels.data_ptr(), B, D, K, logits.data_ptr(), losses.data_ptr(),
                                       preds.data_ptr(), int(zero_losses), weights.data_ptr(), L.stream_ptr()), "heads_ce_w")
    else:
        L.check(L.lib().m2m_heads_ce(arr, nh, labels.data_ptr(), B, D, K, logits.data_ptr(), losses.data_ptr(),
                                     preds.data_ptr(), int(zero_losses), L.stream_ptr()), "heads_ce")
    return logits, losses, preds
```

Baseline: 1.047 million.

## Store captured-step input slots in bf16 for patch-embedding forward and wgrad

Adds bf16 input paths to the fused patch-embedding forward and weight-gradient kernels. In bf16 mode the captured step's input slots are converted to bf16 once at capture, so each step reads half the input bytes and skips the per-element fp32-to-bf16 packing. The data loader can also hold audio in bf16. The cost is extra template instantiations and stricter alignment and width requirements (W % 8). Numerics are unchanged because the kernels already rounded inputs to bf16.

New measurement: 1.053 million (median of 6 runs). About the same (+0.6%).

```diff
diff --git a/include/m2mixer.h b/include/m2mixer.h
--- a/include/m2mixer.h
+++ b/include/m2mixer.h
@@ -107,6 +107,10 @@
 int m2m_embeds_forward(const m2m_embed* const* embeds, const float* const* inputs, float* const* x0s, const int* nsplits,
                        const int64_t* part_strides, int nembeds, int B, const m2m_step_head* head, void* stream);
 int m2m_embed_fwd_splits(const m2m_embed* e);
+#define M2M_IN_F32 0
+#define M2M_IN_BF16 1
+int m2m_embeds_forward_in(const m2m_embed* const* embeds, const void* const* inputs, const int* in_dtypes, float* const* x0s,
+                          const int* nsplits, const int64_t* part_strides, int nembeds, int B, const m2m_step_head* head, void* stream);
 int m2m_embed_forward_head(const m2m_embed* e, const float* input, int B, float* x0, const m2m_step_head* head, void* stream);
 
 int m2m_tower_forward(const m2m_tower* t, const float* x0, int64_t x0_sample_stride, int B,
@@ -188,6 +192,11 @@
                           const m2m_tower* const* embed_towers, int nembeds,
                           int B, uint32_t seed, uint32_t step, const uint32_t* step_dev,
                           const m2m_head* heads, int nheads, int K, uint32_t* bump_counter, void* stream);
+int m2m_towers_wgrad_in(const m2m_tower* const* towers, const m2m_tower* const* dev_towers, int ntowers,
+                        const m2m_embed* const* embeds, const void* const* inputs, const int* in_dtypes, const float* const* d_x0s,
+                        const m2m_tower* const* embed_towers, int nembeds,
+                        int B, uint32_t seed, uint32_t step, const uint32_t* step_dev,
+                        const m2m_head* heads, int nheads, int K, uint32_t* bump_counter, void* stream);
 
 int m2m_tower_backward_heads_ok(const m2m_tower* t, int B, int nheads, int K);
 int m2m_tower_backward_heads(const m2m_tower* t, int B, const m2m_head* heads, int nheads, int own, const int64_t* labels,
diff --git a/m2_mixer_amd/_lib.py b/m2_mixer_amd/_lib.py
--- a/m2_mixer_amd/_lib.py
+++ b/m2_mixer_amd/_lib.py
@@ -42,6 +42,7 @@
                 ("dx0_chn", _fp)]
 
 
+IN_F32, IN_BF16 = 0, 1
 WGRAD_OVERWRITE = 1
 WGRAD_REDUCES_SMALL = 2
 WGRAD_GROUP_SLOTS = 4
@@ -144,6 +145,11 @@
     "m2m_embeds_forward": (C.c_int, [C.POINTER(C.POINTER(Embed)), C.POINTER(_fp), C.POINTER(_fp), C.POINTER(C.c_int), C.POINTER(C.c_int64),
                                      C.c_int, C.c_int, C.POINTER(StepHead), _fp]),
     "m2m_embed_fwd_splits": (C.c_int, [C.POINTER(Embed)]),
+    "m2m_embeds_forward_in": (C.c_int, [C.POINTER(C.POINTER(Embed)), C.POINTER(_fp), C.POINTER(C.c_int), C.POINTER(_fp), C.POINTER(C.c_int),
+                                        C.POINTER(C.c_int64), C.c_int, C.c_int, C.POINTER(StepHead), _fp]),
+    "m2m_towers_wgrad_in": (C.c_int, [C.POINTER(C.POINTER(Tower)), C.POINTER(_fp), C.c_int, C.POINTER(C.POINTER(Embed)), C.POINTER(_fp),
+                                      C.POINTER(C.c_int), C.POINTER(_fp), C.POINTER(C.POINTER(Tower)), C.c_int, C.c_int, C.c_uint32,
+                                      C.c_uint32, _fp, C.POINTER(Head), C.c_int, C.c_int, _fp, _fp]),
     "m2m_heads_ce": (C.c_int, [C.POINTER(Head), C.c_int, _fp, C.c_int, C.c_int, C.c_int, _fp, _fp, _fp, C.c_int, _fp]),
     "m2m_step_prologue": (C.c_int, [_fp, _fp, _fp, C.c_int, _fp]),
     "m2m_heads_bce": (C.c_int, [C.POINTER(Head), C.c_int, _fp, _fp, C.c_int, C.c_int, C.c_int, _fp, _fp, _fp, C.c_int, _fp]),
diff --git a/m2_mixer_amd/config.py b/m2_mixer_amd/config.py
--- a/m2_mixer_amd/config.py
+++ b/m2_mixer_amd/config.py
@@ -25,6 +25,7 @@
     "M2M_HEAD_SLOTS": ("1", "engine construction", "the heads' weight gradients through slots (bit-reproducible) instead of float atomics"),
     "M2M_GROUP_SLOTS": ("1", "engine construction", "the two-tower backward's small gradients through per-workgroup slots"),
     "M2M_EMBED_FAST": ("1", "engine construction", "patch-embedding weight gradients in the single-owner form (d_x0^T image)"),
+    "M2M_INPUT_BF16": ("1", "engine construction", "bf16 precision: bf16 input slots of a captured step for embeddings on the fast forms (0: fp32 slots)"),
     "M2M_EMBED_FOLD": ("0", "engine construction", "patch embeddings inside the two-tower forward launch"),
     "M2M_MIMIC_STREAMS": (None, "engine construction", "none / fwd / bwd / both: side streams of the MIMIC step; unset: none up to batch 1024, else both"),
     "M2M_MIMIC_MERGED_TAIL": ("1", "engine construction", "MIMIC on one stream: one weight-gradient launch, one Adam, one re-pack"),
diff --git a/m2_mixer_amd/csrc/embed.hip b/m2_mixer_amd/csrc/embed.hip
--- a/m2_mixer_amd/csrc/embed.hip
+++ b/m2_mixer_amd/csrc/embed.hip
@@ -29,6 +29,7 @@
     unsigned int* drop_counter;
     float* losses;
     int nlosses, prologue;
+    int in_bf16[2];
 };
 template <int P, int D, int RB>
 __global__ __launch_bounds__(NTHREADS, (P == PREC_BF16 && D <= 128) ? 4 : 1) void embed_fwd_group_kernel(const EmbedFwdGroupArgs a) {
@@ -43,7 +44,11 @@
     const int wg = e ? blockIdx.x - a.nwg0 : blockIdx.x;
     if (P == PREC_BF16 && a.fast[e]) {
         const int ns = a.nsplit[e], split = wg % ns;
-        embed_fwd_fast_body<D>(a.em[e], a.in[e], a.M[e], a.N[e], a.x0[e] + split * a.part_stride[e], wg / ns, split, ns, smem);
+        if (a.in_bf16[e])
+            embed_fwd_fast_body<D, m2m_bf16_in>(a.em[e], reinterpret_cast<const m2m_bf16_in*>(a.in[e]), a.M[e], a.N[e],
+                                                a.x0[e] + split * a.part_stride[e], wg / ns, split, ns, smem);
+        else
+            embed_fwd_fast_body<D>(a.em[e], a.in[e], a.M[e], a.N[e], a.x0[e] + split * a.part_stride[e], wg / ns, split, ns, smem);
     }
     else {
         const int ns = a.nsplit[e], split = wg % ns, tile = wg / ns;
@@ -98,8 +103,8 @@
                                                   (int)embed_fwd_fast_ok(e, in), hd);
 }
 template <int P, int D>
-static int launch_embed_fwd_group(const m2m_embed* const* es, const float* const* ins, float* const* x0s, const int* nsplits,
-                                  const int64_t* part_strides, const m2m_step_head* head, int B, hipStream_t st) {
+static int launch_embed_fwd_group(const m2m_embed* const* es, const float* const* ins, const int* in_dtypes, float* const* x0s,
+                                  const int* nsplits, const int64_t* part_strides, const m2m_step_head* head, int B, hipStream_t st) {
     constexpr int RB = 16;
     EmbedFwdGroupArgs a;
     memset(&a, 0, sizeof(a));
@@ -114,6 +119,13 @@
         const int N = (es[i]->H / es[i]->ph) * (es[i]->W / es[i]->pw);
         a.em[k] = *es[i]; a.in[k] = ins[i]; a.x0[k] = x0s[i]; a.N[k] = N; a.M[k] = (long)B * N;
         a.fast[k] = embed_fwd_fast_ok(es[i], ins[i]);
+        if (in_dtypes && in_dtypes[i] == M2M_IN_BF16) {
+            if (!embed_fwd_fast_ok_bf16(es[i], ins[i])) {
+                m2m_set_error("embeds_forward_in: a bf16 input needs bf16 mode, pw % 8 == 0, W % 8 == 0 and a 16-byte aligned address", __FILE__, __LINE__);
+                return -1;
+            }
+            a.fast[k] = 1; a.in_bf16[k] = 1;
+        }
         a.nsplit[k] = nsplits ? nsplits[i] : 1;
         a.part_stride[k] = part_strides ? (long)part_strides[i] : 0;
         if (a.nsplit[k] < 1 || a.nsplit[k] > 4 || (a.nsplit[k] > 1 && a.part_stride[k] < a.M[k] * (long)D)) {
@@ -191,7 +203,15 @@
 
 extern "C" int m2m_embeds_forward(const m2m_embed* const* embeds, const float* const* inputs, float* const* x0s, const int* nsplits,
                                   const int64_t* part_strides, int nembeds, int B, const m2m_step_head* head, void* stream) {
+    return m2m_embeds_forward_in(embeds, reinterpret_cast<const void* const*>(inputs), nullptr, x0s, nsplits, part_strides, nembeds, B, head, stream);
+}
+extern "C" int m2m_embeds_forward_in(const m2m_embed* const* embeds, const void* const* inputs_, const int* in_dtypes, float* const* x0s,
+                                     const int* nsplits, const int64_t* part_strides, int nembeds, int B, const m2m_step_head* head,
+                                     void* stream) {
+    const float* const* inputs = reinterpret_cast<const float* const*>(inputs_);
     if (!embeds || !inputs || !x0s || nembeds != 2) { m2m_set_error("embeds_forward: exactly two embeddings", __FILE__, __LINE__); return -1; }
+    for (int i = 0; in_dtypes && i < nembeds; ++i)
+        if (in_dtypes[i] != M2M_IN_F32 && in_dtypes[i] != M2M_IN_BF16) { m2m_set_error("embeds_forward_in: unknown input dtype", __FILE__, __LINE__); return -1; }
     for (int i = 0; i < nembeds; ++i) {
         if (int rc = m2m_check_embed(embeds[i], B)) return rc;
         if (embeds[i]->prec != embeds[0]->prec || embeds[i]->D != embeds[0]->D) {
@@ -201,7 +221,7 @@
     }
     hipStream_t st = reinterpret_cast<hipStream_t>(stream);
     const m2m_embed* e = embeds[0];
-    const int rc = m2m_dispatch_pd(m2m_wide_dims{}, e->prec, e->D, [&](auto P, auto D) { return launch_embed_fwd_group<P(), D()>(embeds, inputs, x0s, nsplits, part_strides, head, B, st); });
+    const int rc = m2m_dispatch_pd(m2m_wide_dims{}, e->prec, e->D, [&](auto P, auto D) { return launch_embed_fwd_group<P(), D()>(embeds, inputs, in_dtypes, x0s, nsplits, part_strides, head, B, st); });
     if (rc != M2M_NO_BUILD) return rc;
     m2m_set_error("embeds_forward: unsupported (prec, D)", __FILE__, __LINE__);
     return -1;
diff --git a/m2_mixer_amd/csrc/embed_fwd.h b/m2_mixer_amd/csrc/embed_fwd.h
--- a/m2_mixer_amd/csrc/embed_fwd.h
+++ b/m2_mixer_amd/csrc/embed_fwd.h
@@ -109,8 +109,10 @@
 
 #define EMB_FKS 256
 #define EMB_FDEPTH 2
-template <int D>
-static __device__ __forceinline__ void embed_fwd_fast_body(const m2m_embed& em, const float* __restrict__ in, long M, int N,
+template <class TI> struct EmbFwdSlot { f32x4_t p0, p1; };
+template <> struct EmbFwdSlot<m2m_bf16_in> { u32x4_t q; };
+template <int D, class TI = float>
+static __device__ __forceinline__ void embed_fwd_fast_body(const m2m_embed& em, const TI* __restrict__ in, long M, int N,
                                                            float* __restrict__ x0, int wg, int split, int nsplit, char* smem) {
     typedef Prec<PREC_BF16> Pr;
     constexpr int KSB = EMB_FKS / 32, DT = D / 16, DPW = (DT + NWAVES - 1) / NWAVES, IMG_B = 16 * EMB_FKS * 2;
@@ -129,14 +131,18 @@
 #pragma unroll
     for (int j = 0; j < DPW; ++j) acc[j] = f32x4_t{0.f, 0.f, 0.f, 0.f};
     struct Pre {
-        f32x4_t p0, p1;
+        EmbFwdSlot<TI> s;
         Frag w[DPW][KSB];
     };
     auto load = [&](Pre& p, int st) {
         const int k = min(st * EMB_FKS + wave * 32 + 8 * g, em.K - 8);
-        const float* src = in + (rb >= 0 ? rb : 0) + patch_koff(pg, k);
-        p.p0 = *reinterpret_cast<const f32x4_t*>(src);
-        p.p1 = *reinterpret_cast<const f32x4_t*>(src + 4);
+        const TI* src = in + (rb >= 0 ? rb : 0) + patch_koff(pg, k);
+        if constexpr (InIsBf16<TI>::v) {
+            p.s.q = *reinterpret_cast<const u32x4_t*>(src);
+        } else {
+            p.s.p0 = *reinterpret_cast<const f32x4_t*>(src);
+            p.s.p1 = *reinterpret_cast<const f32x4_t*>(src + 4);
+        }
 #pragma unroll
         for (int j = 0; j < DPW; ++j) {
             const int dt = min(wave + NWAVES * j, DT - 1);
@@ -147,8 +153,12 @@
     auto step = [&](Pre& p, int st) {
         const bool valid = rb >= 0 && st < nst && st * EMB_FKS + wave * 32 + 8 * g < em.K;
         Frag f;
-        f.u[0] = pack_bf2(p.p0[0], p.p0[1]); f.u[1] = pack_bf2(p.p0[2], p.p0[3]);
-        f.u[2] = pack_bf2(p.p1[0], p.p1[1]); f.u[3] = pack_bf2(p.p1[2], p.p1[3]);
+        if constexpr (InIsBf16<TI>::v) {
+            f.u = p.s.q;
+        } else {
+            f.u[0] = pack_bf2(p.s.p0[0], p.s.p0[1]); f.u[1] = pack_bf2(p.s.p0[2], p.s.p0[3]);
+            f.u[2] = pack_bf2(p.s.p1[0], p.s.p1[1]); f.u[3] = pack_bf2(p.s.p1[2], p.s.p1[3]);
+        }
         if (!valid) f.u = u32x4_t{0u, 0u, 0u, 0u};
         char* cur = img + ((st - st_begin) & 1) * IMG_B;
         *reinterpret_cast<u32x4_t*>(cur + tid * 16) = f.u;
@@ -186,3 +196,6 @@
 static inline bool embed_fwd_fast_ok(const m2m_embed* e, const float* in) {
     return e->prec == PREC_BF16 && e->pw % 8 == 0 && e->W % 4 == 0 && e->K >= 8 && (reinterpret_cast<uintptr_t>(in) & 15) == 0;
 }
+static inline bool embed_fwd_fast_ok_bf16(const m2m_embed* e, const void* in) {
+    return e->prec == PREC_BF16 && e->pw % 8 == 0 && e->W % 8 == 0 && e->K >= 8 && (reinterpret_cast<uintptr_t>(in) & 15) == 0;
+}
diff --git a/m2_mixer_amd/csrc/embed_wgrad.h b/m2_mixer_amd/csrc/embed_wgrad.h
--- a/m2_mixer_amd/csrc/embed_wgrad.h
+++ b/m2_mixer_amd/csrc/embed_wgrad.h
@@ -1,7 +1,12 @@
 #pragma once
 #include "host.h"
+#include <type_traits>
 
 #define EBM 32
+
+typedef unsigned short m2m_bf16_in;
+template <class TI> struct InIsBf16 { static constexpr bool v = false; };
+template <> struct InIsBf16<m2m_bf16_in> { static constexpr bool v = true; };
 
 struct PatchGeom {
     int Cin, H, W, ph, pw, GW, N, K;
@@ -133,8 +138,8 @@
 
 #define EFK 32
 template <int D, int NT> static constexpr size_t embed_wgrad_fast_red_bytes() { return (size_t)(NT / 64) * (EFK / 16) * (D / 16) * 64 * 16; }
-template <int D, int NT>
-static __device__ __forceinline__ void embed_wgrad_fast_body(const m2m_embed& em, const float* __restrict__ in,
+template <int D, int NT, class TI = float>
+static __device__ __forceinline__ void embed_wgrad_fast_body(const m2m_embed& em, const TI* __restrict__ in,
                                                              const char* __restrict__ dx0_chn, long M, int N, int npairs, int rpt,
                                                              int chunk, bool vec2, char* smem) {
     typedef Prec<PREC_BF16> Pr;
@@ -159,7 +164,9 @@
 #pragma unroll
         for (int dt = 0; dt < DT; ++dt) acc[jb][dt] = f32x4_t{0.f, 0.f, 0.f, 0.f};
 
-    struct Tile { Frag a[DT]; float v[NB][8]; unsigned int okbits; };
+    constexpr bool BI = InIsBf16<TI>::v;
+    typedef typename std::conditional<BI, unsigned int, float>::type vin_t;
+    struct Tile { Frag a[DT]; vin_t v[NB][8]; unsigned int okbits; };
     auto load = [&](Tile& t, int p) {
 #pragma unroll
         for (int dt = 0; dt < DT; ++dt) t.a[dt] = ld_frag_global(dx0_chn, (long)p * DT + dt, lane);
@@ -180,8 +187,12 @@
             const unsigned int k2 = (unsigned int)max(ko[0], 0);
 #pragma unroll
             for (int e = 0; e < 8; ++e) {
-                const float2 x = *reinterpret_cast<const float2*>(in + rb[e] + k2);
-                t.v[0][e] = x.x; t.v[1][e] = x.y;
+                if constexpr (BI) {
+                    t.v[0][e] = *reinterpret_cast<const unsigned int*>(in + rb[e] + k2);
+                } else {
+                    const float2 x = *reinterpret_cast<const float2*>(in + rb[e] + k2);
+                    t.v[0][e] = x.x; t.v[1][e] = x.y;
+                }
             }
         } else {
 #pragma unroll
@@ -197,11 +208,22 @@
 #pragma unroll
         for (int jb = 0; jb < NB; ++jb) {
             Frag b;
+            if constexpr (BI) {
+                unsigned int z[8];
+#pragma unroll
+                for (int e = 0; e < 8; ++e) {
+                    const unsigned int raw = vec2 ? (jb ? t.v[0][e] >> 16 : t.v[0][e] & 0xFFFFu) : t.v[jb][e];
+                    z[e] = ((t.okbits >> e) & 1u) && ko[jb] >= 0 ? raw : 0u;
+                }
+#pragma unroll
+                for (int e = 0; e < 4; ++e) b.u[e] = z[2 * e] | (z[2 * e + 1] << 16);
+            } else {
             float z[8];
 #pragma unroll
             for (int e = 0; e < 8; ++e) z[e] = ((t.okbits >> e) & 1u) && ko[jb] >= 0 ? t.v[jb][e] : 0.f;
 #pragma unroll
             for (int e = 0; e < 4; ++e) b.u[e] = pack_bf2(z[2 * e], z[2 * e + 1]);
+            }
 #pragma unroll
             for (int dt = 0; dt < DT; ++dt) Pr::mma(acc[jb][dt], t.a[dt], b);
         }
@@ -277,6 +299,7 @@
     int N[EMB_GROUP], tpg[EMB_GROUP], nchunks[EMB_GROUP], groups[EMB_GROUP];
     const char* dx0_chn[EMB_GROUP];
     int npairs[EMB_GROUP], rpt[EMB_GROUP], vec2[EMB_GROUP], fast;
+    int in_bf16[EMB_GROUP];
 };
 template <int P, int D, int NT>
 static __device__ __forceinline__ void embed_wgrad_group_body(const EmbedWgradGroupArgs& a, int id, char* smem) {
@@ -292,6 +315,17 @@
     if constexpr (NT % 64 == 0 && EBM % (NT / 64) == 0)
         embed_wgrad_body<P, D, NT>(a.em[e], a.in[e], a.dx0[e], a.M[e], a.N[e], a.tpg[e], id % a.nchunks[e], id / a.nchunks[e],
                                    a.groups[e] == 1, smem);
+}
+
+template <int D, int NT>
+static __device__ __forceinline__ void embed_wgrad_group_body_in(const EmbedWgradGroupArgs& a, int id, char* smem) {
+    const int e = id < a.nchunks[0] ? 0 : 1;
+    if (e) id -= a.nchunks[0];
+    if (a.in_bf16[e])
+        embed_wgrad_fast_body<D, NT, m2m_bf16_in>(a.em[e], reinterpret_cast<const m2m_bf16_in*>(a.in[e]), a.dx0_chn[e], a.M[e], a.N[e],
+                                                  a.npairs[e], a.rpt[e], id, a.vec2[e] != 0, smem);
+    else
+        embed_wgrad_fast_body<D, NT, float>(a.em[e], a.in[e], a.dx0_chn[e], a.M[e], a.N[e], a.npairs[e], a.rpt[e], id, a.vec2[e] != 0, smem);
 }
 
 struct EmbedWgradPlan { long M; int N, nchunks, groups, tpg; };
@@ -314,7 +348,7 @@
 
 
 static inline int embed_wgrad_group_args_fast(EmbedWgradGroupArgs& a, const m2m_embed* const* es, const float* const* ins,
-                                              const m2m_tower* const* tw, int B) {
+                                              const m2m_tower* const* tw, int B, const int* in_dtypes = nullptr) {
     memset(&a, 0, sizeof(a));
     int total = 0;
     for (int i = 0; i < EMB_GROUP; ++i) {
@@ -329,7 +363,9 @@
         a.M[i] = (long)B * N; a.N[i] = N; a.npairs[i] = (nchain * BM + WPAIR - 1) / WPAIR; a.rpt[i] = SPW * t->N;
         a.nchunks[i] = (e->K + EFK - 1) / EFK; a.groups[i] = 1; a.tpg[i] = 0;
         static const int vec2_on = m2m_env_int("M2M_EMBED_VEC2", 1);
-        a.vec2[i] = (vec2_on && e->pw % 2 == 0 && e->W % 2 == 0 && ((long)e->H * e->W) % 2 == 0 && e->K % 2 == 0 && ((uintptr_t)ins[i] & 7) == 0) ? 1 : 0;
+        a.in_bf16[i] = in_dtypes && in_dtypes[i] == M2M_IN_BF16;
+        a.vec2[i] = (vec2_on && e->pw % 2 == 0 && e->W % 2 == 0 && ((long)e->H * e->W) % 2 == 0 && e->K % 2 == 0 &&
+                     ((uintptr_t)ins[i] & (a.in_bf16[i] ? 3 : 7)) == 0) ? 1 : 0;
         total += a.nchunks[i];
     }
     a.fast = 1;
diff --git a/m2_mixer_amd/csrc/tower_wgrad.hip b/m2_mixer_amd/csrc/tower_wgrad.hip
--- a/m2_mixer_amd/csrc/tower_wgrad.hip
+++ b/m2_mixer_amd/csrc/tower_wgrad.hip
@@ -350,7 +350,12 @@
         return;
     }
     if (id < a.n_embed_pad) {
-        if (id < a.n_embed_first) embed_wgrad_group_body<P, D, WgradKernelGeom<P, D, RCDM>::THREADS>(ea, id, smem);
+        if (id < a.n_embed_first) {
+            if constexpr (P == PREC_BF16) {
+                if (ea.in_bf16[0] | ea.in_bf16[1]) { embed_wgrad_group_body_in<D, WgradKernelGeom<P, D, RCDM>::THREADS>(ea, id, smem); return; }
+            }
+            embed_wgrad_group_body<P, D, WgradKernelGeom<P, D, RCDM>::THREADS>(ea, id, smem);
+        }
         return;
     }
     id -= a.n_embed_pad;
@@ -466,7 +471,8 @@
 static int launch_wgrad_group(const m2m_tower* const* host, const m2m_tower* const* dev, int n, const m2m_embed* const* embeds,
                               const float* const* inputs, const float* const* d_x0s, const m2m_tower* const* embed_towers,
                               int nembeds, int B, unsigned int seed, unsigned int step, const unsigned int* step_dev, hipStream_t st,
-                              const SplitReduceTower* heads_reduce = nullptr, unsigned int* bump_counter = nullptr) {
+                              const SplitReduceTower* heads_reduce = nullptr, unsigned int* bump_counter = nullptr,
+                              const int* in_dtypes = nullptr) {
     typedef WgradKernelGeom<P, D, RCDM> KG;
     WgradGroupArgs a;
     memset(&a, 0, sizeof(a));
@@ -511,8 +517,14 @@
     int n_embed_wgs = 0;
     size_t lds_e = 0;
     bool embeds_separately = false;
+    bool in_bf16 = false;
+    for (int i = 0; in_dtypes && i < nembeds; ++i) in_bf16 = in_bf16 || in_dtypes[i] == M2M_IN_BF16;
     if (nembeds) {
-        n_embed_wgs = (P == PREC_BF16 && nembeds == EMB_GROUP) ? embed_wgrad_group_args_fast(ea, embeds, inputs, embed_towers, B) : 0;
+        n_embed_wgs = (P == PREC_BF16 && nembeds == EMB_GROUP) ? embed_wgrad_group_args_fast(ea, embeds, inputs, embed_towers, B, in_dtypes) : 0;
+        if (in_bf16 && !(n_embed_wgs && ea.fast)) {
+            m2m_set_error("towers_wgrad_in: a bf16 embedding input needs the single-owner form (m2m_embeds_wgrad_form)", __FILE__, __LINE__);
+            return -1;
+        }
         if (n_embed_wgs) lds_e = embed_wgrad_fast_lds<D, KG::THREADS>();
         else if (KG::THREADS == 256) { static const int ewgs = m2m_env_int("M2M_EMBED_WGS", D >= 256 ? 128 : 512);    n_embed_wgs = embed_wgrad_group_args(ea, embeds, inputs, d_x0s, B, ewgs, nembeds); lds_e = embed_wgrad_lds<D, P>(); }
         else embeds_separately = true;
@@ -523,7 +535,7 @@
     }
     if constexpr (P == PREC_BF16) {
         static const int merged = m2m_env_int("M2M_EMBED_MERGED", 1);
-        if (n_embed_wgs && ea.fast && !merged && KG::THREADS != 256) {
+        if (n_embed_wgs && ea.fast && !merged && !in_bf16 && KG::THREADS != 256) {
             const size_t le = embed_wgrad_fast_lds<D, 256>();
             if (int rc = m2m_launch<embed_wgrad_fast_group_kernel<D>>(dim3((unsigned)n_embed_wgs), dim3(256), le, le, st, ea)) return rc;
             n_embed_wgs = 0; lds_e = 0;
@@ -532,6 +544,9 @@
     const size_t lds_t = (size_t)KG::LDS_B;
     const size_t lds = lds_t > lds_e ? lds_t : lds_e;
     static const int embed_first = m2m_env_int("M2M_EMBED_FIRST", 1);
+    if (in_bf16) {
+        a.n_embed_first = n_embed_wgs; a.n_embed_pad = (n_embed_wgs + 7) & ~7; n_embed_wgs = 0;
+    } else
     if (ea.fast && n_embed_wgs && embed_first) { a.n_embed_first = n_embed_wgs; a.n_embed_pad = (n_embed_wgs + 7) & ~7; n_embed_wgs = 0; }
     SplitReduceArgs ra;
     memset(&ra, 0, sizeof(ra));
@@ -593,7 +608,8 @@
                              const m2m_embed* const* embeds, const float* const* inputs, const float* const* d_x0s,
                              const m2m_tower* const* embed_towers, int nembeds,
                              int B, uint32_t seed, uint32_t step, const uint32_t* step_dev,
-                             const m2m_head* heads, int nheads, int K, void* stream, uint32_t* bump_counter = nullptr) {
+                             const m2m_head* heads, int nheads, int K, void* stream, uint32_t* bump_counter = nullptr,
+                             const int* in_dtypes = nullptr) {
     SplitReduceTower hr;
     const SplitReduceTower* heads_reduce = nullptr;
     if (heads && nheads > 0) {
@@ -638,8 +654,17 @@
             return -1;
         }
     }
+    bool in_bf16 = false;
+    for (int i = 0; in_dtypes && i < nembeds; ++i) {
+        if (in_dtypes[i] != M2M_IN_F32 && in_dtypes[i] != M2M_IN_BF16) { m2m_set_error("towers_wgrad_in: unknown input dtype", __FILE__, __LINE__); return -1; }
+        in_bf16 = in_bf16 || in_dtypes[i] == M2M_IN_BF16;
+    }
     hipStream_t st = reinterpret_cast<hipStream_t>(stream);
     const m2m_tower* t = towers[0];
+    if (in_bf16 && m2m_wgrad_recompute(t, B)) {
+        m2m_set_error("towers_wgrad_in: a bf16 embedding input needs the stored-operand form", __FILE__, __LINE__);
+        return -1;
+    }
     if (bump_counter && m2m_wgrad_recompute(t, B)) {
         m2m_set_error("towers_wgrad_tail: the recompute form READS the dropout counter in this launch; advance it with m2m_counter_add", __FILE__, __LINE__);
         return -1;
@@ -649,7 +674,7 @@
             return launch_wgrad_group<PREC_BF16, 128, DM()>(towers, dev_towers, ntowers, embeds, inputs, d_x0s, embed_towers, nembeds, B, seed, step, step_dev, st, heads_reduce);
         });
     const int rc = m2m_dispatch_pd(m2m_wide_dims{}, t->prec, t->D, [&](auto P, auto D) {
-        return launch_wgrad_group<P(), D(), -1>(towers, dev_towers, ntowers, embeds, inputs, d_x0s, embed_towers, nembeds, B, seed, step, step_dev, st, heads_reduce, bump_counter);
+        return launch_wgrad_group<P(), D(), -1>(towers, dev_towers, ntowers, embeds, inputs, d_x0s, embed_towers, nembeds, B, seed, step, step_dev, st, heads_reduce, bump_counter, in_dtypes);
     });
     if (rc != M2M_NO_BUILD) return rc;
     m2m_set_error("towers_wgrad: unsupported (prec, D)", __FILE__, __LINE__);
@@ -676,6 +701,15 @@
                                      int B, uint32_t seed, uint32_t step, const uint32_t* step_dev,
                                      const m2m_head* heads, int nheads, int K, uint32_t* bump_counter, void* stream) {
     return towers_wgrad_impl(towers, dev_towers, ntowers, embeds, inputs, d_x0s, embed_towers, nembeds, B, seed, step, step_dev, heads, nheads, K, stream, bump_counter);
+}
+
+extern "C" int m2m_towers_wgrad_in(const m2m_tower* const* towers, const m2m_tower* const* dev_towers, int ntowers,
+                                   const m2m_embed* const* embeds, const void* const* inputs, const int* in_dtypes, const float* const* d_x0s,
+                                   const m2m_tower* const* embed_towers, int nembeds,
+                                   int B, uint32_t seed, uint32_t step, const uint32_t* step_dev,
+                                   const m2m_head* heads, int nheads, int K, uint32_t* bump_counter, void* stream) {
+    return towers_wgrad_impl(towers, dev_towers, ntowers, embeds, reinterpret_cast<const float* const*>(inputs), d_x0s, embed_towers, nembeds, B,
+                             seed, step, step_dev, heads, nheads, K, stream, bump_counter, in_dtypes);
 }
 
 extern "C" int m2m_embeds_wgrad_form(const m2m_embed* const* embeds, const m2m_tower* const* embed_towers, int nembeds, int B) {
diff --git a/m2_mixer_amd/data.py b/m2_mixer_amd/data.py
--- a/m2_mixer_amd/data.py
+++ b/m2_mixer_amd/data.py
@@ -11,7 +11,10 @@
 
     TRAIN_SPLIT = 55000
 
-    def __init__(self, root_dir: str, device="cuda:0", rank: int = 0, world: int = 1):
+    def __init__(self, root_dir: str, device="cuda:0", rank: int = 0, world: int = 1, input_dtype: torch.dtype = torch.float32):
+        if input_dtype not in (torch.float32, torch.bfloat16):
+            raise ValueError("input_dtype: torch.float32 or torch.bfloat16")
+        self.input_dtype = input_dtype
         self.device = torch.device(device)
         self.rank, self.world = rank, world
         self.splits: Dict[str, Tuple[torch.Tensor, torch.Tensor, torch.Tensor]] = {}
@@ -30,7 +33,7 @@
         if image.shape[0] != audio.shape[0] or image.shape[0] != labels.shape[0]:
             raise ValueError(f"{stage}: image / audio / label counts differ")
         image = torch.from_numpy(image.astype(np.float32)).reshape(image.shape[0], 1, 28, 28)
-        audio = torch.from_numpy(audio.astype(np.float32))[:, None, :, :]
+        audio = torch.from_numpy(audio.astype(np.float32))[:, None, :, :].to(self.input_dtype)
         labels = torch.from_numpy(labels.astype(np.int64))
         return image.to(self.device), audio.to(self.device), labels.to(self.device)
 
diff --git a/m2_mixer_amd/engine.py b/m2_mixer_amd/engine.py
--- a/m2_mixer_amd/engine.py
+++ b/m2_mixer_amd/engine.py
@@ -562,6 +562,9 @@
             for m in mods:
                 m.pack(force=True)
 
+    def _slot_like(self, i: int, t: torch.Tensor) -> torch.Tensor:
+        return t.clone()
+
     def release_capture(self):
         self._graph = None
         self._static = None
@@ -570,7 +573,7 @@
         if steps < 1 or (steps > 1 and grad_sync is not None):
             raise ValueError("steps > 1 is only supported without a gradient exchange")
         nb = len(batch)
-        slots = [tuple(t.clone() for t in batch) for _ in range(steps)]
+        slots = [tuple(self._slot_like(i, t) for i, t in enumerate(batch)) for _ in range(steps)]
         if steps > 1 and config.switch_on("M2M_CAPTURE_SHARE_SLOTS"):
             slots = [slots[0]] * steps
         self._static = slots[0] if steps == 1 else slots
@@ -716,6 +719,19 @@
                             and towers_forward_embeds_ok([self.t_a, self.t_b], [self.e_a, self.e_b], B)
                             and self.t_a.wgrad_form(B) == 0 and self.t_fus.wgrad_form(B) == 0)
         self._pending_bump = False
+        self._in_bf16 = (False, False)
+        if (config.switch_on("M2M_INPUT_BF16") and self.t_a.prec == L.PREC_BF16 and grouped and self.concurrent
+                and not self._embed_fold and can_group_embeds(self.e_a, self.e_b) and self.e_a.prec == self.t_a.prec
+                and self.e_a.D == self.t_a.D and len(self._embed_towers) == 2
+                and L.lib().m2m_embeds_wgrad_form(_embed_ptrs(self._embeds), _tower_ptrs(self._embed_towers), 2, B)
+                and self.t_a.wgrad_form(B) == 0 and self.t_fus.wgrad_form(B) == 0):
+            self._in_bf16 = tuple(bool(e.prec == L.PREC_BF16 and e.desc.pw % 8 == 0 and e.desc.W % 8 == 0 and e.K >= 8)
+                                  for e in (self.e_a, self.e_b))
+
+    def _slot_like(self, i: int, t: torch.Tensor) -> torch.Tensor:
+        if i < 2 and self._in_bf16[i] and t.dtype == torch.float32:
+            return t.to(torch.bfloat16)
+        return t.clone()
 
     def _build_fusion(self):
         B, D, dev = self.B, self.D, self.device
diff --git a/m2_mixer_amd/runtime.py b/m2_mixer_amd/runtime.py
--- a/m2_mixer_amd/runtime.py
+++ b/m2_mixer_amd/runtime.py
@@ -41,6 +41,15 @@
 
 def _data_ptrs(tensors):
     return (C.c_void_p * max(len(tensors), 1))(*[t.data_ptr() for t in tensors])
+
+
+def _in_dtypes(tensors):
+    codes = []
+    for t in tensors:
+        if t.dtype not in (torch.float32, torch.bfloat16):
+            raise RuntimeError(f"patch embedding input: float32 or bfloat16, got {t.dtype}")
+        codes.append(L.IN_BF16 if t.dtype == torch.bfloat16 else L.IN_F32)
+    return (C.c_int * len(codes))(*codes) if L.IN_BF16 in codes else None
 
 
 def _device_descs(towers):
@@ -422,6 +431,13 @@
                  heads: Optional[Sequence[dict]] = None, K: int = 0, bump: Optional[torch.Tensor] = None):
     n, ne = len(towers), len(embeds)
     et = _tower_ptrs(embed_towers) if len(embed_towers) == ne and ne else None
+    dts = _in_dtypes(inputs)
+    if dts is not None:
+        L.check(L.lib().m2m_towers_wgrad_in(_tower_ptrs(towers), _device_descs(towers), n, _embed_ptrs(embeds), _data_ptrs(inputs), dts,
+                                            _data_ptrs(d_x0s), et, ne, B, *_drop_tail(seed, step, step_dev)[:3],
+                                            _head_array(heads) if heads else None, len(heads) if heads else 0, K, L.ptr(bump),
+                                            L.stream_ptr()), "towers_wgrad_in")
+        return
     args = (_tower_ptrs(towers), _device_descs(towers), n, _embed_ptrs(embeds), _data_ptrs(inputs), _data_ptrs(d_x0s), et, ne, B,
             *_drop_tail(seed, step, step_dev)[:3])
     if bump is not None:
@@ -473,6 +489,11 @@
             e.mark_packed()
 
 
+def _float32_input(t: torch.Tensor, what: str):
+    if t.dtype != torch.float32:
+        raise RuntimeError(f"{what}: this launch takes float32 inputs only (bfloat16: embeds_forward / towers_wgrad), got {t.dtype}")
+
+
 class EmbedRuntime:
 
     def __init__(self, Cin: int, H: int, W: int, ph: int, pw: int, D: int, prec: int):
@@ -526,10 +547,12 @@
 
     def forward(self, inp: torch.Tensor, B: int, x0: torch.Tensor, step_head: Optional[tuple] = None):
         head = _step_head(step_head[0], step_head[2], step_head[1]) if step_head is not None else None
+        _float32_input(inp, "embed_forward")
         L.check(L.lib().m2m_embed_forward_head(C.byref(self.desc), inp.data_ptr(), B, x0.data_ptr(), head, L.stream_ptr()),
                 "embed_forward")
 
     def wgrad(self, inp: torch.Tensor, d_x0: torch.Tensor, B: int):
+        _float32_input(inp, "embed_wgrad")
         L.check(L.lib().m2m_embed_wgrad(C.byref(self.desc), inp.data_ptr(), d_x0.data_ptr(), B, L.stream_ptr()),
                 "embed_wgrad")
 
@@ -544,6 +567,11 @@
     ns = (C.c_int * n)(*(nsplits if nsplits is not None else [1] * n))
     ps = (C.c_int64 * n)(*[B * e.N * e.D for e in embeds])
     head = _step_head(step_head[0], step_head[2], step_head[1]) if step_head is not None else None
+    dts = _in_dtypes(inputs)
+    if dts is not None:
+        L.check(L.lib().m2m_embeds_forward_in(_embed_ptrs(embeds), _data_ptrs(inputs), dts, _data_ptrs(x0s), ns, ps, n, B, head,
+                                              L.stream_ptr()), "embeds_forward_in")
+        return
     L.check(L.lib().m2m_embeds_forward(_embed_ptrs(embeds), _data_ptrs(inputs), _data_ptrs(x0s), ns, ps, n, B, head, L.stream_ptr()),
             "embeds_forward")
 
```
